# soham97/mellow

Measured on AMD Instinct MI355X. Metric: audio-pair responses/sec (v0 167M, 2x10s clips, max_len=64, greedy), higher is better.
Workload: dtype f32 (encoder/prefill GEMM operands split EXACTLY into 3 bf16 terms, 6 bf16 MFMA products per fp32 product, f32 accumulate: fp32-accurate, parity suite green; mel included, the STFT is an fp32 FFT; attentions and decode on exact fp32 MFMA / VALU)

## Files before the change

### mellow_amd/csrc/decode.hip

```cpp
#include "common.h"
#include "kernels.h"
#include <cstdio>
#include <mutex>
#include <set>
#include <type_traits>
#include <utility>

namespace mellow {

__device__ uint64_t* g_kdbg = nullptr;
#ifdef MELLOW_KDEBUG
__device__ __forceinline__ void kstamp(int slot, int idx, bool who) {
    if (g_kdbg && who) g_kdbg[slot * 8 + idx] = __builtin_readcyclecounter();
}
__device__ __forceinline__ void kspan(int seq, int end) {
    if (g_kdbg && seq >= 0 && seq < 480 && threadIdx.x == 0) {
        const unsigned long long t = wall_clock64();
        if (end) atomicMax(reinterpret_cast<unsigned long long*>(g_kdbg) + 64 + 2 * seq + 1, t);
        else atomicMin(reinterpret_cast<unsigned long long*>(g_kdbg) + 64 + 2 * seq, t);
    }
}
#else
#define kstamp(slot, idx, who) ((void)0)
#define kspan(seq, end) ((void)0)
// ... 209 lines not shown
        }
        if (nt == 0) {
            ssp = half_sum(ssp);
            if (lane < 32) ssq_s[wave * 32 + lane] = ssp;
        }
#pragma unroll
        for (int r = 0; r < 16; ++r) red[(wave * 16 + r) * 64 + lane] = acc[r];
    }
    __syncthreads();
    if (nt == 0 && tid < 32)
    {
        float ssum = ssq_s[tid & 31];
#pragma unroll
        for (int wv = 1; wv < QW; ++wv) ssum += ssq_s[wv * 32 + (tid & 31)];
        a.ssq1[((int64_t)rb * 32 + tid) * DEC_KC_QKV + kc] = ssum;
    }
    if (tid >= 256) return;
    const int mm = tid & 31, hh = (tid >> 5) & 1, gq = tid >> 6;
    float v[4];
#pragma unroll
    for (int j = 0; j < 4; ++j) {
        const int r = 4 * gq + j;
        float sacc = red[r * 64 + mm + 32 * hh];
#pragma unroll
        for (int wv = 1; wv < QW; ++wv) sacc += red[(wv * 16 + r) * 64 + mm + 32 * hh];
        v[j] = sacc;
    }
    const int n = nt * 32 + 8 * gq + 4 * hh;
    if (W8) {
#pragma unroll
        for (int j = 0; j < 4; ++j) v[j] *= wscale[n + j];
    }
    if (n < 960)
        *reinterpret_cast<float4*>(a.pq + ((int64_t)kc * a.rows + rb * 32 + mm) * 960 + n) = make_float4(v[0], v[1], v[2], v[3]);
    kspan(a.dbg_seq, 1);
}

#ifndef MELLOW_DA_ABL
#define MELLOW_DA_ABL 0
#endif
#ifndef MELLOW_DA_WAVES
#define MELLOW_DA_WAVES 8
#define MELLOW_DA_G 7
#endif
#ifndef MELLOW_DA_MINW
#define MELLOW_DA_MINW 4
#endif
constexpr int DA_MINW = MELLOW_DA_WAVES == 8 || MELLOW_DA_WAVES == 4 ? MELLOW_DA_MINW : 1;
constexpr int DA_WAVES = MELLOW_DA_WAVES;
constexpr int DA_G = MELLOW_DA_G;
#ifndef MELLOW_DA_G1
#define MELLOW_DA_G1 5
#endif
constexpr int DA_G1 = MELLOW_DA_G1 < DA_G ? MELLOW_DA_G1 : DA_G;
#ifndef MELLOW_DA16_MFMA
#define MELLOW_DA16_MFMA 1
#endif
constexpr int DA_GM = 8;
#ifndef MELLOW_DA16_KNT
#define MELLOW_DA16_KNT 0
#endif
#ifndef MELLOW_DA16_MINW
#define MELLOW_DA16_MINW MELLOW_DA_MINW
#endif
#ifndef MELLOW_DA16_NW
#define MELLOW_DA16_NW 8
#endif

template <bool KV16>
__device__ __forceinline__ float4 ld_kv(const float* page, int64_t elem) {
    if constexpr (KV16) {
        typedef unsigned u32x2 __attribute__((ext_vector_type(2)));
        const u32x2 r = __builtin_nontemporal_load(reinterpret_cast<const u32x2*>(reinterpret_cast<const uint16_t*>(page) + elem));
        return make_float4(__uint_as_float(r[0] << 16), __uint_as_float(r[0] & 0xffff0000u), __uint_as_float(r[1] << 16), __uint_as_float(r[1] & 0xffff0000u));
    } else {
        return ldg_nt(reinterpret_cast<const float4*>(page + elem));
    }
}
template <bool KV16>
__device__ __forceinline__ void st_kv(float* page, int64_t elem, float v) {
    if constexpr (KV16) reinterpret_cast<__bf16*>(page)[elem] = static_cast<__bf16>(v);
    else page[elem] = v;
}
template <bool BLK, bool FUSED, bool ONE, bool KV16, int NW, int TS>
__global__ __launch_bounds__(NW * 64, ONE ? 2 : (KV16 && MELLOW_DA16_MFMA && DA_MINW > 1 ? MELLOW_DA16_MINW : DA_MINW)) void dec_attn_kernel(float* __restrict__ k_cache, float* __restrict__ v_cache,
                                                                  const int32_t* __restrict__ d_pos_p, const float* __restrict__ pq_p,
                                                                  const float* __restrict__ xmidF_p, int Tmax_p, int gs_p, int rows_p,
                                                                  const DecArgs a) {
    kspan(a.dbg_seq, 0);
    __shared__ float ssq_part[3];
    __shared__ __attribute__((aligned(16))) float qs[3 * 64];
    __shared__ __attribute__((aligned(16))) float knew[64], vnew[64];
    __shared__ __attribute__((aligned(16))) float xs[320];
    __shared__ __attribute__((aligned(16))) float ored[DA_WAVES * 3 * 64];
    __shared__ float mred[DA_WAVES * 3], lred[DA_WAVES * 3];
    __shared__ float snew_s[3];
    constexpr bool MF = KV16 && MELLOW_DA16_MFMA != 0;
    __shared__ __attribute__((aligned(16))) float pl[MF ? DA_WAVES * 32 * 4 : 4];
    __shared__ __attribute__((aligned(16))) __bf16 qb[MF ? 10 * 64 : 8];
    constexpr int VPW = DA_WAVES / NW;
    static_assert(DA_WAVES % NW == 0 && (MF || NW == DA_WAVES), "the vector form runs one chunk stream per wave");
    auto mf_group = [&](int g0, int u) { return g0 + u * DA_WAVES; };

    static_assert(TS == DEC_TS || !(ONE || KV16), "one row block and the bf16 pages always run DEC_TS key splits (kernels.h dec_key_splits)");
    const int g = blockIdx.x, b = blockIdx.y, sp = blockIdx.z;
    int row = b;
    if (BLK) {
        const int live = a.blk_live[b >> 5];
        if (a.row_of_slot) row = a.row_of_slot[b];
        if (live == 0 || row < 0) return;
    }
    const int tid = threadIdx.x, lane = tid & 63, wave = tid >> 6;
    const int Tmax = Tmax_p;
    float* kpage = k_cache + (((int64_t)row * 3 + g) * Tmax * 64 >> (KV16 ? 1 : 0));
    float* vpage = v_cache + (((int64_t)row * 3 + g) * Tmax * 64 >> (KV16 ? 1 : 0));
    const int sub = lane >> 4, quad = lane & 15;

    const bool dbg = tid == 0 && g == 0 && b == 0 && sp == 0;
    kstamp(1, 0, dbg);
#ifdef MELLOW_POS_VECTOR_LOAD
    const int pos = __builtin_amdgcn_readfirstlane(*reinterpret_cast<const volatile int*>(d_pos_p));
#else
    const int pos = *d_pos_p;
#endif
    const int hsel = (tid >> 5) & 3, i = tid & 31;
    const int r = tid < 80 ? tid : 0;
    const int pcol = r < 48 ? (3 * g + (r >> 4)) * 64 + 4 * (r & 15) : r < 64 ? 576 + g * 64 + 4 * (r - 48) : 768 + g * 64 + 4 * (r - 64);
    const float* prow = pq_p + (int64_t)b * 960 + pcol;
    constexpr int NPQ = FUSED ? Q2_NPQ : DEC_KC_QKV;
    float4 sl4[NPQ], sq4[2];
    if (tid < 80) {
#pragma unroll
        for (int s = 0; s < NPQ; ++s)
            sl4[s] = (MELLOW_DA_ABL & 4) ? make_float4(0.1f * s, 0.2f, 0.3f, 0.4f) : *reinterpret_cast<const float4*>(prow + (int64_t)s * rows_p * 960);
        if (!FUSED) {
            sq4[0] = reinterpret_cast<const float4*>(a.ssq1 + (int64_t)b * DEC_KC_QKV)[0];
            sq4[1] = reinterpret_cast<const float4*>(a.ssq1 + (int64_t)b * DEC_KC_QKV)[1];
        }
    }
    float4 xr4 = make_float4(0.f, 0.f, 0.f, 0.f), xd4[FUSED ? Q2_HC : 1];
    if (FUSED && tid < 144) {
        const int64_t fi = ((int64_t)(b >> 5) * 72 + (tid >> 1)) * 64 + (b & 31) + 32 * (tid & 1);
        xr4 = reinterpret_cast<const float4*>(xmidF_p)[fi];
#pragma unroll
        for (int s = 0; s < Q2_HC; ++s) xd4[s] = reinterpret_cast<const float4*>(a.dslabF)[(int64_t)s * a.slabF_stride4 + fi];
    }
    const float c = a.rope_cur[i], sn = a.rope_cur[32 + i];
    const int gbeg = sp * gs_p;
    const int gend_fixed = sp == TS - 1 ? 0x3fffffff : gbeg + gs_p;
    typedef unsigned u32x2 __attribute__((ext_vector_type(2)));
    const int kk = lane & 31, hf = lane >> 5;
    i32x4 kq[4];
    u32x2 vq[DA_GM];
    auto load_ktile = [&](int g0) {
        const int gi = g0 + (kk >> 2) * DA_WAVES;
        const int tc = min(gi * 4 + (kk & 3), Tmax - 1);
        const i32x4* kp = reinterpret_cast<const i32x4*>(reinterpret_cast<const uint16_t*>(kpage) + (int64_t)tc * 64 + hf * 32);
#pragma unroll
        for (int st = 0; st < 4; ++st)
            kq[st] = (MELLOW_DA_ABL & 1) ? i32x4{tc, 0x3c003c00, st, 0x3c003c00} : (MELLOW_DA16_KNT ? __builtin_nontemporal_load(kp + st) : kp[st]);
    };
    auto load_vgroup = [&](int g0, int u) {
        const int gi = mf_group(g0, u);
        const int tc = min(gi * 4 + sub, Tmax - 1);
        vq[u] = (MELLOW_DA_ABL & 1) ? u32x2{0x3c003c00u, (unsigned)tc}
                                    : __builtin_nontemporal_load(reinterpret_cast<const u32x2*>(reinterpret_cast<const uint16_t*>(vpage) + (int64_t)tc * 64 + quad * 4));
    };
    float4 k4[MF ? 1 : DA_G], v4[MF ? 1 : DA_G];
    auto load_group = [&](int u) {
        const int gi = gbeg + wave + u * DA_WAVES;
        const int tc = min(gi * 4 + sub, Tmax - 1);
        if (MELLOW_DA_ABL & 1) {
            k4[u] = make_float4(0.01f * tc, 0.02f, 0.03f, 0.04f);
            v4[u] = make_float4(0.01f, 0.02f * tc, 0.03f, 0.04f);
        } else {
            k4[u] = ld_kv<KV16>(kpage, (int64_t)tc * 64 + quad * 4);
            v4[u] = ld_kv<KV16>(vpage, (int64_t)tc * 64 + quad * 4);
        }
    };
    const int g_first_mf = gbeg + wave;
    if constexpr (MF) {
        load_ktile(g_first_mf);
#pragma unroll
        for (int u = 0; u < DA_GM / 2; ++u) load_vgroup(g_first_mf, u);
    } else {
#pragma unroll
        for (int u = 0; u < DA_G1; ++u) load_group(u);
    }
    MELLOW_HOIST(a.attF16); MELLOW_HOIST(a.att_ml); MELLOW_HOIST(a.RB); MELLOW_HOIST(a.eps);
    if (FUSED) MELLOW_HOIST(a.xnewR);
    __builtin_amdgcn_sched_barrier(0);
    kstamp(1, 1, dbg);

    const int ngroups = (pos + 3) >> 2;
    const int gend = min(ngroups, gend_fixed);
    static_assert(DEC_KC_QKV == 8, "fixed summation order below");
    if (FUSED) {
        if (tid < 192) {
            float4 x = xr4;
#pragma unroll
            for (int s = 0; s < Q2_HC; ++s) x = f4add(x, xd4[s]);
            const float ss = wave_sum(tid < 144 ? f4ssq(x) : 0.f);
            if (lane == 0) ssq_part[wave] = ss;
            if (g == 0 && sp == 0 && tid < 144) reinterpret_cast<float4*>(a.xnewR + (int64_t)b * 576)[tid] = x;
        }
        if (tid < 80) {
            float4 x = sl4[0];
#pragma unroll
            for (int s = 1; s < NPQ; ++s) x = f4add(x, sl4[s]);
            *reinterpret_cast<float4*>(xs + 4 * tid) = x;
        }
    } else if (tid < 80) {
        float4 x = sl4[0];
#pragma unroll
        for (int s = 1; s < DEC_KC_QKV; ++s) x = f4add(x, sl4[s]);
        const float ssum = ((sq4[0].x + sq4[0].y) + (sq4[0].z + sq4[0].w)) + ((sq4[1].x + sq4[1].y) + (sq4[1].z + sq4[1].w));
        const float rscale = 1.0f / sqrtf(ssum / 576.0f + a.eps);
        *reinterpret_cast<float4*>(xs + 4 * tid) = make_float4(x.x * rscale, x.y * rscale, x.z * rscale, x.w * rscale);
    }
    __syncthreads();
    kstamp(1, 2, dbg);
    const float rs2 = FUSED ? 1.0f / sqrtf(((ssq_part[0] + ssq_part[1]) + ssq_part[2]) / 576.0f + a.eps) : 1.0f;
    if (tid < 128) {
        const int base = hsel < 3 ? hsel * 64 : 192;
        const float x1 = xs[base + i] * rs2, x2 = xs[base + i + 32] * rs2;
        const float o1 = __fadd_rn(__fmul_rn(x1, c), __fmul_rn(-x2, sn));
        const float o2 = __fadd_rn(__fmul_rn(x2, c), __fmul_rn(x1, sn));
        if (hsel < 3) {
            qs[hsel * 64 + i] = o1 * 0.125f;
            qs[hsel * 64 + i + 32] = o2 * 0.125f;
            if constexpr (MF) {
                __bf16 p0, p1, p2;
                split3(o1 * 0.125f, p0, p1, p2);
                qb[(0 * 3 + hsel) * 64 + i] = p0; qb[(1 * 3 + hsel) * 64 + i] = p1; qb[(2 * 3 + hsel) * 64 + i] = p2;
                split3(o2 * 0.125f, p0, p1, p2);
                qb[(0 * 3 + hsel) * 64 + i + 32] = p0; qb[(1 * 3 + hsel) * 64 + i + 32] = p1; qb[(2 * 3 + hsel) * 64 + i + 32] = p2;
            }
        } else {
            knew[i] = o1; knew[i + 32] = o2;
            if (sp == 0) { st_kv<KV16>(kpage, (int64_t)pos * 64 + i, o1); st_kv<KV16>(kpage, (int64_t)pos * 64 + i + 32, o2); }
        }
    } else if (tid < 192) {
        const float x1 = xs[256 + tid - 128] * rs2;
        vnew[tid - 128] = x1;
        if (sp == 0) st_kv<KV16>(vpage, (int64_t)pos * 64 + (tid - 128), x1);
    } else if (MF && tid < 256) {
        qb[9 * 64 + tid - 192] = static_cast<__bf16>(0.f);
    }
    __syncthreads();
    __builtin_amdgcn_sched_barrier(0);
    if constexpr (MF) {
#pragma unroll
        for (int u = DA_GM / 2; u < DA_GM; ++u) load_vgroup(g_first_mf, u);
    } else {
#pragma unroll
        for (int u = DA_G1; u < DA_G; ++u) load_group(u);
    }
    __builtin_amdgcn_sched_barrier(0);
    kstamp(1, 3, dbg);

    if (wave < 3) {
        const float sn_ = wave_sum(qs[wave * 64 + lane] * knew[lane]);
        if (lane == 0) snew_s[wave] = sn_;
    }
    float4 q4[3];
    const int aq_off = ((kk >> 2) < 3 && (kk & 3) < 3 ? (kk >> 2) * 3 + (kk & 3) : 9) * 64 + hf * 32;
    if constexpr (!MF) {
#pragma unroll
        for (int hh = 0; hh < 3; ++hh) q4[hh] = *reinterpret_cast<const float4*>(qs + hh * 64 + quad * 4);
    }
    float m_run[3] = {-INFINITY, -INFINITY, -INFINITY};
    float l_run[3] = {0.f, 0.f, 0.f};
    float4 acc[3];
#pragma unroll
    for (int hh = 0; hh < 3; ++hh) acc[hh] = make_float4(0.f, 0.f, 0.f, 0.f);

#define MELLOW_DA_CHUNK(g0)                                                                                              \
    {                                                                                                                    \
        float sc[DA_G][3];                                                                                               \
        float cmax[3] = {-INFINITY, -INFINITY, -INFINITY};                                                               \
_Pragma("unroll")                                                                                                        \
        for (int u = 0; u < DA_G; ++u) {                                                                                 \
            const int gi = g0 + u * DA_WAVES;                                                                            \
            const int t = gi * 4 + sub;                                                                                  \
            const bool ok = gi < gend && t < pos;                                                                        \
_Pragma("unroll")                                                                                                        \
            for (int hh = 0; hh < 3; ++hh) {                                                                             \
                float sv = q4[hh].x * k4[u].x + q4[hh].y * k4[u].y + q4[hh].z * k4[u].z + q4[hh].w * k4[u].w;            \
                sv = row16_sum(sv);                                                                                      \
                sv = ok ? sv : -INFINITY;                                                                                \
                sc[u][hh] = sv;                                                                                          \
                cmax[hh] = fmaxf(cmax[hh], sv);                                                                          \
            }                                                                                                            \
        }                                                                                                                \
_Pragma("unroll")                                                                                                        \
        for (int hh = 0; hh < 3; ++hh) {                                                                                 \
            float cm = cmax[hh];                                                                                         \
            cm = fmaxf(cm, swz_xor16(cm));                                                                               \
            cm = half_max(cm);                                                                                           \
            const float m_new = fmaxf(m_run[hh], cm);                                                                    \
            const float alpha = fast_exp(m_run[hh] - m_new);                                                             \
            m_run[hh] = m_new;                                                                                           \
// ... 369 lines not shown
#pragma unroll
    for (int r = 0; r < 16; ++r) acc[r] = 0.f;
    if constexpr (W8 == 2) {
        float am = 0.f, inv, sc;
#pragma unroll
        for (int i = 0; i < KPW; ++i) am = fmaxf(am, f4amax(x[i]));
        a8_scales(half_max(am), inv, sc);
        uint32_t xq[KPW];
#pragma unroll
        for (int i = 0; i < KPW; ++i) xq[i] = q4_e4m3(x[i], inv);
        acc = mfma8_32<KPW>(acc, w8, xq);
#pragma unroll
        for (int r = 0; r < 16; ++r) acc[r] *= sc;
    } else {
#pragma unroll
        for (int i = 0; i < KPW; ++i) acc = mfma4(acc, w[i], x[i]);
    }
    kstamp(dslot, 2, dbg && acc[0] == acc[0]);
#pragma unroll
    for (int r = 0; r < 16; ++r) red[(wave * 16 + r) * 64 + lane] = acc[r];
    __syncthreads();
    kstamp(dslot, 3, dbg);
    const bool epi = tid < 256;
    const int mm = tid & 31, hh = (tid >> 5) & 1, gq = (tid >> 6) & 3;
    float v[4];
#pragma unroll
    for (int j = 0; j < 4; ++j) {
        const int r = 4 * gq + j;
        float sacc = red[r * 64 + mm + 32 * hh];
#pragma unroll
        for (int wv = 1; wv < LM_WAVES; ++wv) sacc += red[(wv * 16 + r) * 64 + mm + 32 * hh];
        v[j] = sacc;
    }
    {
        const int n = nt * 32 + 8 * gq + 4 * hh;
        if (W8) {
#pragma unroll
            for (int j = 0; j < 4; ++j) v[j] *= wscale[n + j];
        }
        const int64_t row = (int64_t)rb * 32 + mm;
        if (epi && a.logits && n < N) *reinterpret_cast<float4*>(a.logits + row * N + n) = make_float4(v[0], v[1], v[2], v[3]);
        __syncthreads();
        float bv = v[0];
        int bi = n;
#pragma unroll
        for (int j = 1; j < 4; ++j)
            if (arg_better(v[j], n + j, bv, bi)) { bv = v[j]; bi = n + j; }
        if (epi) {
            red[tid] = bv;
            reinterpret_cast<int*>(red)[256 + tid] = bi;
        }
        __syncthreads();
        if (tid < 32) {
            float best = red[tid];
            int idx = reinterpret_cast<int*>(red)[256 + tid];
#pragma unroll
            for (int q = 1; q < 8; ++q) {
                const float ov = red[tid + 32 * q];
                const int oi = reinterpret_cast<int*>(red)[256 + tid + 32 * q];
                if (arg_better(ov, oi, best, idx)) { best = ov; idx = oi; }
            }
            const int64_t o = ((int64_t)rb * 32 + tid) * (N >> 5) + nt;
            a.cand_val[o] = best;
            a.cand_idx[o] = idx;
        }
    }
    kspan(a.dbg_seq, 1);
}


#ifndef MELLOW_H3_NW
#define MELLOW_H3_NW 8
#endif
#ifndef MELLOW_H3R_D1
#define MELLOW_H3R_D1 1
#endif
#ifndef MELLOW_H3R_D2
#define MELLOW_H3R_D2 1
#endif
#ifndef MELLOW_H3R_D4
#define MELLOW_H3R_D4 1
#endif
constexpr int H3_NW = MELLOW_H3_NW, H3_CP = 3, H3_NC = 36 / H3_CP;
template <int G, int D, bool BLK>
__global__ __launch_bounds__(H3_NW * 64) void dec_head3r_kernel(const float* __restrict__ Wp, const i32x4* __restrict__ X3, int K8p, int N,
                                                                int RB_p, const DecArgs a) {
    kspan(a.dbg_seq, 0);
    extern __shared__ __attribute__((aligned(16))) i32x4 xs[];
    constexpr int PPH = 36 / G, NCH = PPH / H3_CP;
    constexpr int STAGE = G * PPH * 3 * 64;
    static_assert(PPH * G == 36 && NCH * H3_CP == PPH && H3_NC % D == 0 && NCH % D == 0, "phases hold whole chunks");
    const int tid = threadIdx.x, lane = tid & 63, wave = tid >> 6;
    const int nt = blockIdx.x * H3_NW + wave;
    const float4* wbase = reinterpret_cast<const float4*>(Wp) + (int64_t)nt * K8p * 64 + lane;
    for (int rb0 = 0; rb0 < RB_p; rb0 += G) {
        const int gn = min(G, RB_p - rb0);
        f32x16 acc[G];
#pragma unroll
        for (int g = 0; g < G; ++g)
#pragma unroll
            for (int r = 0; r < 16; ++r) acc[g][r] = 0.f;
        float4 wn[D][2 * H3_CP];
#pragma unroll
        for (int d = 0; d < D; ++d)
#pragma unroll
            for (int i = 0; i < 2 * H3_CP; ++i) wn[d][i] = ldg_nt(wbase + (d * 2 * H3_CP + i) * 64);
        for (int ph = 0; ph < G; ++ph) {
            if (ph || rb0) __syncthreads();
            {
                constexpr int FILL = (STAGE + H3_NW * 64 - 1) / (H3_NW * 64);
                i32x4 t[FILL];
#pragma unroll
                for (int j = 0; j < FILL; ++j) {
                    const int i = tid + j * H3_NW * 64;
                    if (i < STAGE) {
                        const int g = i / (PPH * 3 * 64), rest = i % (PPH * 3 * 64);
                        t[j] = X3[(((int64_t)(rb0 + (g < gn ? g : 0)) * 36 + ph * PPH) * 3) * 64 + rest];
                    }
                }
#pragma unroll
                for (int j = 0; j < FILL; ++j) {
                    const int i = tid + j * H3_NW * 64;
                    if (i < STAGE) xs[i] = t[j];
                }
            }
            __syncthreads();
            for (int c0 = 0; c0 < NCH; c0 += D) {
#pragma unroll
                for (int d = 0; d < D; ++d) {
                    const int cc = c0 + d, c = ph * NCH + cc;
                    float4 w[2 * H3_CP];
#pragma unroll
                    for (int i = 0; i < 2 * H3_CP; ++i) w[i] = wn[d][i];
                    if (c + D < H3_NC) {
#pragma unroll
                        for (int i = 0; i < 2 * H3_CP; ++i) wn[d][i] = ldg_nt(wbase + ((c + D) * 2 * H3_CP + i) * 64);
                    }
                    __builtin_amdgcn_sched_barrier(0);
                    i32x4 wp[H3_CP][3];
#pragma unroll
                    for (int p = 0; p < H3_CP; ++p) {
                        pair_natural(w[2 * p], w[2 * p + 1]);
                        split_pair(w[2 * p], w[2 * p + 1], wp[p][0], wp[p][1], wp[p][2]);
                    }
                    const i32x4* st = xs + (cc * H3_CP) * 3 * 64 + lane;
#pragma unroll
                    for (int g = 0; g < G; ++g) {
                        if (g < gn) {
#pragma unroll
                            for (int p = 0; p < H3_CP; ++p) {
                                const i32x4 xq[3] = {st[((g * PPH + p) * 3 + 0) * 64], st[((g * PPH + p) * 3 + 1) * 64], st[((g * PPH + p) * 3 + 2) * 64]};
                                acc[g] = mma6(acc[g], wp[p], xq);
                            }
                        }
                    }
                    __builtin_amdgcn_sched_barrier(0);
                }
            }
        }
        const int m = lane & 31, h = lane >> 5;
#pragma unroll
        for (int g = 0; g < G; ++g) {
            if (g < gn && !(BLK && a.blk_live[rb0 + g] == 0)) {
                const int64_t row = (int64_t)(rb0 + g) * 32 + m;
                float bv = -INFINITY;
                int bi = 0x7fffffff;
#pragma unroll
                for (int q = 0; q < 4; ++q) {
                    const int n = nt * 32 + 8 * q + 4 * h;
                    if (a.logits) *reinterpret_cast<float4*>(a.logits + row * N + n) = make_float4(acc[g][4 * q], acc[g][4 * q + 1], acc[g][4 * q + 2], acc[g][4 * q + 3]);
#pragma unroll
                    for (int j = 0; j < 4; ++j)
                        if (arg_better(acc[g][4 * q + j], n + j, bv, bi)) { bv = acc[g][4 * q + j]; bi = n + j; }
                }
                auto rv = __builtin_amdgcn_permlane32_swap(__float_as_uint(bv), __float_as_uint(bv), false, false);
                auto ri = __builtin_amdgcn_permlane32_swap((unsigned)bi, (unsigned)bi, false, false);
                const float ov = __uint_as_float(h ? rv[0] : rv[1]);
                const int oi = (int)(h ? ri[0] : ri[1]);
                if (arg_better(ov, oi, bv, bi)) { bv = ov; bi = oi; }
                if (h == 0) {
                    const int64_t o = row * (N >> 5) + nt;
                    a.cand_val[o] = bv;
                    a.cand_idx[o] = bi;
                }
            }
        }
    }
    kspan(a.dbg_seq, 1);
}

#define MELLOW_BF16S(W, X, ACC) ACC = __builtin_amdgcn_mfma_f32_16x16x32_bf16(__builtin_bit_cast(bf16x8, W), __builtin_bit_cast(bf16x8, X), ACC, 0, 0, 0)
__device__ __forceinline__ f32x4 mma6s(f32x4 acc, const i32x4 (&w)[3], const i32x4 (&x)[3]) {
// ... 519 lines not shown
        } else {
#pragma unroll
            for (int i = 0; i < HT; ++i) acc = mfma4(acc, w[i], h4[i]);
        }
        kstamp(7, 2, dbg && acc[0] == acc[0]);
        if (side) nt -= 30;
    }
#pragma unroll
    for (int r = 0; r < 16; ++r) red[(wave * 16 + r) * 64 + lane] = acc[r];
    __syncthreads();
    kstamp(7, 3, dbg);
    if (tid < 256) {
        const int mm = tid & 31, hh = (tid >> 5) & 1, gq = tid >> 6;
        float v[4];
#pragma unroll
        for (int j = 0; j < 4; ++j) {
            const int q = 4 * gq + j;
            float sacc = red[q * 64 + mm + 32 * hh];
#pragma unroll
            for (int wv = 1; wv < Q2W; ++wv) sacc += red[(wv * 16 + q) * 64 + mm + 32 * hh];
            v[j] = sacc;
        }
        const int n = nt * 32 + 8 * gq + 4 * hh;
        if (W8) {
#pragma unroll
            for (int j = 0; j < 4; ++j) v[j] *= wsc[n + j];
        }
        const float4 o = make_float4(v[0], v[1], v[2], v[3]);
        if (side) st_out(reinterpret_cast<float4*>(a.dslabF) + (int64_t)slab * a.slabF_stride4 + f32_idx(rb, 72, mm, n), o);
        else st_out(reinterpret_cast<float4*>(a.pq + ((int64_t)slab * a.rows + rb * 32 + mm) * 960 + n), o);
    }
    kstamp(7, 4, dbg);
    kspan(a.dbg_seq, 1);
}

template <int KCD, bool BLK>
__global__ __launch_bounds__(192) void dec_final_norm_kernel(const float* __restrict__ norm_w, const float* __restrict__ xmidF_p,
                                                             const float* __restrict__ dslabF_p, int64_t stride4_p, const DecArgs a) {
    kspan(a.dbg_seq, 0);
    __shared__ float part[3];
    const int b = blockIdx.x, tid = threadIdx.x;
    if (BLK && b == 0 && tid < 32) a.blk_snap[tid] = a.blk_live[tid];
    MELLOW_BLK_EXIT(b >> 5)
    const int xi = tid < 144 ? tid : 0;
    const int64_t fi = f32_idx(b >> 5, 72, b & 31, xi * 4);
    float4 v = reinterpret_cast<const float4*>(xmidF_p)[fi];
    float4 xs[KCD > 0 ? KCD : 1];
#pragma unroll
    for (int s = 0; s < KCD; ++s) xs[s] = reinterpret_cast<const float4*>(dslabF_p)[(int64_t)s * stride4_p + fi];
    const float4 wv = reinterpret_cast<const float4*>(norm_w)[xi];
#pragma unroll
    for (int s = 0; s < KCD; ++s) v = f4add(v, xs[s]);
    float ss = tid < 144 ? f4ssq(v) : 0.f;
    ss = wave_sum(ss);
    if ((tid & 63) == 0) part[tid >> 6] = ss;
    __syncthreads();
    const float r = 1.0f / sqrtf((part[0] + part[1] + part[2]) / 576.0f + a.eps);
    if (tid < 144) {
        float4 y;
        y.x = __fmul_rn(wv.x, __fmul_rn(v.x, r)); y.y = __fmul_rn(wv.y, __fmul_rn(v.y, r));
        y.z = __fmul_rn(wv.z, __fmul_rn(v.z, r)); y.w = __fmul_rn(wv.w, __fmul_rn(v.w, r));
        if (!a.xn3) reinterpret_cast<float4*>(a.xnF)[fi] = y;
    }
    if (a.xn3) {
        float4 y = make_float4(0.f, 0.f, 0.f, 0.f);
        if (tid < 144) {
            y.x = __fmul_rn(wv.x, __fmul_rn(v.x, r)); y.y = __fmul_rn(wv.y, __fmul_rn(v.y, r));
            y.z = __fmul_rn(wv.z, __fmul_rn(v.z, r)); y.w = __fmul_rn(wv.w, __fmul_rn(v.w, r));
        }
        const F3Quad mine = f3_split4(y), other = f3_partner(mine);
        if (tid < 144 && !(tid & 1)) f3_store8(a.xn3, f3_32_slot(b >> 5, 36, b & 31, tid * 4), mine, other);
    }
    kspan(a.dbg_seq, 1);
}

__global__ __launch_bounds__(256) void dec_argmax_kernel(const float* __restrict__ cand_val_p, const int32_t* __restrict__ cand_idx_p, int n,
                                                         const DecArgs a, int32_t* __restrict__ tokens,
                                                         const float* __restrict__ embed, int write_x, const LoopArgs lp) {
    kspan(a.dbg_seq, 0);
    __shared__ float bv[4];
    __shared__ int bi[4];
    __shared__ int tok_s;
    const int b = blockIdx.x, tid = threadIdx.x;
    const int row = lp.row_of_slot ? lp.row_of_slot[b] : b;
    const bool dead = (lp.blk_snap && lp.blk_snap[b >> 5] == 0) || row < 0;
    float best = -INFINITY;
    int idx = 0x7fffffff;
    if (!dead) {
        for (int i = tid; i < n; i += 256) {
            const float v = cand_val_p[(int64_t)b * n + i];
            const int id = cand_idx_p[(int64_t)b * n + i];
            if (arg_better(v, id, best, idx)) { best = v; idx = id; }
        }
#pragma unroll
        for (int off = 32; off > 0; off >>= 1) {
            const float ov = __shfl_xor(best, off, 64);
            const int oi = __shfl_xor(idx, off, 64);
            if (arg_better(ov, oi, best, idx)) { best = ov; idx = oi; }
        }
        if ((tid & 63) == 0) { bv[tid >> 6] = best; bi[tid >> 6] = idx; }
    }
    __syncthreads();
    if (tid == 0) {
        if (!dead) {
            for (int w = 1; w < 4; ++w)
                if (arg_better(bv[w], bi[w], best, idx)) { best = bv[w]; idx = bi[w]; }
            idx = min(max(idx, 0), n * 32 - 1);
            tokens[b] = idx;
            tok_s = idx;
        }
        if (lp.out_tokens) {
            if (!dead) {
                const int max_len = lp.params[0], stop_id = lp.params[1];
                const int step = *a.d_pos - lp.T0 + 1;
                if (step >= 0 && step < max_len) lp.out_tokens[(int64_t)row * max_len + step] = idx;
                if (idx == stop_id && lp.seen_stop[row] == 0) {
                    lp.seen_stop[row] = 1;
                    atomicAdd(lp.n_seen, 1);
                    if (lp.blk_left && atomicSub(lp.blk_left + (b >> 5), 1) == 1) lp.blk_live[b >> 5] = 0;
                }
            }
            asm volatile("s_waitcnt vmcnt(0)" ::: "memory");
            if (atomicAdd(lp.arrive, 1) == (int)gridDim.x - 1) {
                *lp.arrive = 0;
                const int t = *lp.ticket + 1;
                *lp.ticket = t;
                const int ns = atomicAdd(lp.n_seen, 0);
                __hip_atomic_store(lp.host_progress, ((unsigned long long)(unsigned)t << 32) | (unsigned)ns, __ATOMIC_RELAXED,
                                   __HIP_MEMORY_SCOPE_SYSTEM);
            }
        }
    }
    if (dead) return;
    if (write_x) {
        __syncthreads();
        if (tid < 144) {
            const float4 e = reinterpret_cast<const float4*>(embed + (int64_t)tok_s * 576)[tid];
            reinterpret_cast<float4*>(a.xmidF)[f32_idx(b >> 5, 72, b & 31, tid * 4)] = e;
        }
    }
    kspan(a.dbg_seq, 1);
}

__global__ __launch_bounds__(1024) void dec_compact_kernel(const DecArgs a, int B, const LoopArgs lp) {
    __shared__ int src_of[1024];
    __shared__ int row_new[1024];
    __shared__ int wsum[16];
    __shared__ int n_act_s, n_live_s;
    const int tid = threadIdx.x, lane = tid & 63, wave = tid >> 6;
    const int nblk = (B + 31) >> 5;
    int row = -1, active = 0;
    if (tid < B) {
        row = lp.row_of_slot[tid];
        active = row >= 0 && lp.blk_live[tid >> 5] != 0 && lp.seen_stop[row] == 0;
    }
    const unsigned long long m = __ballot(active);
    const int before = __popcll(m & ((1ull << lane) - 1ull));
    if (lane == 0) wsum[wave] = __popcll(m);
    if (tid == 0) {
        int live = 0;
        for (int k = 0; k < nblk; ++k) live += lp.blk_live[k] != 0;
        n_live_s = live;
    }
    src_of[tid] = -1;
    row_new[tid] = -1;
    __syncthreads();
    int base = 0;
    for (int w = 0; w < wave; ++w) base += wsum[w];
    if (tid == 0) {
        int n = 0;
        for (int w = 0; w < 16; ++w) n += wsum[w];
        n_act_s = n;
    }
    __syncthreads();
    const int n_act = n_act_s;
    if ((n_act + 31) / 32 >= n_live_s) return;
    if (active) { src_of[base + before] = tid; row_new[base + before] = row; }
    __syncthreads();
    float4* x = reinterpret_cast<float4*>(a.xmidF);
    for (int d0 = 0; d0 < n_act; d0 += 7) {
        const int d = d0 + tid / 144, c = tid % 144;
        const bool mv = tid < 1008 && d < n_act && src_of[d] != d;
        float4 v = make_float4(0.f, 0.f, 0.f, 0.f);
        if (mv) v = x[f32_idx(src_of[d] >> 5, 72, src_of[d] & 31, c * 4)];
        __syncthreads();
        if (mv) x[f32_idx(d >> 5, 72, d & 31, c * 4)] = v;
        __syncthreads();
    }
    if (tid < B) lp.row_of_slot[tid] = row_new[tid];
    if (tid < 32) {
        const int left = tid < nblk ? min(max(n_act - 32 * tid, 0), 32) : 0;
        lp.blk_left[tid] = left;
        lp.blk_live[tid] = left > 0;
    }
    if (tid == 0) *lp.n_compactions += 1;
}
__global__ __launch_bounds__(256) void kv_to_bf16_kernel(const float4* __restrict__ src, uint4* __restrict__ dst, int64_t n8) {
    for (int64_t i = (int64_t)blockIdx.x * 256 + threadIdx.x; i < n8; i += (int64_t)gridDim.x * 256) {
        const float4 a = src[2 * i], b = src[2 * i + 1];
        typedef __bf16 bf16x8v __attribute__((ext_vector_type(8)));
        const bf16x8v o = {static_cast<__bf16>(a.x), static_cast<__bf16>(a.y), static_cast<__bf16>(a.z), static_cast<__bf16>(a.w),
                           static_cast<__bf16>(b.x), static_cast<__bf16>(b.y), static_cast<__bf16>(b.z), static_cast<__bf16>(b.w)};
        dst[i] = __builtin_bit_cast(uint4, o);
    }
}
void launch_kv_to_bf16(const float* src, void* dst, int64_t n, hipStream_t s) {
    const int64_t n8 = n >> 3;
    const int blocks = (int)((n8 + 255) / 256 < 8192 ? (n8 + 255) / 256 : 8192);
    hipLaunchKernelGGL(kv_to_bf16_kernel, dim3(blocks), dim3(256), 0, s, reinterpret_cast<const float4*>(src), reinterpret_cast<uint4*>(dst), n8);
}
void launch_dec_compact(const DecArgs& a, int B, const LoopArgs& loop, hipStream_t s) {
    hipLaunchKernelGGL(dec_compact_kernel, dim3(1), dim3(1024), 0, s, a, B, loop);
}

__global__ __launch_bounds__(192) void dec_load_rows_kernel(const DecArgs a, const float* __restrict__ in, int64_t ld,
                                                            const int32_t* __restrict__ row_ids, int T_last, int n_src) {
    const int b = blockIdx.x, tid = threadIdx.x;
    const int64_t src = row_ids ? (int64_t)min(max(row_ids[b], 0), n_src - 1) : (int64_t)b * T_last + (T_last - 1);
    if (tid < 144) {
        const float4 e = reinterpret_cast<const float4*>(in + src * ld)[tid];
        reinterpret_cast<float4*>(a.xmidF)[f32_idx(b >> 5, 72, b & 31, tid * 4)] = e;
    }
}

void set_max_dynamic_lds(const void* fn, size_t bytes) {
    if (bytes <= 64 * 1024) return;
    static std::mutex mu;
    static std::set<std::pair<const void*, int>> done;
    int dev = 0;
    (void)hipGetDevice(&dev);
    std::lock_guard<std::mutex> lk(mu);
    if (done.insert({fn, dev}).second) {
        const hipError_t e = hipFuncSetAttribute(fn, hipFuncAttributeMaxDynamicSharedMemorySize, (int)bytes);
        if (e != hipSuccess) fprintf(stderr, "mellow: hipFuncSetAttribute(max dynamic LDS %zu) failed: %s\n", bytes, hipGetErrorString(e));
    }
}
template <class F> static inline void with_bool(bool v, F&& f) {
    if (v) f(std::true_type{}); else f(std::false_type{});
}
template <int V0, int... Vs, class F> static inline void with_int(int v, F&& f) {
    if constexpr (sizeof...(Vs) == 0) f(std::integral_constant<int, V0>{});
    else if (v == V0) f(std::integral_constant<int, V0>{});
    else with_int<Vs...>(v, f);
}
static inline int w8_mode(const DecArgs& a, const float* wscale) { return wscale ? (a.a8 ? 2 : 1) : 0; }
template <class F> static inline void with_blk_w8(const DecArgs& a, const float* wscale, F&& f) {
    with_bool(a.blk_live != nullptr, [&](auto blk) { with_int<2, 1, 0>(w8_mode(a, wscale), [&](auto w8) { f(blk, w8); }); });
}
void launch_dec_qkv(const DecArgs& a, const float* Wp, int K8p, int kcd, hipStream_t s, const float* wscale) {
    const dim3 grid(30, DEC_KC_QKV, a.RB);
    with_int<0, DEC_KC_DOWN>(kcd, [&](auto kcd_c) { with_bool(a.first != 0, [&](auto first) { with_blk_w8(a, wscale, [&](auto blk, auto w8) {
        hipLaunchKernelGGL((dec_qkv_kernel<kcd_c.value, blk.value, first.value, w8.value>), grid, dim3(QKV_THREADS), 0, s, Wp, (const float*)a.xmidF,
                           (const float*)a.dslabF, K8p, a, wscale);
    }); }); });
}
void launch_dec_attn(const DecArgs& a, float* k_cache, float* v_cache, bool fused, hipStream_t s) {
    const dim3 grid(3, a.rows, a.ts);
    const bool one = a.RB == 1 && !a.blk_live;
    if (a.ts != DEC_TS && (one || a.kv16 || a.ts != DEC_TS_MULTI)) {
        fprintf(stderr, "mellow: decode attention launched with %d key splits at RB = %d\n", a.ts, a.RB);
        abort();
    }
    auto launch = [&](auto blk, auto one_c) { with_bool(fused, [&](auto fused_c) { with_bool(a.kv16 != 0, [&](auto kv16) {
        constexpr bool ONE = one_c.value, KV16 = kv16.value;
        constexpr int NW = !KV16 ? DA_WAVES : MELLOW_DA16_MFMA && DA_WAVES == 8 && !ONE ? MELLOW_DA16_NW : DA_WAVES;
        constexpr int TSM = ONE || KV16 ? DEC_TS : DEC_TS_MULTI;
        with_int<DEC_TS, TSM>(a.ts, [&](auto ts) {
            hipLaunchKernelGGL((dec_attn_kernel<blk.value, fused_c.value, ONE, KV16, NW, ts.value>), grid, dim3(NW * 64), 0, s, k_cache, v_cache,
                               (const int32_t*)a.d_pos, (const float*)a.pq, (const float*)a.xmidF, a.Tmax, a.gs, a.rows, a);
        });
    }); }); };
    if (one) launch(std::false_type{}, std::true_type{});
    else with_bool(a.blk_live != nullptr, [&](auto blk) { launch(blk, std::false_type{}); });
}
static void launch_dec_qkv2_any(const DecArgs& a, const float* Wx, int K8x, const float* Wh, int K8h, const float* Wd,
                                const float* sc_x, const float* sc_h, const float* sc_d, hipStream_t s) {
    const dim3 grid(Q2_BLOCKS, a.RB);
#ifdef MELLOW_Q2_WAVES_FORCED
    bool few = false;
#else
    bool few = a.RB == 1;
#endif
    if (w8_mode(a, sc_x) == 2) few = false;
    with_bool(few, [&](auto few_c) { with_blk_w8(a, sc_x, [&](auto blk, auto w8) {
        constexpr int WV = few_c.value ? 4 : Q2_WAVES;
        hipLaunchKernelGGL((dec_qkv2_kernel<blk.value, WV, w8.value>), grid, dim3(WV * 64), 0, s, Wx, Wh, Wd, (const float*)a.xmidF,
                           (const float*)a.guF, K8x, K8h, a, sc_x, sc_h, sc_d);
    }); });
}
constexpr size_t dec_qkv2x3_lds(int rbm) { return (size_t)Q3W * rbm * 16 * 64 * 4; }
constexpr size_t dec_gateup3_lds(int rbm) { return (size_t)GU3W * rbm * 8 * 64 * 4; }
constexpr size_t dec_head3r_lds() { return (size_t)36 * 3 * 64 * 16; }
template <class F> static inline void with_qkv2x3(int rb, bool blk, F&& f) {
    with_int<1, 2, 4>(rb, [&](auto rbm) { with_bool(blk, [&](auto b) { f(&dec_qkv2x3_kernel<b.value, rbm.value>, dec_qkv2x3_lds(rbm.value)); }); });
}
template <class F> static inline void with_gateup3(int rb, bool blk, F&& f) {
    with_int<1, 2, 4>(rb, [&](auto rbm) { with_bool(blk, [&](auto b) { f(&dec_gateup3_kernel<b.value, rbm.value>, dec_gateup3_lds(rbm.value)); }); });
}
template <class F> static inline void with_head3r(int rb, bool blk, F&& f) {
    with_int<1, 2, 4>(rb, [&](auto g) { with_bool(blk, [&](auto b) {
        constexpr int G = g.value, D = G == 1 ? MELLOW_H3R_D1 : G == 2 ? MELLOW_H3R_D2 : MELLOW_H3R_D4;
        f(&dec_head3r_kernel<G, D, b.value>, dec_head3r_lds());
    }); });
}
void launch_dec_qkv2x3(const DecArgs& a, const float* Wq2, const float* Wd, hipStream_t s) {
    const float* Wh = Wq2 + (size_t)72 * 64 * 4;
    const i32x4 *x3 = reinterpret_cast<const i32x4*>(a.xmid3_32), *h3 = reinterpret_cast<const i32x4*>(a.h3);
    with_qkv2x3(a.RB, a.blk_live != nullptr, [&](auto* kernel, size_t lds) {
        set_max_dynamic_lds(reinterpret_cast<const void*>(kernel), lds);
        hipLaunchKernelGGL(kernel, dim3(Q2_BLOCKS), dim3(Q3W * 64), lds, s, Wq2, Wh, Wd, x3, h3, Q2_K8, Q2_K8, a.RB, a);
    });
}
void launch_dec_gateup3(const DecArgs& a, const float* Wp16, hipStream_t s) {
    const i32x4* x3 = reinterpret_cast<const i32x4*>(a.xmid3_16);
    with_gateup3(a.RB, a.blk_live != nullptr, [&](auto* kernel, size_t lds) {
        set_max_dynamic_lds(reinterpret_cast<const void*>(kernel), lds);
        hipLaunchKernelGGL(kernel, dim3(192), dim3(GU3W * 64), lds, s, Wp16, x3, (const float*)a.ssq, a.RB, a);
    });
}
void launch_dec_qkv2(const DecArgs& a, const float* Wq2, const float* Wd, hipStream_t s) {
    launch_dec_qkv2_any(a, Wq2, Q2_K8, Wq2 + (size_t)72 * 64 * 4, Q2_K8, Wd, nullptr, nullptr, nullptr, s);
}
void launch_dec_qkv2_w8(const DecArgs& a, const float* Wx8, const float* sc_x, const float* Wh8, const float* sc_h,
                        const float* Wd8, const float* sc_d, hipStream_t s) {
    launch_dec_qkv2_any(a, Wx8, 72, Wh8, 192, Wd8, sc_x, sc_h, sc_d, s);
}
__global__ __launch_bounds__(256) void compose_f64_kernel(const float* __restrict__ A, const float* __restrict__ B, float* __restrict__ C,
                                                          int M, int N, int K) {
    __shared__ double as[16][17], bs[16][17];
    const int tx = threadIdx.x & 15, ty = threadIdx.x >> 4;
    const int m = blockIdx.y * 16 + ty, n = blockIdx.x * 16 + tx;
    double acc = 0.0;
    for (int k0 = 0; k0 < K; k0 += 16) {
        as[ty][tx] = (m < M && k0 + tx < K) ? (double)A[(int64_t)m * K + k0 + tx] : 0.0;
        bs[ty][tx] = (k0 + ty < K && n < N) ? (double)B[(int64_t)(k0 + ty) * N + n] : 0.0;
        __syncthreads();
#pragma unroll
        for (int kk = 0; kk < 16; ++kk) acc += as[ty][kk] * bs[kk][tx];
        __syncthreads();
    }
    if (m < M && n < N) C[(int64_t)m * N + n] = (float)acc;
}
void launch_compose_f64(const float* A, const float* B, float* C, int M, int N, int K, hipStream_t s) {
    hipLaunchKernelGGL(compose_f64_kernel, dim3((N + 15) / 16, (M + 15) / 16), dim3(256), 0, s, A, B, C, M, N, K);
}
int dec_attn_chunk_groups(bool kv16) { return DA_WAVES * (kv16 && MELLOW_DA16_MFMA ? DA_GM : DA_G); }
void launch_dec_oproj(const DecArgs& a, const float* Wp16, hipStream_t s, const float* wscale) {
#ifdef MELLOW_OPROJ_ROWS
    const int rows = MELLOW_OPROJ_ROWS;
#else
    const int rows = a.RB == 1 ? 8 : 16;
#endif
    with_int<8, 16>(rows, [&](auto rows_c) { with_int<1, DEC_TS>(a.ts, [&](auto ts) { with_blk_w8(a, wscale, [&](auto blk, auto w8) {
        constexpr int ROWS = rows_c.value, PARTS = ROWS == 8 ? 4 : 2;
        hipLaunchKernelGGL((dec_oproj_kernel<blk.value, w8.value, ROWS, ts.value>), dim3(36, PARTS * a.RB), dim3(OP_WAVES * 64), 0, s, Wp16,
                           (const float*)a.attF16, (const float*)a.att_ml, (const float*)a.xnewR, a.RB, a.rows, a, wscale);
    }); }); });
}
void launch_dec_gateup(const DecArgs& a, const float* Wp16, hipStream_t s, const float* wscale) {
    with_blk_w8(a, wscale, [&](auto blk, auto w8) {
        hipLaunchKernelGGL((dec_gateup16_kernel<blk.value, w8.value>), dim3(192, a.RB), dim3(GU_WAVES * 64), 0, s, Wp16, a.xmidF16, a.ssq, a, wscale);
    });
}
void launch_dec_down(const DecArgs& a, const float* Wp, int K8p, hipStream_t s, const float* wscale) {
    with_blk_w8(a, wscale, [&](auto blk, auto w8) {
        hipLaunchKernelGGL((dec_down_kernel<blk.value, w8.value>), dim3(18, DEC_KC_DOWN, a.RB), dim3(DN_WAVES * 64), 0, s, Wp, (const float*)a.guF,
                           K8p, a, wscale);
    });
}
void launch_dec_final_norm(const DecArgs& a, const float* norm_w, int kcd, hipStream_t s) {
    with_int<0, DEC_KC_DOWN>(kcd, [&](auto kcd_c) { with_bool(a.blk_live != nullptr, [&](auto blk) {
        hipLaunchKernelGGL((dec_final_norm_kernel<kcd_c.value, blk.value>), dim3(a.rows), dim3(192), 0, s, norm_w, (const float*)a.xmidF,
                           (const float*)a.dslabF, a.slabF_stride4, a);
    }); });
}
bool dec_head3r_fits(int vocab) { return vocab % 32 == 0 && (vocab / 32) % H3_NW == 0; }
void launch_dec_lm_head(const DecArgs& a, const float* Wp, int K8p, int vocab, hipStream_t s, const float* wscale) {
    if ((a.x3 & DEC_X3_HEAD) && !wscale && a.xn3 && (vocab / 32) % H3_NW == 0) {
        const i32x4* X3 = reinterpret_cast<const i32x4*>(a.xn3);
        with_head3r(a.RB, a.blk_live != nullptr, [&](auto* kernel, size_t lds) {
            set_max_dynamic_lds(reinterpret_cast<const void*>(kernel), lds);
            hipLaunchKernelGGL(kernel, dim3(vocab / 32 / H3_NW), dim3(H3_NW * 64), lds, s, Wp, X3, K8p, vocab, a.RB, a);
        });
        return;
    }
    with_blk_w8(a, wscale, [&](auto blk, auto w8) {
        hipLaunchKernelGGL((dec_fullk_kernel<OUT_LOGITS, blk.value, w8.value>), dim3(vocab / 32, 1, a.RB), dim3(LM_WAVES * 64), 0, s, Wp,
                           (const float*)a.xnF, K8p, vocab, a, wscale);
    });
}
void dec_prepare_lds_attributes() {
    const auto raise = [](auto* kernel, size_t lds) { set_max_dynamic_lds(reinterpret_cast<const void*>(kernel), lds); };
    for (const int rb : {1, 2, 4})
        for (const bool blk : {false, true}) {
            with_head3r(rb, blk, raise);
            with_qkv2x3(rb, blk, raise);
            with_gateup3(rb, blk, raise);
        }
}
__global__ __launch_bounds__(256) void pack_dec_fp8_kernel(const float4* __restrict__ Wp, int slots, int rows, uint32_t* __restrict__ out,
                                                           float* __restrict__ scale) {
    __shared__ unsigned amax_s[32];
    __shared__ float inv_s[32];
    const int tile = blockIdx.x, tid = threadIdx.x;
    if (tid < 32) amax_s[tid] = 0u;
    __syncthreads();
    const float4* src = Wp + (int64_t)tile * slots;
    for (int i = tid; i < slots; i += 256) {
        const float4 v = src[i];
        const float m = fmaxf(fmaxf(fabsf(v.x), fabsf(v.y)), fmaxf(fabsf(v.z), fabsf(v.w)));
        atomicMax(&amax_s[(i & 63) & (rows - 1)], __float_as_uint(m));
    }
    __syncthreads();
    if (tid < rows) {
        const float am = __uint_as_float(amax_s[tid]);
        const float sc = am > 0.f ? am / 448.0f : 1.0f;
        scale[(int64_t)tile * rows + tid] = sc;
        inv_s[tid] = 1.0f / sc;
    }
    __syncthreads();
    for (int i = tid; i < slots; i += 256) {
        const float4 v = src[i];
        const float inv = inv_s[(i & 63) & (rows - 1)];
        int w = 0;
        w = __builtin_amdgcn_cvt_pk_fp8_f32(v.x * inv, v.y * inv, w, false);
        w = __builtin_amdgcn_cvt_pk_fp8_f32(v.z * inv, v.w * inv, w, true);
        out[(int64_t)tile * slots + i] = (uint32_t)w;
    }
}
void launch_pack_dec_fp8(const float* Wp, int tiles, int slots_per_tile, int rows_per_tile, void* out, float* scale, hipStream_t s) {
    hipLaunchKernelGGL(pack_dec_fp8_kernel, dim3(tiles), dim3(256), 0, s, reinterpret_cast<const float4*>(Wp), slots_per_tile,
                       rows_per_tile, reinterpret_cast<uint32_t*>(out), scale);
}
void launch_dec_argmax(const DecArgs& a, int B, int n_tiles, int32_t* tokens, const float* embed, int write_x,
                       const LoopArgs& loop, hipStream_t s) {
    hipLaunchKernelGGL(dec_argmax_kernel, dim3(B), dim3(256), 0, s, (const float*)a.cand_val, (const int32_t*)a.cand_idx, n_tiles, a, tokens, embed,
                       write_x, loop);
}
void launch_dec_load_rows(const DecArgs& a, int B, const float* in, int64_t ld, const int32_t* row_ids, int T_last,
                          int n_src, hipStream_t s) {
    hipLaunchKernelGGL(dec_load_rows_kernel, dim3(B), dim3(192), 0, s, a, in, ld, row_ids, T_last, n_src);
}

__global__ __launch_bounds__(1024) void argmax_kernel(const float* __restrict__ logits, int V, int64_t ld,
                                                      int32_t* __restrict__ tokens) {
    __shared__ float bv[16];
    __shared__ int bi[16];
    const int b = blockIdx.x, tid = threadIdx.x;
    const float4* row = reinterpret_cast<const float4*>(logits + (int64_t)b * ld);
    float best = -INFINITY;
    int idx = 0x7fffffff;
    for (int i = tid; i < (V >> 2); i += 1024) {
        const float4 v = row[i];
        const float vv[4] = {v.x, v.y, v.z, v.w};
#pragma unroll
        for (int j = 0; j < 4; ++j)
            if (arg_better(vv[j], 4 * i + j, best, idx)) { best = vv[j]; idx = 4 * i + j; }
    }
#pragma unroll
    for (int off = 32; off > 0; off >>= 1) {
        const float ov = __shfl_xor(best, off, 64);
        const int oi = __shfl_xor(idx, off, 64);
        if (arg_better(ov, oi, best, idx)) { best = ov; idx = oi; }
    }
    if ((tid & 63) == 0) { bv[tid >> 6] = best; bi[tid >> 6] = idx; }
    __syncthreads();
    if (tid == 0) {
        for (int w = 1; w < 16; ++w)
            if (arg_better(bv[w], bi[w], best, idx)) { best = bv[w]; idx = bi[w]; }
        tokens[b] = min(max(idx, 0), V - 1);
    }
}
void launch_argmax(const float* logits, int B, int V, int64_t ld, int32_t* tokens, hipStream_t s) {
    hipLaunchKernelGGL(argmax_kernel, dim3(B), dim3(1024), 0, s, logits, V, ld, tokens);
}
// ... 34 lines not shown
```

### mellow_amd/csrc/engine.cpp

```cpp
#include "engine_internal.h"

static thread_local std::string g_err;
int fail(const char* fmt, ...) {
    char buf[1024];
    va_list ap;
    va_start(ap, fmt);
    vsnprintf(buf, sizeof(buf), fmt, ap);
    va_end(ap);
    g_err = buf;
    return 1;
}
int ensure(mellow_engine* e, mellow_engine::Buf& b, size_t floats) {
    if (b.cap >= floats) return 0;
    if (b.p) HIPCHK(hipFree(b.p));
    b.p = nullptr;
    b.cap = 0;
    HIPCHK(hipMalloc(&b.p, floats * sizeof(float)));
    b.cap = floats;
    return 0;
}
int dev_alloc(mellow_engine* e, float** out, size_t floats) {
    const size_t bytes = (floats * sizeof(float) + 4095) / 4096 * 4096;
    if (!e->arena) {
        const size_t want = (size_t)(e->opt.arena_mb < 0 ? 0 : e->opt.arena_mb) << 20;
// ... 183 lines not shown
    if (cfg->abi_version != MELLOW_ABI_VERSION) return fail("ABI version mismatch: caller %d, library %d", cfg->abi_version, MELLOW_ABI_VERSION);
    if (cfg->hidden_size != 576 || cfg->head_dim != 64 || cfg->num_heads != 9 || cfg->num_kv_heads != 3 ||
        cfg->intermediate_size != 1536)
        return fail("unsupported decoder geometry (engine is built for SmolLM2-135M: hidden 576, 9q/3kv heads x 64, inter 1536)");
    if (cfg->prefix_len != 2 * 129 + 2 + cfg->text_len) return fail("prefix_len must be 2*129+2+text_len");
    if (cfg->vocab_size % 128) return fail("vocab_size must be a multiple of 128");
    int n = 0;
    if (hipGetDeviceCount(&n) != hipSuccess || n <= 0) return fail("no HIP device available: the Mellow engine has no CPU fallback");
    if (device < 0 || device >= n) return fail("device %d out of range (%d devices)", device, n);
    HIPCHK(hipSetDevice(device));
    mellow_engine* e = new mellow_engine();
    e->cfg = *cfg;
    e->device = device;
    HIPCHK(hipStreamCreateWithFlags(&e->stream, hipStreamNonBlocking));
    HIPCHK(hipEventCreateWithFlags(&e->ev_fork, hipEventDisableTiming));
    for (int i = 0; i < 3; ++i) HIPCHK(hipEventCreateWithFlags(&e->ev_join[i], hipEventDisableTiming));
    for (int i = 0; i < 4; ++i) HIPCHK(hipEventCreate(&e->ev_phase[i]));
    *out = e;
    return mellow_engine_set_precision(e, MELLOW_PRECISION_F32X3);
}

void mellow_engine_destroy(mellow_engine_t* e) {
    if (!e) return;
    hipSetDevice(e->device);
    if (e->stream) hipStreamSynchronize(e->stream);
    if (e->parent && --e->parent->n_forks == 0) e->parent->prefill_parts = e->parent->prefill_parts_saved;
    e->graphs.reset();
    for (void* p : e->allocs) hipFree(p);
    for (auto ev : e->ev_pool) hipEventDestroy(ev);
    for (int i = 0; i < 4; ++i)
        if (e->ev_phase[i]) hipEventDestroy(e->ev_phase[i]);
    if (e->d_tokens) hipFree(e->d_tokens);
    if (e->h_progress) hipHostFree(e->h_progress);
    if (e->ev_fork) hipEventDestroy(e->ev_fork);
    for (int i = 0; i < 3; ++i) {
        if (e->ev_join[i]) hipEventDestroy(e->ev_join[i]);
        if (e->stream2[i]) hipStreamDestroy(e->stream2[i]);
    }
    if (e->stream) hipStreamDestroy(e->stream);
    delete e;
}

int mellow_engine_load_tensor(mellow_engine_t* e, const char* key, const void* data, const int64_t* shape, int ndim,
                              int dtype) {
    if (!e || !key || !data) return fail("null argument");
    if (e->finalized) return fail("engine already finalized");
    std::string k = key;
    if (k.rfind("module.", 0) == 0) k = k.substr(7);
    if (is_ignored_key(k)) return 0;
    bool known = (k == "mellow.rope_cos" || k == "mellow.rope_sin");
    if (!known) {
        for (const auto& r : build_required(&e->cfg))
            if (r == k) { known = true; break; }
    }
    if (!known) return fail("unexpected key in state_dict: %s", key);
    HostTensor t;
    t.dtype = dtype;
    for (int i = 0; i < ndim; ++i) t.shape.push_back(shape[i]);
    const size_t esz = dtype == MELLOW_I64 ? 8 : 4;
    t.data.resize((size_t)t.numel() * esz);
    HIPCHK(hipSetDevice(e->device));
    HIPCHK(hipMemcpy(t.data.data(), data, t.data.size(), hipMemcpyDefault));
    e->host[k] = std::move(t);
    return 0;
}

}

int alloc_state_words(mellow_engine* e) {
    HIPCHK(hipMalloc(&e->d_tokens, 4096 * sizeof(int32_t)));
    HIPCHK(hipMemset(e->d_tokens, 0, 4096 * sizeof(int32_t)));
    e->d_step = e->d_tokens + 1024;
    e->d_pos = e->d_tokens + 1025;
    e->d_nseen = e->d_tokens + 1026;
    e->d_arrive = e->d_tokens + 1027;
    e->d_ticket = e->d_tokens + 1028;
    e->d_params = e->d_tokens + 1032;
    e->d_sparams = reinterpret_cast<uint32_t*>(e->d_tokens + 1536);
    e->d_blk_left = e->d_tokens + 1040;
    e->d_blk_live = e->d_tokens + 1072;
    e->d_seen = e->d_tokens + 2048;
    e->d_row_of_slot = e->d_tokens + 3072;
    e->d_ncompact = e->d_tokens + 1029;
    HIPCHK(hipHostMalloc(reinterpret_cast<void**>(&e->h_progress), 64, hipHostMallocMapped | hipHostMallocCoherent));
    *e->h_progress = 0;
    HIPCHK(hipHostGetDevicePointer(reinterpret_cast<void**>(&e->d_progress), e->h_progress, 0));
    return 0;
}

__global__ void stream_probe_kernel(unsigned long long* out, unsigned long long ticks) {
    const unsigned long long t0 = wall_clock64();
    out[0] = t0;
    while (wall_clock64() - t0 < ticks) __builtin_amdgcn_s_sleep(8);
    out[1] = wall_clock64();
}
static int streams_overlap(mellow_engine* e, hipStream_t a, hipStream_t b, bool* yes) {
    unsigned long long* d = nullptr;
    HIPCHK(hipMalloc(&d, 4 * sizeof(unsigned long long)));
    HIPCHK(hipMemsetAsync(d, 0, 4 * sizeof(unsigned long long), a));
    HIPCHK(hipStreamSynchronize(a));
    HIPCHK(hipStreamSynchronize(b));
    hipLaunchKernelGGL(stream_probe_kernel, dim3(1), dim3(1), 0, a, d, 20000ull);
    hipLaunchKernelGGL(stream_probe_kernel, dim3(1), dim3(1), 0, b, d + 2, 2000ull);
    HIPCHK(hipStreamSynchronize(a));
    HIPCHK(hipStreamSynchronize(b));
    unsigned long long h[4];
    HIPCHK(hipMemcpy(h, d, sizeof(h), hipMemcpyDeviceToHost));
    HIPCHK(hipFree(d));
    *yes = h[2] < h[1];
    return 0;
}
int ensure_prefill_streams(mellow_engine* e) {
    if (e->n_forks > 0 || e->parent) return 0;
    if (e->streams_probed) {
        if (++e->probe_backoff < 16) { e->prefill_parts = e->prefill_parts_ok; return 0; }
        e->streams_probed = false;
        e->probe_backoff = 0;
        e->prefill_parts = e->prefill_parts_want;
    }
    int nh = e->prefill_parts < 1 ? 1 : (e->prefill_parts > 4 ? 4 : e->prefill_parts);
    for (int h = 1; h < nh; ++h) {
        if (e->stream2[h - 1]) continue;
        bool ok = false;
        for (int attempt = 0; attempt < 8 && !ok; ++attempt) {
            hipStream_t st = nullptr;
            HIPCHK(hipStreamCreateWithFlags(&st, hipStreamNonBlocking));
            int rc = streams_overlap(e, e->stream, st, &ok);
            for (int k = 1; k < h && ok && !rc; ++k) rc = streams_overlap(e, e->stream2[k - 1], st, &ok);
            if (rc) { hipStreamDestroy(st); return rc; }
            if (ok) e->stream2[h - 1] = st; else hipStreamDestroy(st);
        }
        if (!ok) {
            e->prefill_parts_want = e->prefill_parts;
            e->prefill_parts = e->prefill_parts_ok = h;
            e->streams_probed = true;
            break;
        }
    }
    return 0;
}
struct OptDesc { const char* key; const char* dflt; bool answers; const char* what; };
static const OptDesc kOptions[] = {
    {"prefill_split", "2", false, "f32x3: parts of the split LM prefill (1..4); bit-identical for every value"},
    {"prefill_fuse_norm", "1", true, "f32x3: norm-free LM prefill (GEMM epilogues emit split output + RMS partials); 0 = a normalisation launch per GEMM input"},
    {"decode_fuse", "1", true, "down projection of layer l fused with q/k/v of layer l + 1 through the load-time product W'Wd; 0 = five launches per layer"},
    {"decode_fuse_max_rb", "1", true, "largest number of 32-row blocks that runs the fused down + q/k/v launch on fp32 weights"},
    {"splitk", "8", true, "f32x3 encoder: largest split count of the split-K launches (0 = never split; a summation order)"},
    {"enc_apb", "0x1CC", false, "f32x3 encoder: Swin stages whose producers hand over pre-split (bit st, 4 + st, 8 + st); bit-identical"},
    {"graph", "1", false, "decode steps as hipGraph replays (0 = eager launches)"},
    {"fp8_decode", "1", true, "fp8 mode: e4m3 weights in the decode kernels"},
    {"fp8_prefill", "1", true, "fp8 mode: e4m3 GEMMs in encoder + LM prefill"},
    {"fp8_decode_act", "1", true, "fp8 mode: e4m3 activations in the decode GEMM kernels (fp8 matrix pipe)"},
    {"fp8_kv16", "1", true, "fp8 mode: bf16 shadow of the K/V pages for the decode step"},
    {"fp8_attn_bf16", "1", true, "fp8 mode: q / k / v stored once as bf16 (LM: bf16 K/V pages + bf16-once prefill attention; Swin: bf16 q/k/v rows into the exact window attention); 0 = fp32 q/k/v, the 3-way split attention"},
    {"decode_x3", "7", true, "f32x3: mask of decode GEMM launches on the bf16 pipe (1 lm_head, 2 gate/up, 4 fused down + q/k/v)"},
    {"decode_x3_min_rb", "2", true, "f32x3: fewest 32-row blocks at which the layer launches take their f32x3 forms"},
    {"x3_stft", "1", true, "f32x3: STFT / mel GEMMs on the split kernel (0 = exact fp32 kernel)"},
    {"stft_fft", "1", true, "f32x3: STFT as a 1024-point FFT when the checkpoint's conv weights are the windowed DFT basis"},
    {"x3_apb", "1", true, "f32x3 LM prefill: producers hand over pre-split, GEMMs staged by LDS-DMA (0 = register-staged kernel on fp32 activations)"},
    {"x3_attn", "1", true, "f32x3: prefill attention on exact bf16 splits (0 = exact fp32 MFMA kernel)"},
    {"x3w", "1", false, "f32x3: K = 96 GEMMs on the weight-stationary persistent kernel; bit-identical"},
    {"row_migration", "1", false, "reference-semantics loop, B > 32: rows still running are packed into the lowest 32-row blocks; tokens unchanged"},
    {"arena_mb", "3400", false, "size of the weight arena in MiB (before the first tensor is loaded)"},
};
static const OptDesc* find_opt(const char* key) {
    for (const auto& o : kOptions)
        if (!strcmp(o.key, key)) return &o;
    return nullptr;
}
static long opt_val(const mellow_engine* e, const char* key) {
    auto it = e->opt.given.find(key);
    return strtol(it != e->opt.given.end() ? it->second.c_str() : find_opt(key)->dflt, nullptr, 0);
}
int apply_options(mellow_engine* e) {
    const int mode = e->opt.mode;
    e->prefill_parts = (int)opt_val(e, "prefill_split");
    e->opt.prefill_fuse_norm = opt_val(e, "prefill_fuse_norm") != 0;
    e->opt.decode_fuse = opt_val(e, "decode_fuse") != 0;
    e->opt.dec_fuse_max_rb = (int)opt_val(e, "decode_fuse_max_rb");
    e->opt.sk_max = (int)opt_val(e, "splitk");
    e->opt.enc_apb_stages = (int)opt_val(e, "enc_apb");
    e->use_graph = opt_val(e, "graph") != 0;
    e->opt.x3_stft = opt_val(e, "x3_stft") != 0;
    e->opt.stft_fft = opt_val(e, "stft_fft") != 0 && e->opt.x3_stft;
    e->opt.x3_apb = opt_val(e, "x3_apb") != 0;
    e->opt.x3_attn = opt_val(e, "x3_attn") != 0;
    e->opt.x3w = opt_val(e, "x3w") != 0;
    e->opt.row_migration = opt_val(e, "row_migration") != 0;
    e->opt.arena_mb = (int)opt_val(e, "arena_mb");
    e->opt.fp8 = mode == MELLOW_PRECISION_FP8;
    e->opt.fp8_decode = e->opt.fp8 && opt_val(e, "fp8_decode") != 0;
    e->opt.fp8_decode_act = e->opt.fp8_decode && opt_val(e, "fp8_decode_act") != 0;
    e->opt.fp8_prefill = opt_val(e, "fp8_prefill") != 0;
    e->opt.fp8_attn_bf16 = opt_val(e, "fp8_attn_bf16") != 0;
    e->opt.kv16 = e->opt.fp8_decode && opt_val(e, "fp8_kv16") != 0;
    e->opt.f32x3_terms = mode == MELLOW_PRECISION_F32X3 ? 6 : 0;
    e->opt.dec_x3 = mode == MELLOW_PRECISION_F32X3 ? ((int)opt_val(e, "decode_x3") & DEC_X3_ALL) : 0;
    e->opt.dec_x3_min_rb = (int)opt_val(e, "decode_x3_min_rb") < 1 ? 1 : (int)opt_val(e, "decode_x3_min_rb");
    return 0;
}

extern "C" {

int mellow_engine_set_option(mellow_engine_t* e, const char* key, const char* value) {
    if (!e || !key || !value) return fail("null argument");
    if (e->finalized) return fail("options must be set before mellow_engine_finalize");
    const OptDesc* o = find_opt(key);
    if (!o) return fail("unknown option \"%s\" (mellow_engine_describe lists them)", key);
    char* end = nullptr;
    const long v = strtol(value, &end, 0);
    if (end == value || *end) return fail("option \"%s\": \"%s\" is not an integer", key, value);
    if (!strcmp(key, "prefill_split") && (v < 1 || v > 4)) return fail("option prefill_split must be 1..4");
    if (!strcmp(key, "arena_mb") && e->arena) return fail("option arena_mb must be set before the first tensor is loaded");
    e->opt.given[key] = value;
    return apply_options(e);
}

int64_t mellow_engine_describe(mellow_engine_t* e, char* buf, int64_t capacity) {
    if (!e) return -1;
    std::string s = "{\"abi\": [" + std::to_string(MELLOW_ABI_VERSION) + ", " + std::to_string(MELLOW_ABI_MINOR) + "], \"precision\": \"";
    s += e->opt.mode == MELLOW_PRECISION_F32 ? "f32" : e->opt.mode == MELLOW_PRECISION_FP8 ? "fp8" : "f32x3";
    s += "\", \"reads_environment\": false, \"finalized\": ";
    s += e->finalized ? "true" : "false";
    s += ", \"stft_is_fft\": ";
    s += e->w.fft_win ? "true" : "false";
    s += ", \"non_default\": [";
    bool first = true;
    for (const auto& o : kOptions)
        if (opt_val(e, o.key) != strtol(o.dflt, nullptr, 0)) { s += std::string(first ? "" : ", ") + "\"" + o.key + "\""; first = false; }
    s += "], \"options\": {";
    first = true;
    for (const auto& o : kOptions) {
        s += std::string(first ? "" : ", ") + "\"" + o.key + "\": {\"value\": " + std::to_string(opt_val(e, o.key)) + ", \"default\": " +
             std::to_string(strtol(o.dflt, nullptr, 0)) + ", \"changes_answers\": " + (o.answers ? "true" : "false") + "}";
        first = false;
    }
    s += "}}";
    if (buf && capacity > (int64_t)s.size()) memcpy(buf, s.c_str(), s.size() + 1);
    return (int64_t)s.size() + 1;
}

int mellow_last_steps_enqueued(mellow_engine_t* e) { return e ? e->last_steps_enqueued : -1; }

int mellow_last_row_repacks(mellow_engine_t* e) { return e ? e->last_compactions : -1; }

int mellow_stft_is_fft(mellow_engine_t* e) { return e && e->w.fft_win ? 1 : 0; }

int mellow_abi_minor(void) { return MELLOW_ABI_MINOR; }
int mellow_prefill_parts(mellow_engine_t* e) {
    if (!e) return -1;
    if (!e->opt.f32x3_terms && !(e->opt.fp8 && e->opt.fp8_prefill)) return 1;
    if (hipSetDevice(e->device) != hipSuccess) return -1;
    if (ensure_prefill_streams(e) != 0) return -1;
    return e->prefill_parts < 1 ? 1 : (e->prefill_parts > 4 ? 4 : e->prefill_parts);
}

int mellow_prof_enable(mellow_engine_t* e, int on) {
    if (!e) return fail("null engine");
    e->prof_on = on != 0;
    return 0;
}

int mellow_prof_reset(mellow_engine_t* e) {
    if (!e) return fail("null engine");
    hipStreamSynchronize(e->stream);
    e->prof.clear();
    e->ev_used = 0;
    return 0;
}

int mellow_prof_get(mellow_engine_t* e, int i, int64_t* launches, double* ms, double* flops, double* bytes) {
// ... 68 lines not shown
```

### mellow_amd/csrc/engine_dev.cpp

```cpp
#include "engine_internal.h"

extern "C" {

__attribute__((visibility("default"))) int mellow_dev_gemm_time(mellow_engine_t* e, int M, int N, int K, int iters, float* ms_out) {
    if (!e || M <= 0 || N <= 0 || K <= 0 || K % 32 || N % 4 || iters <= 0 || !ms_out) return fail("bad argument");
    HIPCHK(hipSetDevice(e->device));
    mellow_engine::Buf A, W, Cc;
    const size_t NP = (size_t)rup(N, 128);
    CHK(ensure(e, A, (size_t)M * K));
    CHK(ensure(e, W, NP * K));
    CHK(ensure(e, Cc, (size_t)M * N));
    HIPCHK(hipMemsetAsync(A.p, 0x3c, (size_t)M * K * 4, e->stream));
    HIPCHK(hipMemsetAsync(W.p, 0x3c, NP * K * 4, e->stream));
    GemmArgs g;
    g.A = A.p; g.lda = K; g.M = M; g.K = K; g.Wp = W.p; g.Nw = N; g.N = N; g.C = Cc.p; g.ldc = N;
    launch_gemm(g, e->stream);
    hipEvent_t a, b;
    HIPCHK(hipEventCreate(&a));
    HIPCHK(hipEventCreate(&b));
    HIPCHK(hipEventRecord(a, e->stream));
    for (int i = 0; i < iters; ++i) launch_gemm(g, e->stream);
    HIPCHK(hipEventRecord(b, e->stream));
    HIPCHK(hipEventSynchronize(b));
    float ms = 0.f;
    HIPCHK(hipEventElapsedTime(&ms, a, b));
    *ms_out = ms / iters;
    hipEventDestroy(a); hipEventDestroy(b);
    return 0;
}

int mellow_debug_gemm_f32(mellow_engine_t* e, int mode, const float* A, int M, int K, const float* W, int N, float* C_out,
                          int iters, float* ms2) {
    if (!e || !A || !W || M <= 0 || N <= 0 || K <= 0 || K % 32 || N % 4) return fail("bad argument");
    if (mode != 0 && mode != 16 && mode != 17) return fail("mode must be 0 (fp32 MFMA), 16 (f32x3, A split in registers) or 17 (f32x3, pre-split A, LDS-DMA)");
    HIPCHK(hipSetDevice(e->device));
    hipStream_t s = e->stream;
    const int NP = rup(N, 128);
    mellow_engine::Buf bA, bW, bWp, bC, bA3, bPB;
    CHK(ensure(e, bA, (size_t)M * K));
    CHK(ensure(e, bW, (size_t)N * K));
    CHK(ensure(e, bWp, (size_t)NP * K));
    CHK(ensure(e, bC, (size_t)M * N));
    CHK(ensure(e, bA3, (size_t)rup(M, 128) * K * 6 / 4));
    CHK(ensure(e, bPB, (size_t)NP * K * 6 / 4));
    float *dA = bA.p, *dW = bW.p, *dWp = bWp.p, *dC = bC.p;
    void *dA3 = bA3.p, *dPB = bPB.p;
    HIPCHK(hipMemcpy(dA, A, (size_t)M * K * 4, hipMemcpyHostToDevice));
    HIPCHK(hipMemcpy(dW, W, (size_t)N * K * 4, hipMemcpyHostToDevice));
    launch_pack_weight(dW, N, K, K, dWp, NP, K, s);
    launch_pack_bf16x3(dWp, NP, K, dPB, s);
    GemmArgs g;
    g.A = dA; g.lda = K; g.M = M; g.K = K; g.Wp = dWp; g.Nw = N; g.N = N; g.C = dC; g.ldc = N;
    g.A8 = reinterpret_cast<const uint8_t*>(dA3); g.lda8 = (int64_t)3 * (K >> 3); g.W8 = reinterpret_cast<const uint8_t*>(dPB);
    auto run = [&](bool pre, bool main) {
        if (mode == 0) { if (main) launch_gemm(g, s); }
        else if (mode == 16) { if (main) launch_gemm_bf16x3_fused(g, s); }
        else { if (pre) launch_split_rows_apb(dA, K, M, K, dA3, s); if (main) launch_gemm_bf16x3_apb(g, s); }
    };
    run(true, true);
    HIPCHK(hipGetLastError());
    HIPCHK(hipStreamSynchronize(s));
    if (C_out) HIPCHK(hipMemcpy(C_out, dC, (size_t)M * N * 4, hipMemcpyDeviceToHost));
    if (ms2 && iters > 0) {
        hipEvent_t a, b;
        HIPCHK(hipEventCreate(&a));
        HIPCHK(hipEventCreate(&b));
        float m0 = 0.f, m1 = 0.f;
        HIPCHK(hipEventRecord(a, s));
        for (int i = 0; i < iters; ++i) run(true, false);
        HIPCHK(hipEventRecord(b, s));
        HIPCHK(hipEventSynchronize(b));
        HIPCHK(hipEventElapsedTime(&m0, a, b));
        HIPCHK(hipEventRecord(a, s));
        for (int i = 0; i < iters; ++i) run(false, true);
        HIPCHK(hipEventRecord(b, s));
        HIPCHK(hipEventSynchronize(b));
        HIPCHK(hipEventElapsedTime(&m1, a, b));
        ms2[0] = m0 / iters;
        ms2[1] = m1 / iters;
        hipEventDestroy(a); hipEventDestroy(b);
    }
    return 0;
}

int mellow_debug_gemm_fp8(mellow_engine_t* e, const float* A, int M, int K, const float* W, int N, float* C_out, int iters,
                        float* ms_out) {
    if (!e || !A || !W || M <= 0 || N <= 0 || K <= 0 || K % 32 || N % 4) return fail("bad argument");
    HIPCHK(hipSetDevice(e->device));
    hipStream_t s = e->stream;
    const int NP = rup(N, 128), K64 = rup(K, 64), Mp = rup(M, 128);
    mellow_engine::Buf bA, bW, bWp, bC, bsa, bsw, bA8, bW8;
    CHK(ensure(e, bA, (size_t)M * K));
    CHK(ensure(e, bW, (size_t)N * K));
    CHK(ensure(e, bWp, (size_t)NP * K));
    CHK(ensure(e, bC, (size_t)M * N));
    CHK(ensure(e, bsa, (size_t)Mp * ((K64 / 64 + 3) / 4) * 2));
    CHK(ensure(e, bsw, (size_t)NP));
    CHK(ensure(e, bA8, (size_t)Mp * K64 / 4));
    CHK(ensure(e, bW8, (size_t)NP * K64 / 4));
    float *dA = bA.p, *dW = bW.p, *dWp = bWp.p, *dC = bC.p, *dsa = bsa.p, *dsw = bsw.p;
    uint8_t *dA8 = reinterpret_cast<uint8_t*>(bA8.p), *dW8 = reinterpret_cast<uint8_t*>(bW8.p);
    HIPCHK(hipMemcpy(dA, A, (size_t)M * K * 4, hipMemcpyHostToDevice));
    HIPCHK(hipMemcpy(dW, W, (size_t)N * K * 4, hipMemcpyHostToDevice));
    launch_pack_weight(dW, N, K, K, dWp, NP, K, s);
    launch_pack_fp8(dWp, NP, K, dW8, dsw, s);
    GemmArgs g;
    g.A = dA; g.lda = K; g.M = M; g.K = K; g.Wp = dWp; g.Nw = N; g.N = N; g.C = dC; g.ldc = N;
    g.A8 = dA8; g.lda8 = K64; g.a_sc = reinterpret_cast<const uint32_t*>(dsa); g.W8 = dW8; g.w_scale = dsw;
    launch_quant_mx8(dA, K, M, K, dA8, dsa, s);
    launch_gemm_fp8(g, s);
    HIPCHK(hipGetLastError());
// ... 71 lines not shown
```

### mellow_amd/csrc/engine_internal.h

```cpp
#pragma once
#include <hip/hip_runtime.h>

#include <chrono>
#include <cmath>
#include <cstdarg>
#include <cstdio>
#include <cstdlib>
#include <cstring>
#include <map>
#include <unordered_map>
#include <string>
#include <thread>
#include <type_traits>
#include <utility>
#include <vector>

#include "../../include/mellow_hip.h"
#include "kernels.h"

using namespace mellow;

int fail(const char* fmt, ...);
struct mellow_engine;
int apply_options(mellow_engine* e);
// ... 29 lines not shown
    std::vector<char> data;
    std::vector<int64_t> shape;
    int dtype = 0;
    int64_t numel() const {
        int64_t n = 1;
        for (auto d : shape) n *= d;
        return n;
    }
    const float* f() const { return reinterpret_cast<const float*>(data.data()); }
};

struct Packed {
    float* p = nullptr;
    int N = 0, K = 0, NP = 0, KP = 0;
    int Nw = 0;
};

struct SwinBlockW {
    float *n1w, *n1b, *n2w, *n2b;
    Packed qkv, proj, fc1, fc2;
    float *qkv_b, *proj_b, *fc1_b, *fc2_b;
    float* bias_exp;
    float* mask;
};
struct MergeW {
    float *nw, *nb;
    Packed red;
};
struct DecW {
    const float *p, *scale;
};
struct LMLayerW {
    Packed qkv, o, gateup, down;
    Packed qkv_f, gateup_f;
    float* o16 = nullptr;
    float* gu16n = nullptr;
    float* gu16 = nullptr;
    float* qkv2 = nullptr;
    float *q2h8 = nullptr, *q2h_sc = nullptr;
    float *qkv8 = nullptr, *qkv_sc = nullptr, *o8 = nullptr, *o_sc = nullptr, *gu8 = nullptr, *gu_sc = nullptr, *dn8 = nullptr,
          *dn_sc = nullptr;
    float *in_ln, *post_ln;
    DecW qkv_w() const { return qkv8 ? DecW{qkv8, qkv_sc} : DecW{qkv_f.p, nullptr}; }
    DecW o_w() const { return o8 ? DecW{o8, o_sc} : DecW{o16, nullptr}; }
    DecW gateup_w() const { return gu8 ? DecW{gu8, gu_sc} : DecW{gu16, nullptr}; }
    DecW down_w() const { return dn8 ? DecW{dn8, dn_sc} : DecW{down.p, nullptr}; }
};

struct ProfRec {
    int fam;
    hipEvent_t a, b;
    double flops, bytes;
    int M = 0, N = 0, K = 0, epi = 0;
};

#define LOCAL __attribute__((visibility("hidden")))
struct mellow_engine {
    struct Buf {
        float* p = nullptr;
        size_t cap = 0;
        Buf() = default; Buf(const Buf&) = delete; Buf& operator=(const Buf&) = delete;
        Buf(Buf&& o) noexcept : p(o.p), cap(o.cap) { o.p = nullptr; o.cap = 0; }
        Buf& operator=(Buf&& o) noexcept { std::swap(p, o.p); std::swap(cap, o.cap); return *this; }
        LOCAL ~Buf() { if (p) (void)hipFree(p); }
    };
    struct LOCAL Options {
        std::map<std::string, std::string> given;
        int mode = MELLOW_PRECISION_F32X3;
        bool x3_stft = true, stft_fft = true, x3_apb = true, x3_attn = true, x3w = true, row_migration = true, decode_fuse = true;
        int arena_mb = 3400;
        bool kv16 = false;
        bool fp8 = false;
        bool fp8_decode = false;
        bool fp8_decode_act = false;
        bool fp8_attn_bf16 = true;
        bool fp8_prefill = true;
        int dec_x3_min_rb = 2;
        int dec_x3 = 0;
        int f32x3_terms = 0;
        bool prefill_fuse_norm = true;
        int enc_apb_stages = 0x1CC;
        int sk_max = 8;
        int dec_fuse_max_rb = 1;
    };
    struct Fp8W { uint8_t* w8; float* scale; };
    struct LOCAL Weights {
        Packed dft, mel;
        float *fft_win = nullptr, *fft_tw1 = nullptr, *fft_tw2 = nullptr;
        float *bn_alpha = nullptr, *bn_beta = nullptr;
        float *pe_w = nullptr, *pe_b = nullptr, *pe_nw = nullptr, *pe_nb = nullptr;
        std::vector<SwinBlockW> blocks[4];
        MergeW merge[3];
        int32_t* win_map[4][2] = {{nullptr}};
        float *fn_w = nullptr, *fn_b = nullptr;
        Packed tscam, c2l, lin1, lin2;
        float *tscam_b = nullptr, *c2l_b = nullptr, *pln_w = nullptr, *pln_b = nullptr;
        int32_t* emb_row_map = nullptr;
        float* embed = nullptr;
        Packed lm_head;
        std::vector<LMLayerW> layers;
        float* final_norm = nullptr;
        float *rope_cos = nullptr, *rope_sin = nullptr;
        float *head8 = nullptr, *head_sc = nullptr;
        DecW head_w() const { return head8 ? DecW{head8, head_sc} : DecW{lm_head.p, nullptr}; }
        std::unordered_map<const float*, void*> bf_w;
        std::unordered_map<const float*, Fp8W> fp8_w;
    };
    struct LOCAL StepGraphs {
        struct Key {
            int B = -1, Tmax = -1, sample = -1;
            const void *out_tok = nullptr, *blk_live = nullptr, *row_of_slot = nullptr;
            bool operator==(const Key& k) const { return B == k.B && Tmax == k.Tmax && out_tok == k.out_tok && blk_live == k.blk_live && row_of_slot == k.row_of_slot && sample == k.sample; }
        };
        hipGraphExec_t one = nullptr, eight = nullptr;
        Key key;
        StepGraphs() = default; StepGraphs(const StepGraphs&) = delete; StepGraphs& operator=(const StepGraphs&) = delete;
        void reset() {
            for (hipGraphExec_t* x : {&one, &eight}) if (*x) { (void)hipGraphExecDestroy(*x); *x = nullptr; }
        }
        ~StepGraphs() { reset(); }
    };

    mellow_config_t cfg;
    int device = 0;
    hipStream_t stream = nullptr;
    Options opt;
    Weights w;
    bool use_graph = true;
    int prefill_parts = 2;
    bool streams_probed = false;
    int probe_backoff = 0, prefill_parts_ok = 1, prefill_parts_want = 2;
    hipStream_t stream2[3] = {nullptr, nullptr, nullptr};
    hipEvent_t ev_fork = nullptr, ev_join[3] = {nullptr, nullptr, nullptr};
    bool finalized = false;
    bool owns_weights = true;
    std::map<std::string, HostTensor> host;
    std::vector<void*> allocs;
    char* arena = nullptr;
    size_t arena_size = 0, arena_used = 0;
    bool decode_only_weight = false;

    Buf wavcat, wpad, power, logmel, X0, X1, T, QKV, H, ats, fpx, fpxavg, latv, emb33, e1, gbuf, sbuf, proj33;
    Buf lm_x, lm_xn, lm_q, lm_o, lm_h, kcache, vcache;
    Buf kcache16, vcache16;
    bool kv16_direct = false;
    Buf lm_xn3, lm_o3, lm_h3;
    Buf lm_ssq;
    Buf dec;
    Buf dlogits, cand;
    Buf sc_prefix, sc_part, sc_ws;
    Buf sk_ws;
    bool sk_enable = false;
    Buf enc_a3, enc_h3;
    Buf a8, a8_scale;
    DecArgs da;
    int32_t *d_tokens = nullptr, *d_step = nullptr, *d_pos = nullptr, *d_seen = nullptr, *d_nseen = nullptr;
    int32_t *d_arrive = nullptr, *d_ticket = nullptr, *d_params = nullptr;
    int32_t *d_blk_left = nullptr, *d_blk_live = nullptr;
    int32_t *d_row_of_slot = nullptr, *d_ncompact = nullptr;
    int last_compactions = 0;
    unsigned long long* h_progress = nullptr;
    unsigned long long* d_progress = nullptr;
    std::map<std::pair<int, int>, float*> resample_banks;
    int32_t h_params[2] = {0, 0};
    uint32_t* d_sparams = nullptr;
    uint32_t h_sparams[SMP_WORDS] = {0};
    bool sample_on = false;
    int32_t h_blk[64] = {0};
    std::vector<int32_t> h_ident;
    int last_steps_enqueued = 0;
    Buf out_tok;
    int kv_B = 0, kv_Tmax = 0;
    int cur_B = 0, cur_pos = 0;
    int32_t h_pos_word = 0;
    StepGraphs graphs;

    bool taps_on = false;
    std::map<std::string, Buf> taps;
    std::map<std::string, int64_t> tap_numel;

    uint64_t dbg_spans[960] = {};
    int dbg_seq0 = -1;
    mellow_engine* parent = nullptr;
    int n_forks = 0, prefill_parts_saved = 2;

    bool prof_on = false;
    std::vector<ProfRec> prof;
    std::vector<hipEvent_t> ev_pool;
    size_t ev_used = 0;
    hipEvent_t ev_phase[4] = {nullptr, nullptr, nullptr, nullptr};
    float phase_ms[3] = {0, 0, 0};
};

#undef LOCAL
static_assert(!std::is_copy_constructible<mellow_engine::Buf>::value, "a Buf owns its device memory: it moves, it is never copied");
static_assert(std::is_copy_assignable<mellow_engine::Weights>::value && std::is_copy_assignable<mellow_engine::Options>::value, "a fork copies these by assignment: no owning member (Buf, StepGraphs) belongs in them");

int ensure(mellow_engine* e, mellow_engine::Buf& b, size_t floats);
int dev_alloc(mellow_engine* e, float** out, size_t floats);
int upload(mellow_engine* e, float** out, const float* src, size_t floats, size_t alloc_floats = 0);
hipEvent_t next_event(mellow_engine* e);
int tap(mellow_engine* e, const char* name, const float* src, int64_t n);
std::vector<std::string> build_required(const mellow_config_t* cfg);
const std::vector<std::string>& default_required();
bool is_ignored_key(const std::string& k);
void window_map_host(int R, int shift, int32_t* out);
void pack_weight_host(const float* w, int N, int K, int NP, int KP, float* out);
void rope_tables_host(float theta, int head_dim, int P, float* c, float* s);
int alloc_state_words(mellow_engine* e);
struct ProfScope {
    mellow_engine* e;
    ProfRec r;
    bool on;
    ProfScope(mellow_engine* e_, int fam, double flops, double bytes) : e(e_), on(e_->prof_on) {
        if (on) {
            r.fam = fam;
            r.flops = flops;
            r.bytes = bytes;
            r.a = next_event(e);
            r.b = next_event(e);
            hipEventRecord(r.a, e->stream);
        }
    }
    ~ProfScope() {
        if (on) {
            hipEventRecord(r.b, e->stream);
            e->prof.push_back(r);
        }
    }
};
int run_gemm(mellow_engine* e, const GemmArgs& a);
int run_gemm_apb(mellow_engine* e, const GemmArgs& a, const void* a3, hipStream_t st = nullptr, const void* a3_scales = nullptr);
GemmArgs lin(const float* A, int64_t lda, int M, const Packed& w, float* C, int64_t ldc, const float* bias);
int run_encoder(mellow_engine* e, const float* wav, int n, int64_t n_samples, int want_logmel_only, int apply_bn, float* logmel_out);
static inline int rb_of(int B) { return (B + 31) / 32; }
static inline size_t kv_layer_floats(const mellow_engine* e) { return (size_t)e->kv_B * 3 * e->kv_Tmax * 64; }
struct RecordArgs {
    bool embed_next = false;
};
int ensure_lm(mellow_engine* e, int B, int T, int Tmax, int ctx_end = 0);
int clear_page_tails(mellow_engine* e, int T, int t_end);
LoopArgs loop_args(mellow_engine* e);
int run_lm_head(mellow_engine* e, int B, int pending_kcd, const RecordArgs* rec);
int run_prefill(mellow_engine* e, int B, int T, const RecordArgs* rec, bool all_positions = false);
int enqueue_decode_layer_range(mellow_engine* e, int B, int l_begin, int l_end, bool inc_pos);
int enqueue_decode_layers(mellow_engine* e, int B, const RecordArgs* rec);
int ensure_prefill_streams(mellow_engine* e);
int encode_pair_to_prefix(mellow_engine* e, const float* a1, const float* a2, int64_t n_samples, const int32_t* ids, int B, float* prefix_out);
int run_score_head(mellow_engine* e, int B, int T, int from_pos, int n, const int32_t* targets, float* out_logprob,
                   int32_t* out_argmax, float* out_lse, float* out_max);
void clear_bad_id(mellow_engine* e);
int check_bad_id(mellow_engine* e);
```

### mellow_amd/csrc/engine_lm.cpp

```cpp
#include "engine_internal.h"

int ensure_lm(mellow_engine* e, int B, int T, int Tmax, int ctx_end) {
    if (B > 1024) return fail("batch of %d exceeds the 1024 rows one pass takes (mellow_generate chunks larger batches itself; the decode state block is sized for 32 row blocks)", B);
    if (ctx_end <= 0 || ctx_end > Tmax) ctx_end = Tmax;
    if (Tmax > e->cfg.max_positions) return fail("prefix + max_len = %d exceeds max_positions %d", Tmax, e->cfg.max_positions);
    const size_t Mp = (size_t)B * T;
    CHK(ensure(e, e->lm_x, Mp * 576));
    CHK(ensure(e, e->lm_xn, Mp * 576));
    CHK(ensure(e, e->lm_q, Mp * 576));
    CHK(ensure(e, e->lm_o, Mp * 576));
    CHK(ensure(e, e->lm_h, Mp * 1536));
    if (e->opt.f32x3_terms || (e->opt.fp8 && e->opt.fp8_prefill)) {
        const size_t Mq = (size_t)rup((int)Mp, 128) + 3 * 128;
        CHK(ensure(e, e->lm_xn3, Mq * 576 * 6 / 4));
        CHK(ensure(e, e->lm_o3, Mq * 576 * 6 / 4));
        CHK(ensure(e, e->lm_h3, Mq * 1536 * 6 / 4));
        CHK(ensure(e, e->lm_ssq, Mq * 2 * 16));
    }
    e->kv16_direct = e->opt.kv16 && e->opt.fp8 && e->opt.fp8_prefill && e->opt.fp8_attn_bf16 && e->opt.x3_apb && e->opt.x3_attn && !e->w.layers.empty() &&
                     e->w.fp8_w.count(e->w.layers[0].qkv.p) != 0;
    dec_prepare_lds_attributes();
    const int Bp = rb_of(B) * 32;
    if (e->kv_B != Bp || e->kv_Tmax != Tmax) {
        e->kv_B = Bp;
        e->kv_Tmax = Tmax;
        CHK(ensure(e, e->kcache, kv_layer_floats(e) * e->cfg.num_layers));
        CHK(ensure(e, e->vcache, kv_layer_floats(e) * e->cfg.num_layers));
        if (e->opt.kv16) {
            CHK(ensure(e, e->kcache16, kv_layer_floats(e) * e->cfg.num_layers / 2));
            CHK(ensure(e, e->vcache16, kv_layer_floats(e) * e->cfg.num_layers / 2));
        }
        HIPCHK(hipMemsetAsync(e->kcache.p, 0, kv_layer_floats(e) * e->cfg.num_layers * sizeof(float), e->stream));
        HIPCHK(hipMemsetAsync(e->vcache.p, 0, kv_layer_floats(e) * e->cfg.num_layers * sizeof(float), e->stream));
        if (e->opt.kv16) {
            HIPCHK(hipMemsetAsync(e->kcache16.p, 0, kv_layer_floats(e) * e->cfg.num_layers * sizeof(float) / 2, e->stream));
            HIPCHK(hipMemsetAsync(e->vcache16.p, 0, kv_layer_floats(e) * e->cfg.num_layers * sizeof(float) / 2, e->stream));
        }
        e->graphs.reset();
    }
    {
        const size_t RB = (size_t)Bp / 32, V = (size_t)e->cfg.vocab_size;
        const size_t n_x = (size_t)Bp * 576;
        size_t off = 0;
        auto take = [&](size_t n) { size_t o = off; off += (n + 63) / 64 * 64; return o; };
        const size_t o_xmidF = take(n_x), o_xnewR = take(n_x), o_xnF = take(n_x * 3 / 2);
        const size_t o_dslabF = take(DEC_KC_DOWN * n_x), o_ssq1 = take((size_t)Bp * DEC_KC_QKV), o_rope = take(64);
        const size_t o_pq = take((size_t)DEC_KC_QKV * Bp * 960);
        const size_t o_att = take((size_t)DEC_TS * n_x), o_aml = take((size_t)DEC_TS * 9 * Bp * 2);
        const size_t o_ssq = take((size_t)Bp * 40), o_gu = take(RB * 192 * 256), o_xmidF16 = take(n_x);
        const bool x3l = (e->opt.dec_x3 & DEC_X3_GATEUP) && (e->opt.dec_x3 & DEC_X3_QKV) && (int)RB >= e->opt.dec_x3_min_rb && !e->opt.fp8_decode &&
                         e->w.layers.size() > 1 && e->w.layers[1].qkv2 != nullptr && e->w.layers[1].gu16n != nullptr;
        const size_t o_x3a = take(x3l ? n_x * 3 / 2 : 0), o_x3b = take(x3l ? n_x * 3 / 2 : 0), o_h3 = take(x3l ? RB * 192 * 256 * 3 / 2 : 0);
        const bool fresh = e->dec.cap < off;
        CHK(ensure(e, e->dec, off));
        CHK(ensure(e, e->dlogits, (size_t)Bp * V));
        CHK(ensure(e, e->cand, (size_t)2 * Bp * (V / 32)));
        if (fresh) {
            HIPCHK(hipMemsetAsync(e->dec.p, 0, off * sizeof(float), e->stream));
            e->graphs.reset();
        }
        float* p = e->dec.p;
        DecArgs& a = e->da;
        a.rows = Bp; a.RB = (int)RB; a.Tmax = Tmax; a.eps = e->cfg.rms_norm_eps; a.d_pos = e->d_pos; a.inc_pos = 0; a.first = 0;
        a.a8 = e->opt.fp8_decode_act ? 1 : 0;
        a.kv16 = e->opt.kv16 ? 1 : 0;
        a.x3 = e->opt.dec_x3;
        a.blk_live = nullptr;
        a.row_of_slot = nullptr;
        a.rope_cos = e->w.rope_cos; a.rope_sin = e->w.rope_sin;
        a.xmidF = p + o_xmidF; a.xnewR = p + o_xnewR; a.xnF = p + o_xnF;
        a.xn3 = (a.x3 & DEC_X3_HEAD) && !e->w.head8 && dec_head3r_fits(e->cfg.vocab_size) ? (void*)(p + o_xnF) : nullptr;
        a.xmid3_32 = x3l ? (void*)(p + o_x3a) : nullptr; a.xmid3_16 = x3l ? (void*)(p + o_x3b) : nullptr; a.h3 = x3l ? (void*)(p + o_h3) : nullptr;
        a.dslabF = p + o_dslabF; a.slabF_stride4 = (int64_t)(n_x / 4); a.ssq1 = p + o_ssq1; a.rope_cur = p + o_rope;
        {
            const int ng_end = (ctx_end - 1 + 3) / 4, chunk = dec_attn_chunk_groups(e->opt.kv16);
            a.ts = dec_key_splits((int)RB, e->opt.kv16 || e->opt.mode != MELLOW_PRECISION_F32X3);
            int gs = (ng_end + a.ts - 1) / a.ts;
            if (gs > chunk && gs % chunk <= 4) gs -= gs % chunk;
            gs = gs < 1 ? 1 : gs;
            if (gs != a.gs) e->graphs.reset();
            a.gs = gs;
        }
        a.pq = p + o_pq; a.attF16 = p + o_att; a.att_ml = p + o_aml; a.ssq = p + o_ssq; a.guF = p + o_gu; a.xmidF16 = p + o_xmidF16;
        a.logits = e->dlogits.p; a.cand_val = e->cand.p; a.cand_idx = reinterpret_cast<int32_t*>(e->cand.p + (size_t)Bp * (V / 32));
    }
    if (Bp > 1024) return fail("batch too large for the decode state block");
    return 0;
}

int clear_page_tails(mellow_engine* e, int T, int t_end) {
    const int Tmax = e->kv_Tmax;
    if (t_end > Tmax) t_end = Tmax;
    if (T >= t_end) return 0;
    if (e->kv16_direct) launch_clear_page_slots(e->vcache16.p, (int64_t)e->cfg.num_layers * e->kv_B * 3, Tmax, T, t_end, e->stream, true);
    else launch_clear_page_slots(e->vcache.p, (int64_t)e->cfg.num_layers * e->kv_B * 3, Tmax, T, t_end, e->stream);
    HIPCHK(hipGetLastError());
    return 0;
}

LoopArgs loop_args(mellow_engine* e) {
    LoopArgs lp;
    lp.out_tokens = reinterpret_cast<int32_t*>(e->out_tok.p);
    lp.params = e->d_params; lp.seen_stop = e->d_seen; lp.n_seen = e->d_nseen; lp.arrive = e->d_arrive; lp.ticket = e->d_ticket;
    lp.host_progress = e->d_progress; lp.T0 = e->cfg.prefix_len;
    if (e->da.blk_live) { lp.blk_left = e->d_blk_left; lp.blk_live = e->d_blk_live; lp.blk_snap = e->d_blk_live + 32; }
    if (e->da.row_of_slot) { lp.row_of_slot = e->d_row_of_slot; lp.n_compactions = e->d_ncompact; }
    return lp;
}

int run_lm_head(mellow_engine* e, int B, int pending_kcd, const RecordArgs* rec) {
    const int NT = e->cfg.vocab_size / 32, Bp = e->da.rows;
    auto dh = [&](int k) { DecArgs x = e->da; x.dbg_seq = e->dbg_seq0 >= 0 ? e->dbg_seq0 + 5 * e->cfg.num_layers + k : -1000; return x; };
    { ProfScope ps(e, PF_NORM, 0, (double)(pending_kcd + 2) * Bp * 576 * 4);
      launch_dec_final_norm(dh(0), e->w.final_norm, pending_kcd, e->stream); }
    { ProfScope ps(e, PF_SKINNY, 2.0 * Bp * 576.0 * e->cfg.vocab_size, 576.0 * e->cfg.vocab_size * 4);
      const DecW h = e->w.head_w();
      launch_dec_lm_head(dh(1), h.p, e->w.lm_head.KP / 8, e->cfg.vocab_size, e->stream, h.scale); }
    { ProfScope ps(e, PF_MISC, 0, 0);
      if (e->sample_on) {
          SampleArgs sa;
          sa.logits = e->da.logits; sa.ld = e->cfg.vocab_size; sa.prm = e->d_sparams;
          launch_dec_sample(sa, dh(2), B, e->d_tokens, e->w.embed, (rec && rec->embed_next) ? 1 : 0, rec ? loop_args(e) : LoopArgs(),
                            e->stream);
      } else {
          launch_dec_argmax(dh(2), B, NT, e->d_tokens, e->w.embed, (rec && rec->embed_next) ? 1 : 0, rec ? loop_args(e) : LoopArgs(),
                            e->stream);
      }
      if (rec && e->da.row_of_slot) launch_dec_compact(e->da, B, loop_args(e), e->stream); }
    return 0;
}

int run_prefill(mellow_engine* e, int B, int T, const RecordArgs* rec, bool all_positions) {
    hipStream_t s = e->stream;
    const int M = B * T, Tmax = e->kv_Tmax;
    const int NL = e->cfg.num_layers;
    float *x = e->lm_x.p, *xn = e->lm_xn.p;
    const bool amx = e->opt.fp8 && e->opt.fp8_prefill && e->opt.x3_apb && e->w.fp8_w.count(e->w.layers[0].qkv.p) != 0;
    const bool apb = (e->opt.f32x3_terms && e->opt.x3_apb) || amx;
    if (apb && !e->prof_on && (e->prefill_parts > 1 || e->streams_probed)) CHK(ensure_prefill_streams(e));
    int nh = (apb && !e->prof_on) ? e->prefill_parts : 1;
    nh = nh < 1 ? 1 : (nh > 4 ? 4 : nh);
    if (nh > B) nh = B;
    int hb0[4], hB[4];
    size_t prow[4];
    hipStream_t hs[4] = {s, e->stream2[0], e->stream2[1], e->stream2[2]};
    for (int h = 0, b0 = 0, r = 0; h < nh; ++h) {
        hb0[h] = b0; hB[h] = B / nh + (h < B % nh ? 1 : 0); prow[h] = (size_t)r;
        b0 += hB[h]; r += rup(hB[h] * T, 128);
    }
    const bool split = nh > 1;
    struct Join {
        mellow_engine* e; hipStream_t* hs; int nh; bool done;
        int run() {
            if (done) return 0;
            done = true;
            for (int h = 1; h < nh; ++h) {
                HIPCHK(hipEventRecord(e->ev_join[h - 1], hs[h]));
                HIPCHK(hipStreamWaitEvent(hs[0], e->ev_join[h - 1], 0));
            }
            return 0;
        }
        ~Join() { (void)run(); }
    } join{e, hs, nh, !split};
    if (split) {
        HIPCHK(hipEventRecord(e->ev_fork, s));
        for (int h = 1; h < nh; ++h) HIPCHK(hipStreamWaitEvent(hs[h], e->ev_fork, 0));
    }
    for (int l = 0; l < NL; ++l) {
        const LMLayerW& w = e->w.layers[l];
        bool last = false;
        for (int h = 0; h < nh; ++h) {
            hipStream_t st = hs[h];
            const int64_t r0 = (int64_t)hb0[h] * T;
            const int Mh = hB[h] * T, Bh = hB[h];
            float* xh = x + r0 * 576;
            float* xnh = xn + r0 * 576;
            float* qh = e->lm_q.p + r0 * 576;
            float* oh = e->lm_o.p + r0 * 576;
            float* hh = e->lm_h.p + r0 * 1536;
            const bool p16 = amx && e->kv16_direct;
            float* kc = p16 ? e->kcache16.p + (kv_layer_floats(e) * l + (size_t)hb0[h] * 3 * Tmax * 64) / 2
                            : e->kcache.p + kv_layer_floats(e) * l + (size_t)hb0[h] * 3 * Tmax * 64;
            float* vc = p16 ? e->vcache16.p + (kv_layer_floats(e) * l + (size_t)hb0[h] * 3 * Tmax * 64) / 2
                            : e->vcache.p + kv_layer_floats(e) * l + (size_t)hb0[h] * 3 * Tmax * 64;
            char* xn3 = apb ? reinterpret_cast<char*>(e->lm_xn3.p) + prow[h] * 576 * 6 : nullptr;
            char* o3 = apb ? reinterpret_cast<char*>(e->lm_o3.p) + prow[h] * 576 * 6 : nullptr;
            char* h3 = apb ? reinterpret_cast<char*>(e->lm_h3.p) + prow[h] * 1536 * 6 : nullptr;
            char *xn3s = nullptr, *o3s = nullptr, *h3s = nullptr;
            if (amx) {
                xn3s = xn3 + (size_t)rup(Mh, 128) * 576; o3s = o3 + (size_t)rup(Mh, 128) * 576; h3s = h3 + (size_t)rup(Mh, 128) * 1536;
            }
            auto c3_amx = [&](GemmArgs& g, char* scales, int kt64) { if (amx) { g.c3_fmt = 1; g.C3s = reinterpret_cast<uint8_t*>(scales); g.c3_kt64 = kt64; } };
            const bool fz = apb && e->opt.prefill_fuse_norm && w.gateup_f.p != nullptr;
            float* ssq_in = fz ? e->lm_ssq.p + prow[h] * 9 : nullptr;
            float* ssq_mid = fz ? e->lm_ssq.p + e->lm_ssq.cap / 2 + prow[h] * 9 : nullptr;
            auto with_rs = [&](GemmArgs& g, const float* ssq) { g.rs_ssq = ssq; g.rs_parts = 9; g.rs_dim = 576.f; g.rs_eps = e->cfg.rms_norm_eps; };
            (void)ssq_mid;
            const bool fz_in = fz && l > 0;
            if (fz_in) {}
            else if (apb) { ProfScope ps(e, PF_NORM, 0, 2.5 * Mh * 576 * 4); launch_rmsnorm_apb(xh, xn3, Mh, 576, w.in_ln, e->cfg.rms_norm_eps, st, xn3s); }
            else { ProfScope ps(e, PF_NORM, 0, 2.0 * Mh * 576 * 4); launch_rmsnorm(xh, xnh, Mh, 576, w.in_ln, e->cfg.rms_norm_eps, st); }
            {
                GemmArgs g;
                g.A = xnh; g.lda = 576; g.M = Mh; g.K = 576; g.Wp = fz_in ? w.qkv_f.p : w.qkv.p; g.Nw = 960; g.N = 960; g.epi = EPI_QKV_ROPE;
                if (fz_in) with_rs(g, ssq_in);
                g.q_out = qh; g.k_cache = kc; g.v_cache = vc; g.rope_cos = e->w.rope_cos; g.rope_sin = e->w.rope_sin;
                g.T = T; g.Tmax = Tmax; g.q_heads = 9; g.kv_heads = 3; g.kv16 = p16 ? 1 : 0;
                if (apb) CHK(run_gemm_apb(e, g, xn3, st, xn3s)); else CHK(run_gemm(e, g));
            }
            if (l == NL - 1 && !all_positions) { last = true; continue; }
            {
                ProfScope ps(e, PF_PREFILL_ATTN, 4.0 * 64 * 9 * (double)Bh * ((double)T * (T + 1) / 2), 0);
                const bool attn_f32 = !e->opt.x3_attn;
                launch_prefill_attention(qh, kc, vc, oh, apb ? o3 : nullptr, Bh, T, Tmax, (e->opt.f32x3_terms != 0 || amx) && !attn_f32, st, o3s, amx && e->opt.fp8_attn_bf16, p16);
            }
            {
                GemmArgs g = lin(oh, 576, Mh, w.o, xh, 576, nullptr);
                g.resid = xh; g.ldr = 576;
                if (fz) { g.C3 = xn3; g.ssq_out = ssq_mid; g.ssq_parts = 9; c3_amx(g, xn3s, 9); }
                if (apb) CHK(run_gemm_apb(e, g, o3, st, o3s)); else CHK(run_gemm(e, g));
            }
            if (fz) {}
            else if (apb) { ProfScope ps(e, PF_NORM, 0, 2.5 * Mh * 576 * 4); launch_rmsnorm_apb(xh, xn3, Mh, 576, w.post_ln, e->cfg.rms_norm_eps, st, xn3s); }
            else { ProfScope ps(e, PF_NORM, 0, 2.0 * Mh * 576 * 4); launch_rmsnorm(xh, xnh, Mh, 576, w.post_ln, e->cfg.rms_norm_eps, st); }
            {
                GemmArgs g;
                g.A = xnh; g.lda = 576; g.M = Mh; g.K = 576; g.Wp = fz ? w.gateup_f.p : w.gateup.p; g.Nw = 3072; g.N = 1536; g.C = hh; g.ldc = 1536;
                g.epi = EPI_SWIGLU;
                if (fz) with_rs(g, ssq_mid);
                if (apb) { g.C3 = h3; c3_amx(g, h3s, 24); CHK(run_gemm_apb(e, g, xn3, st, xn3s)); } else CHK(run_gemm(e, g));
            }
            {
                GemmArgs g = lin(hh, 1536, Mh, w.down, xh, 576, nullptr);
                g.resid = xh; g.ldr = 576;
                if (fz) { g.C3 = xn3; g.ssq_out = ssq_in; g.ssq_parts = 9; c3_amx(g, xn3s, 9); }
                if (apb) CHK(run_gemm_apb(e, g, h3, st, h3s)); else CHK(run_gemm(e, g));
            }
        }
        if (last) break;
    }
    CHK(join.run());
    if (e->opt.kv16 && !e->kv16_direct && !all_positions) {
        ProfScope ps(e, PF_MISC, 0, 3.0 * kv_layer_floats(e) * NL * 4);
        launch_kv_to_bf16(e->kcache.p, e->kcache16.p, (int64_t)(kv_layer_floats(e) * NL), s);
        launch_kv_to_bf16(e->vcache.p, e->vcache16.p, (int64_t)(kv_layer_floats(e) * NL), s);
    }
    if (all_positions) {
        HIPCHK(hipGetLastError());
        return 0;
    }
    { ProfScope ps(e, PF_MISC, 0, 0); launch_dec_load_rows(e->da, B, x, 576, nullptr, T, 0, s); }
    e->cur_B = B;
    e->cur_pos = T;
    e->h_pos_word = T - 1;
    HIPCHK(hipMemcpyAsync(e->d_pos, &e->h_pos_word, sizeof(int32_t), hipMemcpyHostToDevice, s));
    CHK(enqueue_decode_layer_range(e, B, NL - 1, NL, false));
    CHK(run_lm_head(e, B, DEC_KC_DOWN, rec));
    HIPCHK(hipGetLastError());
    return 0;
}

int enqueue_decode_layer_range(mellow_engine* e, int B, int l_begin, int l_end, bool inc_pos) {
    hipStream_t s = e->stream;
    const int Bp = e->da.rows;
#ifdef MELLOW_DEVPROBE
    static const bool same_w = getenv("MELLOW_DEV_SAME_WEIGHTS") != nullptr, same_kv = getenv("MELLOW_DEV_SAME_KV") != nullptr;
    static const int skip = getenv("MELLOW_DEV_SKIP") ? atoi(getenv("MELLOW_DEV_SKIP")) : 0;
#else
    constexpr bool same_w = false, same_kv = false;
    constexpr int skip = 0;
#endif
    for (int l = l_begin; l < l_end; ++l) {
        const LMLayerW& w = e->w.layers[same_w ? 0 : l];
        const DecW qkv = w.qkv_w(), o = w.o_w(), gu = w.gateup_w(), dn = w.down_w();
        float* kc = e->opt.kv16 ? e->kcache16.p + kv_layer_floats(e) / 2 * (same_kv ? 0 : l) : e->kcache.p + kv_layer_floats(e) * (same_kv ? 0 : l);
        float* vc = e->opt.kv16 ? e->vcache16.p + kv_layer_floats(e) / 2 * (same_kv ? 0 : l) : e->vcache.p + kv_layer_floats(e) * (same_kv ? 0 : l);
        const int kcd = l == l_begin ? 0 : DEC_KC_DOWN;
        const bool x3l = e->da.xmid3_32 != nullptr;
        const bool fuse_rb = x3l || e->da.RB <= e->opt.dec_fuse_max_rb;
        const bool fused_in = l > l_begin && ((w.qkv2 != nullptr && fuse_rb) || w.q2h8 != nullptr) && !same_w;
        DecArgs a = e->da;
        const int sq = e->dbg_seq0 >= 0 ? e->dbg_seq0 + 5 * (l - l_begin) : -1000;
        auto da = [&](int k) { DecArgs x = e->da; x.dbg_seq = sq + k; return x; };
        a.dbg_seq = sq;
        a.first = l == l_begin ? 1 : 0;
        a.inc_pos = (inc_pos && l == l_begin) ? 1 : 0;
        if (!(skip & 1) && !fused_in)
        { ProfScope ps(e, PF_SKINNY, 2.0 * Bp * 576.0 * 960.0, 576.0 * 960.0 * 4);
          launch_dec_qkv(a, qkv.p, w.qkv_f.KP / 8, kcd, s, qkv.scale); }
        if (!(skip & 2))
        { ProfScope ps(e, PF_DECODE_ATTN, 4.0 * 64 * 9 * (double)B * (e->cur_pos + 1), 2.0 * (double)B * 3 * 64 * 4 * (e->cur_pos + 1));
          launch_dec_attn(da(1), kc, vc, fused_in, s); }
        if (!(skip & 4))
        { ProfScope ps(e, PF_SKINNY, 2.0 * Bp * 576.0 * 576.0, 576.0 * 576.0 * 4);
          launch_dec_oproj(da(2), o.p, s, o.scale); }
        if (!(skip & 8))
        { ProfScope ps(e, PF_SKINNY, 2.0 * Bp * 576.0 * 3072.0, 576.0 * 3072.0 * 4);
          if (x3l && !w.gu8) launch_dec_gateup3(da(3), w.gu16n, s);
          else launch_dec_gateup(da(3), gu.p, s, gu.scale); }
        const LMLayerW* nx = (l + 1 < l_end && !same_w) ? &e->w.layers[l + 1] : nullptr;
        if (nx && ((nx->qkv2 && fuse_rb) || nx->q2h8)) {
            if (!(skip & 16))
            { ProfScope ps(e, PF_SKINNY, 2.0 * Bp * (2112.0 * 960.0 + 1536.0 * 576.0), (2112.0 * 960.0 + 1536.0 * 576.0) * (nx->q2h8 ? 1 : 4));
              if (nx->q2h8) launch_dec_qkv2_w8(da(4), nx->qkv8, nx->qkv_sc, nx->q2h8, nx->q2h_sc, w.dn8, w.dn_sc, s);
              else if (x3l) launch_dec_qkv2x3(da(4), nx->qkv2, w.down.p, s);
              else launch_dec_qkv2(da(4), nx->qkv2, w.down.p, s); }
        } else if (!(skip & 16))
        { ProfScope ps(e, PF_SKINNY, 2.0 * Bp * 576.0 * 1536.0, 576.0 * 1536.0 * 4);
          launch_dec_down(da(4), dn.p, w.down.KP / 8, s, dn.scale); }
    }
    return 0;
}
int enqueue_decode_layers(mellow_engine* e, int B, const RecordArgs* rec) {
    CHK(enqueue_decode_layer_range(e, B, 0, e->cfg.num_layers, true));
    CHK(run_lm_head(e, B, DEC_KC_DOWN, rec));
    return 0;
}

static int capture_steps(mellow_engine* e, int B, const RecordArgs* rec, int n, hipGraphExec_t* exec) {
    hipGraph_t gr = nullptr;
    HIPCHK(hipStreamBeginCapture(e->stream, hipStreamCaptureModeThreadLocal));
    int rc = 0;
    for (int k = 0; k < n && !rc; ++k) rc = enqueue_decode_layers(e, B, rec);
    hipError_t err = hipStreamEndCapture(e->stream, &gr);
    if (!rc && err != hipSuccess) rc = fail("hipStreamEndCapture failed: %s", hipGetErrorString(err));
    if (!rc && (err = hipGraphInstantiate(exec, gr, nullptr, nullptr, 0)) != hipSuccess) { *exec = nullptr; rc = fail("instantiating the captured decode step failed: %s", hipGetErrorString(err)); }
    if (gr) (void)hipGraphDestroy(gr);
    return rc;
}

int encode_pair_to_prefix(mellow_engine* e, const float* a1, const float* a2, int64_t n_samples, const int32_t* ids,
                                 int B, float* prefix_out) {
    mellow_engine::Buf& cat = e->wavcat;
    CHK(ensure(e, cat, (size_t)2 * B * n_samples));
    HIPCHK(hipMemcpyAsync(cat.p, a1, (size_t)B * n_samples * 4, hipMemcpyDeviceToDevice, e->stream));
    HIPCHK(hipMemcpyAsync(cat.p + (size_t)B * n_samples, a2, (size_t)B * n_samples * 4, hipMemcpyDeviceToDevice, e->stream));
    CHK(run_encoder(e, cat.p, 2 * B, n_samples, 0, 1, nullptr));
    { ProfScope ps(e, PF_MISC, 0, 0);
      launch_prefix_assemble(e->proj33.p, e->w.embed, ids, B, e->cfg.text_len, e->cfg.sep_token_id, e->cfg.vocab_size, prefix_out,
                             e->d_progress + 1, e->stream); }
    HIPCHK(hipGetLastError());
    return 0;
}

void clear_bad_id(mellow_engine* e) { __atomic_store_n(e->h_progress + 1, 0ull, __ATOMIC_RELEASE); }

int check_bad_id(mellow_engine* e) {
    const unsigned long long w = __atomic_load_n(e->h_progress + 1, __ATOMIC_ACQUIRE);
    if (!w) return 0;
    return fail("index out of range in self: prompt id %d of example %u is outside the vocabulary [0, %d)", (int)(unsigned)(w & 0xffffffffu),
                (unsigned)((w >> 32) & 0x7fffffffu), e->cfg.vocab_size);
}

static int wait_ticket(mellow_engine* e, unsigned want, unsigned* nseen) {
    const auto t0 = std::chrono::steady_clock::now();
    for (unsigned spins = 1;; ++spins) {
        const unsigned long long v = __atomic_load_n(e->h_progress, __ATOMIC_ACQUIRE);
        if ((unsigned)(v >> 32) >= want) {
            if (nseen) *nseen = (unsigned)(v & 0xffffffffu);
            return 0;
        }
        if ((spins & 0x3ff) == 0) {
            const hipError_t q = hipStreamQuery(e->stream);
            if (q == hipSuccess) {
                const unsigned long long v2 = __atomic_load_n(e->h_progress, __ATOMIC_ACQUIRE);
                if ((unsigned)(v2 >> 32) >= want) continue;
                return fail("decode progress word stalled at ticket %u (wanted %u) with an idle stream", (unsigned)(v2 >> 32), want);
            }
            if (q != hipErrorNotReady) return fail("stream error while waiting for a decode step: %s", hipGetErrorString(q));
            if (std::chrono::steady_clock::now() - t0 > std::chrono::seconds(60))
                return fail("timed out waiting for decode ticket %u", want);
        }
#if defined(__x86_64__) || defined(__i386__)
        __builtin_ia32_pause();
#elif defined(__aarch64__)
        __asm__ __volatile__("yield");
#endif
        if (spins > 4096) std::this_thread::yield();
    }
}

static void clear_bad_target(mellow_engine* e) { __atomic_store_n(e->h_progress + 2, 0ull, __ATOMIC_RELEASE); }
static int check_bad_target(mellow_engine* e, const char* what, int lo) {
    const unsigned long long w = __atomic_load_n(e->h_progress + 2, __ATOMIC_ACQUIRE);
    if (!w) return 0;
    return fail("index out of range in self: %s id %d of row %u is outside [%d, %d)", what, (int)(unsigned)(w & 0xffffffffu),
                (unsigned)((w >> 32) & 0x7fffffffu), lo, e->cfg.vocab_size);
}

int run_score_head(mellow_engine* e, int B, int T, int from_pos, int n, const int32_t* targets, float* out_logprob,
                   int32_t* out_argmax, float* out_lse, float* out_max) {
    hipStream_t s = e->stream;
    const int V = e->cfg.vocab_size, rows = B * n, groups = V / 64;
    if (V % 64 != 0 || e->w.lm_head.Nw != V) return fail("the scoring head tiles the vocabulary in groups of 64 columns (vocab %d)", V);
    const size_t ld = (size_t)rup(rows, 64);
    CHK(ensure(e, e->sc_part, (size_t)groups * ld * 3));
    float2* part_ms = reinterpret_cast<float2*>(e->sc_part.p);
    int32_t* part_arg = reinterpret_cast<int32_t*>(e->sc_part.p + (size_t)groups * ld * 2);
    float* tgt_logit = e->sc_ws.p;
    GemmArgs g = lin(e->lm_xn.p, 576, rows, e->w.lm_head, nullptr, 0, nullptr);
    g.epi = EPI_LSE;
    g.lse_target = targets; g.lse_ms = part_ms; g.lse_arg = part_arg; g.lse_tgt = tgt_logit; g.lse_ld = (int64_t)ld;
    ProfScope ps(e, PF_LM_HEAD, gemm_flops(g), 576.0 * V * 4 + (double)rows * 576 * 4 + 3.0 * rows * groups * 12);
    launch_gather_span(e->lm_x.p, B, T, from_pos, n, e->lm_o.p, s);
    launch_rmsnorm(e->lm_o.p, e->lm_xn.p, rows, 576, e->w.final_norm, e->cfg.rms_norm_eps, s);
    launch_gemm(g, s);
    launch_lse_merge(part_ms, part_arg, (int64_t)ld, groups, rows, targets, tgt_logit, V, out_logprob, out_argmax, out_lse, out_max,
                     e->d_progress + 2, s);
    HIPCHK(hipGetLastError());
    return 0;
}

extern "C" {

int mellow_prefix(mellow_engine_t* e, const float* audio1, const float* audio2, int64_t n_samples, const int32_t* input_ids,
                  int B, float* out) {
    if (!e || !e->finalized) return fail("engine not finalized");
    if (!audio1 || !audio2 || !input_ids || !out) return fail("null argument");
    if (B <= 0) return fail("B must be positive");
    HIPCHK(hipSetDevice(e->device));
    clear_bad_id(e);
    CHK(encode_pair_to_prefix(e, audio1, audio2, n_samples, input_ids, B, out));
    HIPCHK(hipStreamSynchronize(e->stream));
    return check_bad_id(e);
}

int mellow_lm_prefill(mellow_engine_t* e, const float* prefix, int B, int T, int reserve, float* logits) {
    if (!e || !e->finalized) return fail("engine not finalized");
    if (!prefix || B <= 0 || T <= 0 || reserve < 0) return fail("bad argument");
    HIPCHK(hipSetDevice(e->device));
    CHK(ensure_lm(e, B, T, T + reserve + 1));
    HIPCHK(hipMemcpyAsync(e->lm_x.p, prefix, (size_t)B * T * 576 * 4, hipMemcpyDeviceToDevice, e->stream));
    CHK(clear_page_tails(e, T, e->kv_Tmax));
    CHK(run_prefill(e, B, T, nullptr));
    if (logits)
        HIPCHK(hipMemcpyAsync(logits, e->dlogits.p, (size_t)B * e->cfg.vocab_size * 4, hipMemcpyDeviceToDevice, e->stream));
    HIPCHK(hipStreamSynchronize(e->stream));
    return 0;
}

int mellow_lm_decode_step(mellow_engine_t* e, const int32_t* token_ids, float* logits) {
    if (!e || !e->finalized) return fail("engine not finalized");
    if (!token_ids) return fail("null argument");
    if (e->cur_B <= 0) return fail("decode step without a prefill");
    if (e->cur_pos + 1 > e->kv_Tmax) return fail("KV pages exhausted (reserve too small)");
    HIPCHK(hipSetDevice(e->device));
    const int B = e->cur_B;
    launch_dec_load_rows(e->da, B, e->w.embed, 576, token_ids, 0, e->cfg.vocab_size, e->stream);
    CHK(enqueue_decode_layers(e, B, nullptr));
    e->cur_pos += 1;
    if (logits)
        HIPCHK(hipMemcpyAsync(logits, e->dlogits.p, (size_t)B * e->cfg.vocab_size * 4, hipMemcpyDeviceToDevice, e->stream));
    HIPCHK(hipGetLastError());
    HIPCHK(hipStreamSynchronize(e->stream));
    return 0;
}

int mellow_debug_dec_head(mellow_engine_t* e, const float* x, int B, int act_fp8, float* logits) {
    if (!e || !e->finalized) return fail("engine not finalized");
    if (!x || !logits || B <= 0 || B > 1024) return fail("bad argument");
    if (e->cfg.hidden_size != 576) return fail("the decode kernels are built for hidden size 576");
    HIPCHK(hipSetDevice(e->device));
    CHK(ensure_lm(e, B, 1, 2));
    DecArgs a = e->da;
    a.blk_live = nullptr; a.row_of_slot = nullptr;
    a.a8 = (act_fp8 && e->w.head8) ? 1 : 0;
    a.xnF = a.xmidF;
    a.xn3 = nullptr;
    launch_dec_load_rows(a, B, x, 576, nullptr, 1, 0, e->stream);
    const DecW h = e->w.head_w();
    launch_dec_lm_head(a, h.p, e->w.lm_head.KP / 8, e->cfg.vocab_size, e->stream, h.scale);
    HIPCHK(hipMemcpyAsync(logits, e->dlogits.p, (size_t)B * e->cfg.vocab_size * 4, hipMemcpyDeviceToDevice, e->stream));
    HIPCHK(hipGetLastError());
    HIPCHK(hipStreamSynchronize(e->stream));
    e->cur_B = 0;
    return 0;
}

int mellow_embed_tokens(mellow_engine_t* e, const int32_t* token_ids, int n, float* out) {
    if (!e || !e->finalized) return fail("engine not finalized");
    if (!token_ids || !out || n <= 0) return fail("bad argument");
    HIPCHK(hipSetDevice(e->device));
    launch_gather_rows(e->w.embed, 576, token_ids, n, e->cfg.vocab_size, out, e->stream);
    HIPCHK(hipGetLastError());
    HIPCHK(hipStreamSynchronize(e->stream));
    return 0;
}

int mellow_lm_forward_logits(mellow_engine_t* e, const float* embeds, int B, int T, int from_pos, float* logits) {
    if (!e || !e->finalized) return fail("engine not finalized");
    if (!embeds || !logits || B <= 0 || T <= 0 || from_pos < 0 || from_pos >= T) return fail("bad argument");
    HIPCHK(hipSetDevice(e->device));
    hipStream_t s = e->stream;
    CHK(ensure_lm(e, B, T, T + 1));
    HIPCHK(hipMemcpyAsync(e->lm_x.p, embeds, (size_t)B * T * 576 * 4, hipMemcpyDeviceToDevice, s));
    CHK(run_prefill(e, B, T, nullptr, true));
    e->cur_B = 0;
    const int n = T - from_pos;
    GemmArgs g = lin(e->lm_xn.p, 576, B * n, e->w.lm_head, logits, e->cfg.vocab_size, nullptr);
    { ProfScope ps(e, PF_LM_HEAD, gemm_flops(g), (576.0 + (double)B * n) * e->cfg.vocab_size * 4 + (double)B * n * 576 * 4);
      launch_gather_span(e->lm_x.p, B, T, from_pos, n, e->lm_o.p, s);
      launch_rmsnorm(e->lm_o.p, e->lm_xn.p, B * n, 576, e->w.final_norm, e->cfg.rms_norm_eps, s);
      launch_gemm(g, s); }
    HIPCHK(hipGetLastError());
    HIPCHK(hipStreamSynchronize(s));
    return 0;
}

int mellow_lm_score(mellow_engine_t* e, const float* embeds, int B, int T, int from_pos, const int32_t* targets,
                    float* out_logprob, int32_t* out_argmax, float* out_lse, float* out_max) {
    if (!e || !e->finalized) return fail("engine not finalized");
    if (!embeds || !targets || !out_logprob || B <= 0 || T <= 0 || from_pos < 0 || from_pos >= T) return fail("bad argument");
    HIPCHK(hipSetDevice(e->device));
    hipStream_t s = e->stream;
    CHK(ensure_lm(e, B, T, T + 1));
    CHK(ensure(e, e->sc_ws, (size_t)B * (T - from_pos)));
    clear_bad_target(e);
    HIPCHK(hipMemcpyAsync(e->lm_x.p, embeds, (size_t)B * T * 576 * 4, hipMemcpyDeviceToDevice, s));
    CHK(run_prefill(e, B, T, nullptr, true));
    e->cur_B = 0;
    CHK(run_score_head(e, B, T, from_pos, T - from_pos, targets, out_logprob, out_argmax, out_lse, out_max));
    HIPCHK(hipStreamSynchronize(s));
    return check_bad_target(e, "target", -1);
}

int mellow_score(mellow_engine_t* e, const float* audio1, const float* audio2, int64_t n_samples, const int32_t* input_ids, int B,
                 const int32_t* cand_ids, const int32_t* cand_len, int K, int L, float* out_logprob, float* out_sum,
                 int32_t* out_argmax) {
    if (!e || !e->finalized) return fail("engine not finalized");
    if (!audio1 || !audio2 || !input_ids || !cand_ids || !cand_len || !out_logprob || !out_sum) return fail("null argument");
    if (B <= 0 || K <= 0 || L <= 0) return fail("B, K and L must be positive");
    if (B > 1024) return fail("mellow_score takes at most 1024 examples per call (got %d)", B);
// ... 151 lines not shown
                         int ignore_stop, int32_t* out_tokens, int32_t* out_len, int32_t* out_steps, float* first_token_ms,
                         const SampleCall& sc) {
    const auto t_entry = std::chrono::steady_clock::now();
    HIPCHK(hipSetDevice(e->device));
    hipStream_t s = e->stream;
    const int T = e->cfg.prefix_len;
    int Tmax = rup(T + max_len, 64);
    if (Tmax > e->cfg.max_positions) Tmax = T + max_len;
    CHK(ensure_lm(e, B, T, Tmax, T + max_len));
    const int Bp = e->da.rows;
    CHK(ensure(e, e->out_tok, (size_t)Bp * max_len));
    HIPCHK(hipEventRecord(e->ev_phase[0], s));
    __atomic_store_n(e->h_progress, 0ull, __ATOMIC_RELEASE);
    clear_bad_id(e);
    HIPCHK(hipMemsetAsync(e->d_nseen, 0, 3 * sizeof(int32_t), s));
    HIPCHK(hipMemsetAsync(e->d_seen, 0, 1024 * sizeof(int32_t), s));
    e->h_params[0] = max_len;
    e->h_params[1] = stop_id;
    HIPCHK(hipMemcpyAsync(e->d_params, e->h_params, 2 * sizeof(int32_t), hipMemcpyHostToDevice, s));
    e->da.logits = nullptr;
    e->sample_on = sc.on;
    struct SampleOff { mellow_engine* e; ~SampleOff() { e->sample_on = false; } } sample_off{e};
    if (sc.on) {
        e->da.logits = e->dlogits.p;
        stage_sampling(e, sc.top_p, sc.temperature, sc.seed, sc.row_offset, 0);
        HIPCHK(hipMemcpyAsync(e->d_sparams, e->h_sparams, sizeof(e->h_sparams), hipMemcpyHostToDevice, s));
    }
    e->da.blk_live = (!ignore_stop && e->da.RB > 1) ? e->d_blk_live : nullptr;
    e->da.blk_snap = e->d_blk_live + 32;
#ifdef MELLOW_DEVPROBE
    static const bool dev_dead = getenv("MELLOW_DEV_DEAD_BLOCKS") != nullptr;
#else
    constexpr bool dev_dead = false;
#endif
    const bool no_migrate = !e->opt.row_migration;
    e->da.row_of_slot = nullptr;
    if (dev_dead) {
        e->da.blk_live = e->d_blk_live;
        HIPCHK(hipMemsetAsync(e->d_blk_left, 0, 96 * sizeof(int32_t), s));
    } else if (e->da.blk_live) {
        if (!no_migrate && B <= 1024) {
            std::vector<int32_t> ident(1024);
            for (int i = 0; i < 1024; ++i) ident[i] = i < B ? i : -1;
            e->h_ident = ident;
            HIPCHK(hipMemcpyAsync(e->d_row_of_slot, e->h_ident.data(), 1024 * sizeof(int32_t), hipMemcpyHostToDevice, s));
            HIPCHK(hipMemsetAsync(e->d_ncompact, 0, sizeof(int32_t), s));
            e->da.row_of_slot = e->d_row_of_slot;
        }
        for (int rb = 0; rb < 32; ++rb) {
            const int left = B - 32 * rb;
            e->h_blk[rb] = left <= 0 ? 0 : (left > 32 ? 32 : left);
            e->h_blk[32 + rb] = left > 0 ? 1 : 0;
        }
        HIPCHK(hipMemcpyAsync(e->d_blk_left, e->h_blk, 64 * sizeof(int32_t), hipMemcpyHostToDevice, s));
        HIPCHK(hipMemsetAsync(e->out_tok.p, 0xff, (size_t)Bp * max_len * sizeof(int32_t), s));
    }
    CHK(clear_page_tails(e, T, e->kv_Tmax));
    CHK(encode_pair_to_prefix(e, audio1, audio2, n_samples, input_ids, B, e->lm_x.p));
    HIPCHK(hipEventRecord(e->ev_phase[1], s));
    RecordArgs rec;
    rec.embed_next = true;
    CHK(run_prefill(e, B, T, &rec));
    HIPCHK(hipEventRecord(e->ev_phase[2], s));

    const bool graph = e->use_graph && !e->prof_on && max_len > 1;
    const mellow_engine::StepGraphs::Key want{B, e->kv_Tmax, (int)sc.on, e->out_tok.p, e->da.blk_live, e->da.row_of_slot};
    if (graph && (!e->graphs.one || !(e->graphs.key == want))) {
        e->graphs.reset();
        int rc = capture_steps(e, B, &rec, 1, &e->graphs.one);
        if (!rc) rc = capture_steps(e, B, &rec, 8, &e->graphs.eight);
        if (rc) { e->graphs.reset(); return rc; }
        e->graphs.key = want;
    }
    int steps_done = 1;
    double first_ms = -1.0;
    auto note_first = [&]() {
        if (first_ms < 0) first_ms = std::chrono::duration<double, std::milli>(std::chrono::steady_clock::now() - t_entry).count();
    };
    if (ignore_stop) {
        for (int i = 1; i < max_len;) {
            const bool eight = graph && i + 8 <= max_len;
            if (eight) HIPCHK(hipGraphLaunch(e->graphs.eight, s));
            else if (graph) HIPCHK(hipGraphLaunch(e->graphs.one, s));
            else CHK(enqueue_decode_layers(e, B, &rec));
            i += eight ? 8 : 1;
            e->cur_pos += eight ? 8 : 1;
            steps_done = i;
        }
        CHK(wait_ticket(e, 1, nullptr));
        note_first();
    } else {
        for (int i = 1; i < max_len; ++i) {
            if (graph) HIPCHK(hipGraphLaunch(e->graphs.one, s));
            else CHK(enqueue_decode_layers(e, B, &rec));
            e->cur_pos += 1;
            steps_done = i + 1;
            unsigned nseen = 0;
            CHK(wait_ticket(e, (unsigned)i, &nseen));
            note_first();
            if ((int)nseen >= B) break;
        }
        if (first_ms < 0) { CHK(wait_ticket(e, 1, nullptr)); note_first(); }
    }
    HIPCHK(hipEventRecord(e->ev_phase[3], s));
    HIPCHK(hipGetLastError());
    std::vector<int32_t> toks((size_t)B * max_len);
    HIPCHK(hipMemcpyAsync(out_tokens, e->out_tok.p, toks.size() * sizeof(int32_t), hipMemcpyDefault, s));
    HIPCHK(hipMemcpyAsync(toks.data(), e->out_tok.p, toks.size() * sizeof(int32_t), hipMemcpyDeviceToHost, s));
    HIPCHK(hipStreamSynchronize(s));
    CHK(check_bad_id(e));
    for (int i = 0; i < 3; ++i) HIPCHK(hipEventElapsedTime(&e->phase_ms[i], e->ev_phase[i], e->ev_phase[i + 1]));
    if (first_token_ms) *first_token_ms = (float)first_ms;
    int ref_steps = steps_done;
    if (!ignore_stop) {
        std::vector<char> seen(B, 0);
        int nseen = 0;
        for (int st = 0; st < steps_done; ++st) {
            for (int b = 0; b < B; ++b)
                if (!seen[b] && toks[(size_t)b * max_len + st] == stop_id) { seen[b] = 1; ++nseen; }
            if (nseen == B) { ref_steps = st + 1; break; }
        }
    }
    e->last_steps_enqueued = steps_done;
    e->cur_B = 0;
    e->last_compactions = 0;
    if (e->da.row_of_slot) HIPCHK(hipMemcpy(&e->last_compactions, e->d_ncompact, sizeof(int32_t), hipMemcpyDeviceToHost));
    if (out_steps) *out_steps = ref_steps;
    if (out_len)
        for (int b = 0; b < B; ++b) {
            int n = ref_steps;
            for (int st = 0; st < ref_steps; ++st)
                if (toks[(size_t)b * max_len + st] == stop_id) { n = st; break; }
            out_len[b] = n;
        }
    return 0;
}

}
```

### mellow_amd/csrc/engine_weights.cpp

```cpp
#include "engine_internal.h"

static const HostTensor* get(mellow_engine* e, const std::string& k) {
    auto it = e->host.find(k);
    return it == e->host.end() ? nullptr : &it->second;
}
static int expect_shape(const HostTensor* t, const std::string& k, std::initializer_list<int64_t> shp) {
    if (!t) return fail("missing key in state_dict: %s", k.c_str());
    if (t->dtype != MELLOW_F32) return fail("%s: expected float32", k.c_str());
    if (t->shape.size() != shp.size())
        return fail("size mismatch for %s: rank %d in the checkpoint, %d expected", k.c_str(), (int)t->shape.size(), (int)shp.size());
    size_t i = 0;
    for (auto d : shp) {
        if (t->shape[i] != d)
            return fail("size mismatch for %s: dimension %d is %lld in the checkpoint, %lld expected", k.c_str(), (int)i,
                        (long long)t->shape[i], (long long)d);
        ++i;
    }
    return 0;
}
static int up_vec(mellow_engine* e, const std::string& k, int64_t n, float** out, int64_t pad_to = 0) {
    const HostTensor* t = get(e, k);
    CHK(expect_shape(t, k, {n}));
    return upload(e, out, t->f(), (size_t)n, (size_t)pad_to);
}
// ... 269 lines not shown
        CHK(pack_key(e, p + "self_attn.o_proj.weight", H, 576, &w.o));
        const HostTensor *g = get(e, p + "mlp.gate_proj.weight"), *u = get(e, p + "mlp.up_proj.weight");
        CHK(expect_shape(g, p + "mlp.gate_proj.weight", {I, H}));
        CHK(expect_shape(u, p + "mlp.up_proj.weight", {I, H}));
        CHK(make_packed(e, g->f(), u->f(), I, H, &w.gateup));
        CHK(pack_key(e, p + "mlp.down_proj.weight", H, I, &w.down));
        CHK(up_vec(e, p + "input_layernorm.weight", H, &w.in_ln));
        CHK(up_vec(e, p + "post_attention_layernorm.weight", H, &w.post_ln));
        {
            const HostTensor *l1 = get(e, p + "input_layernorm.weight"), *l2 = get(e, p + "post_attention_layernorm.weight");
            std::vector<float> f(qkv);
            for (int n = 0; n < 960; ++n)
                for (int kk = 0; kk < H; ++kk) f[(size_t)n * H + kk] = qkv[(size_t)n * H + kk] * l1->f()[kk];
            e->decode_only_weight = true;
            CHK(make_packed(e, f.data(), nullptr, 960, H, &w.qkv_f));
            e->decode_only_weight = false;
            if (e->opt.prefill_fuse_norm) { CHK(make_pb(e, w.qkv_f)); CHK(make_w8(e, w.qkv_f)); }
            if (fuse && l > 0) {
                const std::string kd = L + "model.layers." + std::to_string(l - 1) + ".mlp.down_proj.weight";
                CHK(expect_shape(get(e, kd), kd, {H, I}));
                HIPCHK(hipMemcpyAsync(cmpF.p, f.data(), (size_t)960 * 576 * 4, hipMemcpyHostToDevice, e->stream));
                HIPCHK(hipMemcpyAsync(cmpD.p, get(e, kd)->f(), (size_t)576 * 1536 * 4, hipMemcpyHostToDevice, e->stream));
                launch_compose_f64(cmpF.p, cmpD.p, cmpQ.p, 960, 1536, 576, e->stream);
                if (e->opt.fp8_decode) {
                    launch_pack_weight(cmpQ.p, 960, 1536, 1536, cmpCat.p, 1024, 1536, e->stream);
                    HIPCHK(hipGetLastError());
                    CHK(make_dec_fp8(e, cmpCat.p, 32, (1536 / 8) * 64, 32, &w.q2h8, &w.q2h_sc));
                } else {
                    HIPCHK(hipMemcpy2DAsync(cmpCat.p, (size_t)2112 * 4, cmpF.p, (size_t)576 * 4, (size_t)576 * 4, 960, hipMemcpyDeviceToDevice, e->stream));
                    HIPCHK(hipMemcpy2DAsync(cmpCat.p + 576, (size_t)2112 * 4, cmpQ.p, (size_t)1536 * 4, (size_t)1536 * 4, 960, hipMemcpyDeviceToDevice, e->stream));
                    CHK(dev_alloc(e, &w.qkv2, (size_t)1024 * 2112));
                    launch_pack_weight(cmpCat.p, 960, 2112, 2112, w.qkv2, 1024, 2112, e->stream);
                    HIPCHK(hipGetLastError());
                    HIPCHK(hipStreamSynchronize(e->stream));
                }
            }
            std::vector<float> gf((size_t)I * H), uf((size_t)I * H);
            for (int n = 0; n < I; ++n)
                for (int kk = 0; kk < H; ++kk) {
                    gf[(size_t)n * H + kk] = g->f()[(size_t)n * H + kk] * l2->f()[kk];
                    uf[(size_t)n * H + kk] = u->f()[(size_t)n * H + kk] * l2->f()[kk];
                }
            if (e->opt.prefill_fuse_norm && (e->opt.f32x3_terms || (e->opt.fp8 && e->opt.fp8_prefill))) {
                e->decode_only_weight = true;
                CHK(make_packed(e, gf.data(), uf.data(), I, H, &w.gateup_f));
                e->decode_only_weight = false;
                CHK(make_pb(e, w.gateup_f));
                CHK(make_w8(e, w.gateup_f));
            }
            {
                std::vector<float> il((size_t)2 * I * H);
                for (int t = 0; t < I / 8; ++t) {
                    memcpy(il.data() + (size_t)(2 * t) * 8 * H, gf.data() + (size_t)t * 8 * H, (size_t)8 * H * 4);
                    memcpy(il.data() + (size_t)(2 * t + 1) * 8 * H, uf.data() + (size_t)t * 8 * H, (size_t)8 * H * 4);
                }
                CHK(make_packed16(e, il.data(), 2 * I, H, &w.gu16));
                if (e->opt.f32x3_terms && fuse && !e->opt.fp8_decode) CHK(make_packed16(e, il.data(), 2 * I, H, &w.gu16n, true));
            }
            CHK(make_packed16(e, get(e, p + "self_attn.o_proj.weight")->f(), H, 576, &w.o16));
        }
        if (e->opt.fp8_decode) {
            CHK(make_dec_fp8(e, w.qkv_f.p, w.qkv_f.NP / 32, (w.qkv_f.KP / 8) * 64, 32, &w.qkv8, &w.qkv_sc));
            CHK(make_dec_fp8(e, w.o16, H / 16, (576 / 16) * 64, 16, &w.o8, &w.o_sc));
            CHK(make_dec_fp8(e, w.gu16, 2 * I / 16, (H / 16) * 64, 16, &w.gu8, &w.gu_sc));
            CHK(make_dec_fp8(e, w.down.p, w.down.NP / 32, (w.down.KP / 8) * 64, 32, &w.dn8, &w.dn_sc));
        }
        e->w.layers.push_back(w);
    }
    CHK(up_vec(e, L + "model.norm.weight", H, &e->w.final_norm));
    {
        const int P = e->cfg.max_positions;
        const HostTensor *tc = get(e, "mellow.rope_cos"), *ts = get(e, "mellow.rope_sin");
        std::vector<float> c((size_t)P * 32), s((size_t)P * 32);
        if (tc && ts && tc->numel() == (int64_t)P * 32 && ts->numel() == (int64_t)P * 32) {
            memcpy(c.data(), tc->f(), c.size() * 4);
            memcpy(s.data(), ts->f(), s.size() * 4);
        } else {
            rope_tables_host(e->cfg.rope_theta, 64, P, c.data(), s.data());
        }
        CHK(upload(e, &e->w.rope_cos, c.data(), c.size()));
        CHK(upload(e, &e->w.rope_sin, s.data(), s.size()));
    }
    CHK(alloc_state_words(e));
    e->host.clear();
    e->finalized = true;
    return 0;
}
```

### mellow_amd/csrc/kernels.h

```cpp
#pragma once
#include <hip/hip_runtime.h>
#include <stdint.h>

namespace mellow {

void launch_pack_weight(const float* w, int N, int K, int64_t ldw, float* out, int NP, int KP, hipStream_t s);
void launch_pack_weight_pairs(const float* w0, const float* w1, int N, int K, int64_t ldw, float* out, int NP,
                              int KP, hipStream_t s);

enum { ACT_NONE = 0, ACT_GELU = 1, ACT_SIGMOID = 2 };
enum { EPI_LINEAR = 0, EPI_POWER = 1, EPI_LOGMEL = 2, EPI_SWIGLU = 3, EPI_QKV_ROPE = 4, EPI_LSE = 5 };
enum { A_PLAIN = 0, A_FRAMES = 1 };

struct GemmArgs {
    const float* A = nullptr;
    int64_t lda = 0;
    int M = 0;
    int K = 0;
    int a_mode = A_PLAIN;
    int fpc = 1;
    int64_t clip_stride = 0;
    int hop = 0;
    const float* Wp = nullptr;
    int Nw = 0;
// ... 36 lines not shown
    uint8_t* C3s = nullptr;
    int c3_kt64 = 0;
    const int32_t* lse_target = nullptr;
    float2* lse_ms = nullptr;
    int32_t* lse_arg = nullptr;
    float* lse_tgt = nullptr;
    int64_t lse_ld = 0;
};
void launch_gemm(const GemmArgs& a, hipStream_t s);
void launch_quant_mx8(const float* A, int64_t lda, int M, int K, void* img, void* sc, hipStream_t s);
void launch_pack_fp8(const float* Wp, int NP, int KP, uint8_t* W8, float* w_scale, hipStream_t s);
void launch_gemm_fp8(const GemmArgs& a, hipStream_t s);
void launch_pack_bf16x3(const float* Wp, int NP, int KP, void* PB, hipStream_t s);
void launch_gemm_bf16x3_fused(const GemmArgs& a, hipStream_t s);
void launch_split_rows_apb(const float* A, int64_t lda, int M, int K, void* out, hipStream_t s);
void launch_gemm_bf16x3_apb(const GemmArgs& a, hipStream_t s);
double gemm_flops(const GemmArgs& a);

void set_max_dynamic_lds(const void* fn, size_t bytes);

constexpr int DEC_KC_QKV = 8;
#ifndef MELLOW_DEC_KC_DOWN
#define MELLOW_DEC_KC_DOWN 8
#endif
constexpr int DEC_KC_DOWN = MELLOW_DEC_KC_DOWN;
#ifndef MELLOW_DEC_TS
#define MELLOW_DEC_TS 2
#endif
constexpr int DEC_TS = MELLOW_DEC_TS;
#ifndef MELLOW_DEC_TS_MULTI
#define MELLOW_DEC_TS_MULTI 1
#endif
constexpr int DEC_TS_MULTI = MELLOW_DEC_TS_MULTI;
inline int dec_key_splits(int RB, bool fixed) { return RB <= 1 || fixed ? DEC_TS : DEC_TS_MULTI; }
#ifndef MELLOW_Q2_HC
#define MELLOW_Q2_HC 4
#endif
#ifndef MELLOW_Q2_WAVES
#define MELLOW_Q2_WAVES 12
#else
#define MELLOW_Q2_WAVES_FORCED 1
#endif
constexpr int Q2_HC = MELLOW_Q2_HC, Q2_WAVES = MELLOW_Q2_WAVES;
constexpr int Q2_NPQ = 2 + Q2_HC;
constexpr int Q2_K8 = 72 + 192;
constexpr int Q2_BLOCKS = 60 + 48 * Q2_HC;
static_assert(Q2_NPQ <= DEC_KC_QKV && Q2_HC <= DEC_KC_DOWN, "the fused kernel reuses the slab buffers of the split-K kernels");
enum { DEC_X3_HEAD = 1, DEC_X3_GATEUP = 2, DEC_X3_QKV = 4, DEC_X3_ALL = 7 };
struct DecArgs {
    int rows = 0, RB = 0;
    int Tmax = 0;
    float eps = 1e-5f;
    int32_t* d_pos = nullptr;
    int first = 0;
    int inc_pos = 0;
    int gs = 1;
    int ts = DEC_TS;
    float* rope_cur = nullptr;
    float* ssq1 = nullptr;
    const float* rope_cos = nullptr;
    const float* rope_sin = nullptr;
    float* xmidF = nullptr;
    float* xnewR = nullptr;
    float* dslabF = nullptr;
    int64_t slabF_stride4 = 0;
    float* pq = nullptr;
    float* attF16 = nullptr;
    float* att_ml = nullptr;
    float* ssq = nullptr;
    float* xmidF16 = nullptr;
    float* guF = nullptr;
    float* xnF = nullptr;
    void *xmid3_32 = nullptr, *xmid3_16 = nullptr, *h3 = nullptr;
    void* xn3 = nullptr;
    const int32_t* blk_live = nullptr;
    int32_t* blk_snap = nullptr;
    const int32_t* row_of_slot = nullptr;
    int kv16 = 0;
    int a8 = 0;
    int x3 = 0;
    int dbg_seq = -1;
    float* logits = nullptr;
    float* cand_val = nullptr; int32_t* cand_idx = nullptr;
};
void launch_dec_qkv(const DecArgs& a, const float* Wp_folded, int K8p, int kcd, hipStream_t s, const float* wscale = nullptr);
void launch_pack_dec_fp8(const float* Wp, int tiles, int slots_per_tile, int rows_per_tile, void* out, float* scale, hipStream_t s);
void launch_dec_attn(const DecArgs& a, float* k_cache, float* v_cache, bool fused, hipStream_t s);
void launch_kv_to_bf16(const float* src, void* dst, int64_t n, hipStream_t s);
void launch_dec_qkv2(const DecArgs& a, const float* Wq2, const float* Wd, hipStream_t s);
void launch_dec_qkv2x3(const DecArgs& a, const float* Wq2, const float* Wd, hipStream_t s);
void dec_prepare_lds_attributes();
void launch_dec_gateup3(const DecArgs& a, const float* Wp16n_folded_pairs, hipStream_t s);
void launch_dec_qkv2_w8(const DecArgs& a, const float* Wx8, const float* sc_x, const float* Wh8, const float* sc_h,
                        const float* Wd8, const float* sc_d, hipStream_t s);
void launch_compose_f64(const float* A, const float* B, float* C, int M, int N, int K, hipStream_t s);
int dec_attn_chunk_groups(bool kv16);
void launch_dec_oproj(const DecArgs& a, const float* Wp16, hipStream_t s, const float* wscale = nullptr);
void launch_dec_gateup(const DecArgs& a, const float* Wp16_folded_pairs, hipStream_t s, const float* wscale = nullptr);
void launch_dec_down(const DecArgs& a, const float* Wp, int K8p, hipStream_t s, const float* wscale = nullptr);
void launch_dec_final_norm(const DecArgs& a, const float* norm_w, int kcd, hipStream_t s);
bool dec_head3r_fits(int vocab);
void launch_dec_lm_head(const DecArgs& a, const float* Wp, int K8p, int vocab, hipStream_t s, const float* wscale = nullptr);
struct LoopArgs {
    int32_t* out_tokens = nullptr;
    const int32_t* params = nullptr;
    int32_t* seen_stop = nullptr;
    int32_t* n_seen = nullptr;
    int32_t* arrive = nullptr;
    int32_t* ticket = nullptr;
    int32_t* blk_left = nullptr;
    int32_t* blk_live = nullptr;
    const int32_t* blk_snap = nullptr;
    int32_t* row_of_slot = nullptr;
    int32_t* n_compactions = nullptr;
    unsigned long long* host_progress = nullptr;
    int T0 = 0;
};
void launch_dec_argmax(const DecArgs& a, int B, int n_tiles, int32_t* tokens, const float* embed, int write_x,
                       const LoopArgs& loop, hipStream_t s);
enum { SMP_SEED_LO = 0, SMP_SEED_HI, SMP_ROW_OFF, SMP_TOP_P, SMP_TEMP, SMP_STEP, SMP_WORDS = 8 };
struct SampleArgs {
    const float* logits = nullptr;
    int64_t ld = 0;
    const uint32_t* prm = nullptr;
    const int32_t* row_ids = nullptr;
};
constexpr int SAMPLE_MAX_V = 49152;
void launch_dec_sample(const SampleArgs& sa, const DecArgs& a, int B, int32_t* tokens, const float* embed, int write_x,
                       const LoopArgs& loop, hipStream_t s);
void launch_sample_logits(const SampleArgs& sa, int B, int32_t* tokens, hipStream_t s);
void launch_dec_compact(const DecArgs& a, int B, const LoopArgs& loop, hipStream_t s);
void launch_dec_load_rows(const DecArgs& a, int B, const float* in, int64_t ld, const int32_t* row_ids, int T_last,
                          int n_src , hipStream_t s);
void launch_pack_weight16(const float* w, int N, int K, float* out, hipStream_t s);
void launch_pack_weight16n(const float* w, int N, int K, float* out, hipStream_t s);
void set_kernel_debug_buffer(uint64_t* p);
void set_gemm_debug_buffer(uint64_t* p);

void launch_resample(const float* x, int n_clips, int64_t n_in, const float* wT, int orig, int nw, int klen, int width,
                     float* out, int64_t n_out, hipStream_t s);
void launch_reflect_pad(const float* wav, int n_clips, int64_t n_samples, float* out, int64_t padded_len, int pad,
                        hipStream_t s);
void launch_fold_patch_embed(const float* logmel_bn, int n_src, int src_frames, int n_crops, int crop_hop,
                             int crop_len, const float* conv_w, const float* conv_b, const float* ln_w,
                             const float* ln_b, float* x0, hipStream_t s);

void launch_layernorm(const float* in, float* out, int M, int C, const float* w, const float* b,
                      const int32_t* row_map, int ntok, hipStream_t s);
void launch_merge_layernorm(const float* in, float* out, int n, int R, int C, const float* w, const float* b,
                            hipStream_t s);
void launch_stft_fft_power(const float* wpad, int fpc, int64_t clip_stride, int hop, int M, const float* win, const float* tw1,
                           const float* tw2, float* power, hipStream_t s);
void launch_rmsnorm(const float* in, float* out, int M, int C, const float* w, float eps, hipStream_t s);
void launch_layernorm_apb(const float* in, void* out_apb, int M, int C, const float* w, const float* b, const int32_t* row_map,
                          int ntok, hipStream_t s, void* out_scales = nullptr);
void launch_rmsnorm_apb(const float* in, void* out_apb, int M, int C, const float* w, float eps, hipStream_t s, void* out_scales = nullptr);

void launch_window_attention(const float* qkv, float* out, int M, int C, int nH, const float* bias_exp,
                             const float* mask, int nW, hipStream_t s, void* out_apb = nullptr, bool qkv16 = false);

void launch_tail_latent_im2col(const float* y, int n, float* latent, int64_t latent_stride, float* a_ts,
                               hipStream_t s);
void launch_crop_average(const float* in, int n, int n_crops, int64_t len, int64_t in_stride, float* out,
                         int64_t out_stride, hipStream_t s);
void launch_gelu(const float* in, float* out, int64_t n, hipStream_t s);
void launch_prefix_assemble(const float* proj33, const float* embed, const int32_t* ids, int B, int text_len,
                            int sep_id, int vocab, float* prefix, unsigned long long* bad_id_word, hipStream_t s);
void launch_gather_rows(const float* table, int width, const int32_t* ids, int n, int n_rows, float* out, hipStream_t s);
void launch_gather_span(const float* in, int B, int T, int from_pos, int n, float* out, hipStream_t s);
void launch_clear_page_slots(float* cache, int64_t pages, int Tmax, int t0, int t1, hipStream_t s, bool pages16 = false);
void launch_downsample33(const float* proj33, int n, float* out, hipStream_t s);

void launch_prefill_attention(const float* q, const float* k_cache, const float* v_cache, float* o, void* o_apb, int B, int T,
                              int Tmax, bool x3, hipStream_t s, void* o_scales = nullptr, bool bf16_once = false, bool pages16 = false);
void launch_lse_merge(const float2* part_ms, const int32_t* part_arg, int64_t ld, int groups, int rows, const int32_t* targets,
                      const float* tgt_logit, int vocab, float* out_logprob, int32_t* out_argmax, float* out_lse, float* out_max,
                      unsigned long long* bad_word, hipStream_t s);
void launch_score_build_input(const float* prefix, const float* embed, const int32_t* cand_ids, const int32_t* cand_len, int K,
                              int L, int P, int vocab, int row0, int nr, float* x, int32_t* targets, unsigned long long* bad_word,
                              hipStream_t s);
void launch_score_sum(const float* logprob, const int32_t* cand_len, int rows, int L, float* out_sum, hipStream_t s);
void launch_argmax(const float* logits, int B, int V, int64_t ld, int32_t* tokens, hipStream_t s);

}
```

### mellow_amd/csrc/sample.hip

```cpp
#include "common.h"
#include "kernels.h"

namespace mellow {

namespace {

constexpr int SMP_THREADS = 1024, SMP_WAVES = SMP_THREADS / 64;
constexpr int SMP_NV4 = SAMPLE_MAX_V / 4 / SMP_THREADS;
static_assert(SMP_NV4 * 4 * SMP_THREADS == SAMPLE_MAX_V, "row tiling");

__device__ __forceinline__ int64_t f32_idx(int rb, int K8, int m, int k) {
    return ((int64_t)rb * K8 + (k >> 3)) * 64 + m + 32 * ((k >> 2) & 1);
}

__device__ __forceinline__ uint32_t okey(float z) {
    const uint32_t u = __float_as_uint(z);
    return (u & 0x80000000u) ? ~u : (u | 0x80000000u);
}

__device__ __forceinline__ float opaque(float x) {
    asm volatile("" : "+v"(x));
    return x;
}

// ... 120 lines not shown
    if (nan_idx != 0x7fffffff) return nan_idx;
    m = block_reduce(m, [](float a, float b) { return fmaxf(a, b); }, red_f);

    auto q_of = [&](int k, int j) -> unsigned long long {
        const float zz = opaque(z[k][j]);
        const float e = zz == m ? 1.0f : expf(zz - m);
        return __float2uint_rn(e * 2147483648.0f);
    };
    bool keep_all = !(top_p < 1.0f);
    uint32_t kstar = 0;
    int idx_cut = 0x7fffffff;
    if (!keep_all) {
        unsigned long long above, mass, thr;
        keep_all = !radix_select([&](int k, int j, uint32_t& key) { key = okey(opaque(z[k][j])); return true; }, q_of,
                                 [&](unsigned long long S) { return top_p > 0.0f ? (unsigned long long)((double)top_p * (double)S) : 0ull; },
                                 24, sh, kstar, above, mass, thr);
        if (!keep_all) {
#pragma unroll
            for (int k = 0; k < SMP_NV4; ++k)
#pragma unroll
                for (int j = 0; j < 4; ++j)
                    if (okey(opaque(z[k][j])) == kstar) qtie_s = (uint32_t)q_of(k, j);
            __syncthreads();
            const unsigned long long qt = qtie_s;
            const unsigned long long n_tie = mass / qt, c = (thr - above) / qt + 1;
            if (c < n_tie) {
                uint32_t kidx;
                unsigned long long a2, m2, t2;
                radix_select([&](int k, int j, uint32_t& key) {
                                 key = 0xFFFFu - (uint32_t)(4 * (k * SMP_THREADS + tid) + j);
                                 return okey(opaque(z[k][j])) == kstar; },
                             [](int, int) { return 1ull; }, [c](unsigned long long) { return c - 1; }, 8, sh, kidx, a2, m2, t2);
                idx_cut = (int)(0xFFFFu - kidx);
            }
        }
    }

    float best = -INFINITY;
    int bidx = 0x7fffffff;
#pragma unroll
    for (int k = 0; k < SMP_NV4; ++k) {
        const int i4 = k * SMP_THREADS + tid;
        bool kept[4], any = false;
#pragma unroll
        for (int j = 0; j < 4; ++j) {
            const uint32_t key = okey(opaque(z[k][j]));
            kept[j] = (keep_all || key > kstar || (key == kstar && 4 * i4 + j <= idx_cut));
            any |= kept[j];
        }
        if (any) {
            uint32_t x[4];
            philox4x32_10((uint32_t)i4, step, grow, 0u, seed_lo, seed_hi, x);
#pragma unroll
            for (int j = 0; j < 4; ++j)
                if (kept[j]) {
                    const float u = (float)(2u * (x[j] >> 9) + 1u) * 0x1p-24f;
                    const float s = z[k][j] - logf(-logf(u));
                    const int id = 4 * i4 + j;
                    if (s > best || (s == best && id < bidx)) { best = s; bidx = id; }
                }
        }
    }
#pragma unroll
    for (int off = 32; off > 0; off >>= 1) {
        const float ob = __shfl_xor(best, off, 64);
        const int oi = __shfl_xor(bidx, off, 64);
        if (ob > best || (ob == best && oi < bidx)) { best = ob; bidx = oi; }
    }
    if ((tid & 63) == 0) { red_f[tid >> 6] = best; red_i[tid >> 6] = bidx; }
    __syncthreads();
    best = red_f[0]; bidx = red_i[0];
    for (int w = 1; w < SMP_WAVES; ++w)
        if (red_f[w] > best || (red_f[w] == best && red_i[w] < bidx)) { best = red_f[w]; bidx = red_i[w]; }
    __syncthreads();
    return min(max(bidx, 0), SAMPLE_MAX_V - 1);
}

}

__global__ __launch_bounds__(SMP_THREADS) void dec_sample_kernel(const SampleArgs sa, const DecArgs a, int32_t* __restrict__ tokens,
                                                                 const float* __restrict__ embed, int write_x, const LoopArgs lp) {
    __shared__ int tok_s;
    const int b = blockIdx.x, tid = threadIdx.x;
    const int row = lp.row_of_slot ? lp.row_of_slot[b] : b;
    const bool dead = (lp.blk_snap && lp.blk_snap[b >> 5] == 0) || row < 0;
    int idx = 0;
    if (!dead) {
        const int step = lp.out_tokens ? *a.d_pos - lp.T0 + 1 : (int)sa.prm[SMP_STEP];
        idx = sample_row(sa.logits + (int64_t)b * sa.ld, sa.prm, sa.prm[SMP_ROW_OFF] + (uint32_t)row, (uint32_t)step);
    }
    if (tid == 0) {
        if (!dead) {
            tokens[b] = idx;
            tok_s = idx;
        }
        if (lp.out_tokens) {
            if (!dead) {
                const int max_len = lp.params[0], stop_id = lp.params[1];
                const int step = *a.d_pos - lp.T0 + 1;
                if (step >= 0 && step < max_len) lp.out_tokens[(int64_t)row * max_len + step] = idx;
                if (idx == stop_id && lp.seen_stop[row] == 0) {
                    lp.seen_stop[row] = 1;
                    atomicAdd(lp.n_seen, 1);
                    if (lp.blk_left && atomicSub(lp.blk_left + (b >> 5), 1) == 1) lp.blk_live[b >> 5] = 0;
                }
            }
            asm volatile("s_waitcnt vmcnt(0)" ::: "memory");
            if (atomicAdd(lp.arrive, 1) == (int)gridDim.x - 1) {
                *lp.arrive = 0;
                const int t = *lp.ticket + 1;
                *lp.ticket = t;
                const int ns = atomicAdd(lp.n_seen, 0);
                __hip_atomic_store(lp.host_progress, ((unsigned long long)(unsigned)t << 32) | (unsigned)ns, __ATOMIC_RELAXED,
                                   __HIP_MEMORY_SCOPE_SYSTEM);
            }
        }
    }
    if (dead) return;
    if (write_x) {
        __syncthreads();
        if (tid < 144) {
            const float4 e = reinterpret_cast<const float4*>(embed + (int64_t)tok_s * 576)[tid];
            reinterpret_cast<float4*>(a.xmidF)[f32_idx(b >> 5, 72, b & 31, tid * 4)] = e;
        }
    }
}

__global__ __launch_bounds__(SMP_THREADS) void sample_logits_kernel(const SampleArgs sa, int32_t* __restrict__ tokens) {
    const int b = blockIdx.x;
    const uint32_t grow = sa.prm[SMP_ROW_OFF] + (uint32_t)(sa.row_ids ? sa.row_ids[b] : b);
    const int idx = sample_row(sa.logits + (int64_t)b * sa.ld, sa.prm, grow, sa.prm[SMP_STEP]);
    if (threadIdx.x == 0) tokens[b] = idx;
}

void launch_dec_sample(const SampleArgs& sa, const DecArgs& a, int B, int32_t* tokens, const float* embed, int write_x,
                       const LoopArgs& loop, hipStream_t s) {
    hipLaunchKernelGGL(dec_sample_kernel, dim3(B), dim3(SMP_THREADS), 0, s, sa, a, tokens, embed, write_x, loop);
}

void launch_sample_logits(const SampleArgs& sa, int B, int32_t* tokens, hipStream_t s) {
    hipLaunchKernelGGL(sample_logits_kernel, dim3(B), dim3(SMP_THREADS), 0, s, sa, tokens);
}

}
```

Baseline: 462.5.

## Precompute layer-0 QKV per vocab token and fold final norm into lm_head

At finalize time the engine builds a table holding the layer-0 QKV projection (and its sum of squares) for every vocabulary token's embedding. During decode, the first layer's attention kernel looks up the current token's row instead of running the layer-0 QKV GEMM. That kernel also takes over the position increment and the rope update. A second path, used when a head_norm flag is set, fuses the final RMSNorm into the lm_head kernel. The cost is vocab×960 floats of extra memory, an extra position-tracking word, and token bookkeeping in the compact kernel.

```diff
diff --git a/mellow_amd/csrc/decode.hip b/mellow_amd/csrc/decode.hip
--- a/mellow_amd/csrc/decode.hip
+++ b/mellow_amd/csrc/decode.hip
@@ -315,7 +315,7 @@
     if constexpr (KV16) reinterpret_cast<__bf16*>(page)[elem] = static_cast<__bf16>(v);
     else page[elem] = v;
 }
-template <bool BLK, bool FUSED, bool ONE, bool KV16, int NW, int TS>
+template <bool BLK, bool FUSED, bool ONE, bool KV16, int NW, int TS, bool TAB = false>
 __global__ __launch_bounds__(NW * 64, ONE ? 2 : (KV16 && MELLOW_DA16_MFMA && DA_MINW > 1 ? MELLOW_DA16_MINW : DA_MINW)) void dec_attn_kernel(float* __restrict__ k_cache, float* __restrict__ v_cache,
                                                                   const int32_t* __restrict__ d_pos_p, const float* __restrict__ pq_p,
                                                                   const float* __restrict__ xmidF_p, int Tmax_p, int gs_p, int rows_p,
@@ -336,7 +336,15 @@
     auto mf_group = [&](int g0, int u) { return g0 + u * DA_WAVES; };
 
     static_assert(TS == DEC_TS || !(ONE || KV16), "one row block and the bf16 pages always run DEC_TS key splits (kernels.h dec_key_splits)");
+    static_assert(!TAB || (!FUSED && !KV16), "the table serves the first layer of a step on fp32 pages");
     const int g = blockIdx.x, b = blockIdx.y, sp = blockIdx.z;
+    if (TAB && g == 0 && b == 0 && sp == 0 && threadIdx.x < 32) {
+        const int p = *d_pos_p + a.inc_pos;
+        const float c0 = a.rope_cos[(int64_t)p * 32 + threadIdx.x], s0 = a.rope_sin[(int64_t)p * 32 + threadIdx.x];
+        a.rope_cur[threadIdx.x] = c0;
+        a.rope_cur[32 + threadIdx.x] = s0;
+        if (threadIdx.x == 0) *a.d_pos = p;
+    }
     int row = b;
     if (BLK) {
         const int live = a.blk_live[b >> 5];
@@ -354,21 +362,23 @@
 #ifdef MELLOW_POS_VECTOR_LOAD
     const int pos = __builtin_amdgcn_readfirstlane(*reinterpret_cast<const volatile int*>(d_pos_p));
 #else
-    const int pos = *d_pos_p;
+    const int pos = TAB ? *d_pos_p + a.inc_pos : *d_pos_p;
 #endif
     const int hsel = (tid >> 5) & 3, i = tid & 31;
     const int r = tid < 80 ? tid : 0;
     const int pcol = r < 48 ? (3 * g + (r >> 4)) * 64 + 4 * (r & 15) : r < 64 ? 576 + g * 64 + 4 * (r - 48) : 768 + g * 64 + 4 * (r - 64);
-    const float* prow = pq_p + (int64_t)b * 960 + pcol;
-    constexpr int NPQ = FUSED ? Q2_NPQ : DEC_KC_QKV;
+    const int tok = TAB ? min(max(a.tok0[b], 0), a.q0_vocab - 1) : 0;
+    const float* prow = TAB ? a.q0 + (int64_t)tok * 960 + pcol : pq_p + (int64_t)b * 960 + pcol;
+    const float* sqrow = TAB ? a.q0ssq + (int64_t)tok * DEC_KC_QKV : a.ssq1 + (int64_t)b * DEC_KC_QKV;
+    constexpr int NPQ = TAB ? 1 : FUSED ? Q2_NPQ : DEC_KC_QKV;
     float4 sl4[NPQ], sq4[2];
     if (tid < 80) {
 #pragma unroll
         for (int s = 0; s < NPQ; ++s)
             sl4[s] = (MELLOW_DA_ABL & 4) ? make_float4(0.1f * s, 0.2f, 0.3f, 0.4f) : *reinterpret_cast<const float4*>(prow + (int64_t)s * rows_p * 960);
         if (!FUSED) {
-            sq4[0] = reinterpret_cast<const float4*>(a.ssq1 + (int64_t)b * DEC_KC_QKV)[0];
-            sq4[1] = reinterpret_cast<const float4*>(a.ssq1 + (int64_t)b * DEC_KC_QKV)[1];
+            sq4[0] = reinterpret_cast<const float4*>(sqrow)[0];
+            sq4[1] = reinterpret_cast<const float4*>(sqrow)[1];
         }
     }
     float4 xr4 = make_float4(0.f, 0.f, 0.f, 0.f), xd4[FUSED ? Q2_HC : 1];
@@ -378,7 +388,9 @@
 #pragma unroll
         for (int s = 0; s < Q2_HC; ++s) xd4[s] = reinterpret_cast<const float4*>(a.dslabF)[(int64_t)s * a.slabF_stride4 + fi];
     }
-    const float c = a.rope_cur[i], sn = a.rope_cur[32 + i];
+    if (TAB && g == 0 && sp == 0 && tid < 144)
+        xr4 = reinterpret_cast<const float4*>(xmidF_p)[((int64_t)(b >> 5) * 72 + (tid >> 1)) * 64 + (b & 31) + 32 * (tid & 1)];
+    const float c = TAB ? a.rope_cos[(int64_t)pos * 32 + i] : a.rope_cur[i], sn = TAB ? a.rope_sin[(int64_t)pos * 32 + i] : a.rope_cur[32 + i];
     const int gbeg = sp * gs_p;
     const int gend_fixed = sp == TS - 1 ? 0x3fffffff : gbeg + gs_p;
     typedef unsigned u32x2 __attribute__((ext_vector_type(2)));
@@ -446,11 +458,12 @@
     } else if (tid < 80) {
         float4 x = sl4[0];
 #pragma unroll
-        for (int s = 1; s < DEC_KC_QKV; ++s) x = f4add(x, sl4[s]);
+        for (int s = 1; s < NPQ; ++s) x = f4add(x, sl4[s]);
         const float ssum = ((sq4[0].x + sq4[0].y) + (sq4[0].z + sq4[0].w)) + ((sq4[1].x + sq4[1].y) + (sq4[1].z + sq4[1].w));
         const float rscale = 1.0f / sqrtf(ssum / 576.0f + a.eps);
         *reinterpret_cast<float4*>(xs + 4 * tid) = make_float4(x.x * rscale, x.y * rscale, x.z * rscale, x.w * rscale);
     }
+    if (TAB && g == 0 && sp == 0 && tid < 144) reinterpret_cast<float4*>(a.xnewR + (int64_t)b * 576)[tid] = xr4;
     __syncthreads();
     kstamp(1, 2, dbg);
     const float rs2 = FUSED ? 1.0f / sqrtf(((ssq_part[0] + ssq_part[1]) + ssq_part[2]) / 576.0f + a.eps) : 1.0f;
@@ -986,10 +999,12 @@
 #define MELLOW_H3R_D4 1
 #endif
 constexpr int H3_NW = MELLOW_H3_NW, H3_CP = 3, H3_NC = 36 / H3_CP;
-template <int G, int D, bool BLK>
+template <int G, int D, bool BLK, bool NORM = false>
 __global__ __launch_bounds__(H3_NW * 64) void dec_head3r_kernel(const float* __restrict__ Wp, const i32x4* __restrict__ X3, int K8p, int N,
-                                                                int RB_p, const DecArgs a) {
+                                                                int RB_p, const DecArgs a, const float* __restrict__ norm_w) {
     kspan(a.dbg_seq, 0);
+    static_assert(!NORM || (G == 1 && !BLK && H3_NW == 8 && DEC_KC_DOWN >= 1), "the in-head norm is written for one row block and 512 threads");
+    __shared__ float rinv_s[NORM ? 32 : 1];
     extern __shared__ __attribute__((aligned(16))) i32x4 xs[];
     constexpr int PPH = 36 / G, NCH = PPH / H3_CP;
     constexpr int STAGE = G * PPH * 3 * 64;
@@ -1011,7 +1026,49 @@
             for (int i = 0; i < 2 * H3_CP; ++i) wn[d][i] = ldg_nt(wbase + (d * 2 * H3_CP + i) * 64);
         for (int ph = 0; ph < G; ++ph) {
             if (ph || rb0) __syncthreads();
-            {
+            if constexpr (NORM) {
+                const int m = lane & 31, hq = lane >> 5;
+                float4 x[9], nw[9];
+#pragma unroll
+                for (int j = 0; j < 9; ++j) nw[j] = reinterpret_cast<const float4*>(norm_w)[2 * (wave + 8 * j) + hq];
+#pragma unroll
+                for (int j0 = 0; j0 < 9; j0 += 3) {
+                    float4 sl[3][DEC_KC_DOWN];
+#pragma unroll
+                    for (int jj = 0; jj < 3; ++jj) {
+                        x[j0 + jj] = reinterpret_cast<const float4*>(a.xmidF)[tid + (j0 + jj) * 512];
+#pragma unroll
+                        for (int sk = 0; sk < DEC_KC_DOWN; ++sk)
+                            sl[jj][sk] = reinterpret_cast<const float4*>(a.dslabF)[(int64_t)sk * a.slabF_stride4 + tid + (j0 + jj) * 512];
+                    }
+#pragma unroll
+                    for (int jj = 0; jj < 3; ++jj)
+#pragma unroll
+                        for (int sk = 0; sk < DEC_KC_DOWN; ++sk) x[j0 + jj] = f4add(x[j0 + jj], sl[jj][sk]);
+                }
+                float* ssl = reinterpret_cast<float*>(xs);
+#pragma unroll
+                for (int j = 0; j < 9; ++j) ssl[m * 192 + 2 * (wave + 8 * j) + hq] = f4ssq(x[j]);
+                __syncthreads();
+                for (int row = wave; row < 32; row += 8) {
+                    const float p0 = wave_sum(ssl[row * 192 + lane]), p1 = wave_sum(ssl[row * 192 + 64 + lane]);
+                    const float p2 = wave_sum(lane < 16 ? ssl[row * 192 + 128 + lane] : 0.f);
+                    if (lane == 0) rinv_s[row] = 1.0f / sqrtf((p0 + p1 + p2) / 576.0f + a.eps);
+                }
+                __syncthreads();
+                const float r = rinv_s[m];
+#pragma unroll
+                for (int j = 0; j < 9; ++j) {
+                    const int k8 = wave + 8 * j;
+                    float4 y;
+                    y.x = __fmul_rn(nw[j].x, __fmul_rn(x[j].x, r)); y.y = __fmul_rn(nw[j].y, __fmul_rn(x[j].y, r));
+                    y.z = __fmul_rn(nw[j].z, __fmul_rn(x[j].z, r)); y.w = __fmul_rn(nw[j].w, __fmul_rn(x[j].w, r));
+                    asm volatile("" : "+v"(y.x), "+v"(y.y), "+v"(y.z), "+v"(y.w));
+                    const F3Quad q = f3_split4(y);
+                    uint2* half = reinterpret_cast<uint2*>(xs) + ((int64_t)((k8 >> 1) * 3) * 64 + m + 32 * (k8 & 1)) * 2 + hq;
+                    half[0] = q.p[0]; half[128] = q.p[1]; half[256] = q.p[2];
+                }
+            } else {
                 constexpr int FILL = (STAGE + H3_NW * 64 - 1) / (H3_NW * 64);
                 i32x4 t[FILL];
 #pragma unroll
@@ -1697,6 +1754,7 @@
     __shared__ int bi[4];
     __shared__ int tok_s;
     const int b = blockIdx.x, tid = threadIdx.x;
+    if (b == 0 && tid == 0 && a.d_pos_done) *a.d_pos_done = *a.d_pos;
     const int row = lp.row_of_slot ? lp.row_of_slot[b] : b;
     const bool dead = (lp.blk_snap && lp.blk_snap[b >> 5] == 0) || row < 0;
     float best = -INFINITY;
@@ -1757,7 +1815,7 @@
     kspan(a.dbg_seq, 1);
 }
 
-__global__ __launch_bounds__(1024) void dec_compact_kernel(const DecArgs a, int B, const LoopArgs lp) {
+__global__ __launch_bounds__(1024) void dec_compact_kernel(const DecArgs a, int B, const LoopArgs lp, int32_t* __restrict__ tokens) {
     __shared__ int src_of[1024];
     __shared__ int row_new[1024];
     __shared__ int wsum[16];
@@ -1792,6 +1850,9 @@
     if ((n_act + 31) / 32 >= n_live_s) return;
     if (active) { src_of[base + before] = tid; row_new[base + before] = row; }
     __syncthreads();
+    const int tok_mv = tokens && tid < n_act ? tokens[src_of[tid]] : 0;
+    __syncthreads();
+    if (tokens && tid < n_act) tokens[tid] = tok_mv;
     float4* x = reinterpret_cast<float4*>(a.xmidF);
     for (int d0 = 0; d0 < n_act; d0 += 7) {
         const int d = d0 + tid / 144, c = tid % 144;
@@ -1824,8 +1885,8 @@
     const int blocks = (int)((n8 + 255) / 256 < 8192 ? (n8 + 255) / 256 : 8192);
     hipLaunchKernelGGL(kv_to_bf16_kernel, dim3(blocks), dim3(256), 0, s, reinterpret_cast<const float4*>(src), reinterpret_cast<uint4*>(dst), n8);
 }
-void launch_dec_compact(const DecArgs& a, int B, const LoopArgs& loop, hipStream_t s) {
-    hipLaunchKernelGGL(dec_compact_kernel, dim3(1), dim3(1024), 0, s, a, B, loop);
+void launch_dec_compact(const DecArgs& a, int B, const LoopArgs& loop, hipStream_t s, int32_t* tokens) {
+    hipLaunchKernelGGL(dec_compact_kernel, dim3(1), dim3(1024), 0, s, a, B, loop, tokens);
 }
 
 __global__ __launch_bounds__(192) void dec_load_rows_kernel(const DecArgs a, const float* __restrict__ in, int64_t ld,
@@ -1869,21 +1930,48 @@
                            (const float*)a.dslabF, K8p, a, wscale);
     }); }); });
 }
-void launch_dec_attn(const DecArgs& a, float* k_cache, float* v_cache, bool fused, hipStream_t s) {
+__global__ __launch_bounds__(256) void dec_qkv0_sum_kernel(const float* __restrict__ pq, const float* __restrict__ ssq1, int rows, int id0,
+                                                           float* __restrict__ q0, float* __restrict__ q0ssq) {
+    const int r = blockIdx.x, tid = threadIdx.x;
+    if (tid < 240) {
+        const float* prow = pq + (int64_t)r * 960 + 4 * tid;
+        float4 x = *reinterpret_cast<const float4*>(prow);
+#pragma unroll
+        for (int s = 1; s < DEC_KC_QKV; ++s) x = f4add(x, *reinterpret_cast<const float4*>(prow + (int64_t)s * rows * 960));
+        reinterpret_cast<float4*>(q0 + (int64_t)(id0 + r) * 960)[tid] = x;
+    } else if (tid < 240 + DEC_KC_QKV) {
+        q0ssq[(int64_t)(id0 + r) * DEC_KC_QKV + tid - 240] = ssq1[(int64_t)r * DEC_KC_QKV + tid - 240];
+    }
+}
+void launch_dec_qkv0_table(const DecArgs& a, const float* Wp, int K8p, const float* embed, int vocab, int id0, int n, float* q0,
+                           float* q0ssq, hipStream_t s) {
+    if (n <= 0 || n > a.rows || id0 < 0 || id0 + n > vocab || a.RB * 32 != a.rows) { fprintf(stderr, "mellow: bad layer-0 table block\n"); abort(); }
+    hipLaunchKernelGGL(dec_load_rows_kernel, dim3(n), dim3(192), 0, s, a, embed + (int64_t)id0 * 576, (int64_t)576, (const int32_t*)nullptr, 1, vocab);
+    hipLaunchKernelGGL((dec_qkv_kernel<0, false, false, 0>), dim3(30, DEC_KC_QKV, a.RB), dim3(QKV_THREADS), 0, s, Wp, (const float*)a.xmidF,
+                       (const float*)a.dslabF, K8p, a, (const float*)nullptr);
+    hipLaunchKernelGGL(dec_qkv0_sum_kernel, dim3(n), dim3(256), 0, s, (const float*)a.pq, (const float*)a.ssq1, a.rows, id0, q0, q0ssq);
+}
+void launch_dec_attn(const DecArgs& a, float* k_cache, float* v_cache, bool fused, hipStream_t s, bool table) {
     const dim3 grid(3, a.rows, a.ts);
+    if (table && (fused || a.kv16 || !a.q0 || !a.q0ssq || !a.tok0 || !a.d_pos_done)) {
+        fprintf(stderr, "mellow: layer-0 table attention launched without its table / on a fused or bf16-page layer\n");
+        abort();
+    }
     const bool one = a.RB == 1 && !a.blk_live;
     if (a.ts != DEC_TS && (one || a.kv16 || a.ts != DEC_TS_MULTI)) {
         fprintf(stderr, "mellow: decode attention launched with %d key splits at RB = %d\n", a.ts, a.RB);
         abort();
     }
-    auto launch = [&](auto blk, auto one_c) { with_bool(fused, [&](auto fused_c) { with_bool(a.kv16 != 0, [&](auto kv16) {
-        constexpr bool ONE = one_c.value, KV16 = kv16.value;
+    auto launch = [&](auto blk, auto one_c) { with_int<2, 1, 0>(table ? 2 : fused ? 1 : 0, [&](auto src) { with_bool(a.kv16 != 0, [&](auto kv16) {
+        constexpr bool ONE = one_c.value, KV16 = kv16.value, TAB = src.value == 2, FUSED = src.value == 1;
+        if constexpr (!(TAB && KV16)) {
         constexpr int NW = !KV16 ? DA_WAVES : MELLOW_DA16_MFMA && DA_WAVES == 8 && !ONE ? MELLOW_DA16_NW : DA_WAVES;
         constexpr int TSM = ONE || KV16 ? DEC_TS : DEC_TS_MULTI;
         with_int<DEC_TS, TSM>(a.ts, [&](auto ts) {
-            hipLaunchKernelGGL((dec_attn_kernel<blk.value, fused_c.value, ONE, KV16, NW, ts.value>), grid, dim3(NW * 64), 0, s, k_cache, v_cache,
-                               (const int32_t*)a.d_pos, (const float*)a.pq, (const float*)a.xmidF, a.Tmax, a.gs, a.rows, a);
+            hipLaunchKernelGGL((dec_attn_kernel<blk.value, FUSED, ONE, KV16, NW, ts.value, TAB>), grid, dim3(NW * 64), 0, s, k_cache, v_cache,
+                               (const int32_t*)(TAB ? a.d_pos_done : a.d_pos), (const float*)a.pq, (const float*)a.xmidF, a.Tmax, a.gs, a.rows, a);
         });
+        }
     }); }); };
     if (one) launch(std::false_type{}, std::true_type{});
     else with_bool(a.blk_live != nullptr, [&](auto blk) { launch(blk, std::false_type{}); });
@@ -1918,6 +2006,7 @@
         f(&dec_head3r_kernel<G, D, b.value>, dec_head3r_lds());
     }); });
 }
+constexpr auto dec_head3r_norm_kernel = &dec_head3r_kernel<1, MELLOW_H3R_D1, false, true>;
 void launch_dec_qkv2x3(const DecArgs& a, const float* Wq2, const float* Wd, hipStream_t s) {
     const float* Wh = Wq2 + (size_t)72 * 64 * 4;
     const i32x4 *x3 = reinterpret_cast<const i32x4*>(a.xmid3_32), *h3 = reinterpret_cast<const i32x4*>(a.h3);
@@ -1990,12 +2079,22 @@
     }); });
 }
 bool dec_head3r_fits(int vocab) { return vocab % 32 == 0 && (vocab / 32) % H3_NW == 0; }
-void launch_dec_lm_head(const DecArgs& a, const float* Wp, int K8p, int vocab, hipStream_t s, const float* wscale) {
+bool dec_head_norm_fits(const DecArgs& a, int vocab) {
+    return a.head_norm && (a.x3 & DEC_X3_HEAD) && a.xn3 && a.RB == 1 && !a.blk_live && dec_head3r_fits(vocab);
+}
+void launch_dec_lm_head(const DecArgs& a, const float* Wp, int K8p, int vocab, hipStream_t s, const float* wscale, const float* norm_w) {
+    if (norm_w) {
+        if (wscale || !dec_head_norm_fits(a, vocab)) { fprintf(stderr, "mellow: lm_head asked to normalise in a form that cannot\n"); abort(); }
+        set_max_dynamic_lds(reinterpret_cast<const void*>(dec_head3r_norm_kernel), dec_head3r_lds());
+        hipLaunchKernelGGL(dec_head3r_norm_kernel, dim3(vocab / 32 / H3_NW), dim3(H3_NW * 64), dec_head3r_lds(), s, Wp, (const i32x4*)nullptr, K8p,
+                           vocab, a.RB, a, norm_w);
+        return;
+    }
     if ((a.x3 & DEC_X3_HEAD) && !wscale && a.xn3 && (vocab / 32) % H3_NW == 0) {
         const i32x4* X3 = reinterpret_cast<const i32x4*>(a.xn3);
         with_head3r(a.RB, a.blk_live != nullptr, [&](auto* kernel, size_t lds) {
             set_max_dynamic_lds(reinterpret_cast<const void*>(kernel), lds);
-            hipLaunchKernelGGL(kernel, dim3(vocab / 32 / H3_NW), dim3(H3_NW * 64), lds, s, Wp, X3, K8p, vocab, a.RB, a);
+            hipLaunchKernelGGL(kernel, dim3(vocab / 32 / H3_NW), dim3(H3_NW * 64), lds, s, Wp, X3, K8p, vocab, a.RB, a, (const float*)nullptr);
         });
         return;
     }
@@ -2006,6 +2105,7 @@
 }
 void dec_prepare_lds_attributes() {
     const auto raise = [](auto* kernel, size_t lds) { set_max_dynamic_lds(reinterpret_cast<const void*>(kernel), lds); };
+    raise(dec_head3r_norm_kernel, dec_head3r_lds());
     for (const int rb : {1, 2, 4})
         for (const bool blk : {false, true}) {
             with_head3r(rb, blk, raise);
diff --git a/mellow_amd/csrc/engine.cpp b/mellow_amd/csrc/engine.cpp
--- a/mellow_amd/csrc/engine.cpp
+++ b/mellow_amd/csrc/engine.cpp
@@ -289,6 +289,7 @@
     e->d_seen = e->d_tokens + 2048;
     e->d_row_of_slot = e->d_tokens + 3072;
     e->d_ncompact = e->d_tokens + 1029;
+    e->d_pos_done = e->d_tokens + 1030;
     HIPCHK(hipHostMalloc(reinterpret_cast<void**>(&e->h_progress), 64, hipHostMallocMapped | hipHostMallocCoherent));
     *e->h_progress = 0;
     HIPCHK(hipHostGetDevicePointer(reinterpret_cast<void**>(&e->d_progress), e->h_progress, 0));
@@ -367,6 +368,8 @@
     {"x3_apb", "1", true, "f32x3 LM prefill: producers hand over pre-split, GEMMs staged by LDS-DMA (0 = register-staged kernel on fp32 activations)"},
     {"x3_attn", "1", true, "f32x3: prefill attention on exact bf16 splits (0 = exact fp32 MFMA kernel)"},
     {"x3w", "1", false, "f32x3: K = 96 GEMMs on the weight-stationary persistent kernel; bit-identical"},
+    {"dec_qkv0_table", "1", false, "f32 / f32x3: layer 0 of a decode step reads W'0 . embed[token] from a table built at load time with the decode kernels (189 MB); 0 = the q/k/v launch; bit-identical"},
+    {"dec_head_norm", "1", false, "f32x3, batches of one 32-row block: the lm_head forms its normalised pre-split operand itself; 0 = the final-norm launch; bit-identical"},
     {"row_migration", "1", false, "reference-semantics loop, B > 32: rows still running are packed into the lowest 32-row blocks; tokens unchanged"},
     {"arena_mb", "3400", false, "size of the weight arena in MiB (before the first tensor is loaded)"},
 };
@@ -394,6 +397,8 @@
     e->opt.x3_attn = opt_val(e, "x3_attn") != 0;
     e->opt.x3w = opt_val(e, "x3w") != 0;
     e->opt.row_migration = opt_val(e, "row_migration") != 0;
+    e->opt.dec_qkv0_table = opt_val(e, "dec_qkv0_table") != 0;
+    e->opt.dec_head_norm = opt_val(e, "dec_head_norm") != 0;
     e->opt.arena_mb = (int)opt_val(e, "arena_mb");
     e->opt.fp8 = mode == MELLOW_PRECISION_FP8;
     e->opt.fp8_decode = e->opt.fp8 && opt_val(e, "fp8_decode") != 0;
diff --git a/mellow_amd/csrc/engine_dev.cpp b/mellow_amd/csrc/engine_dev.cpp
--- a/mellow_amd/csrc/engine_dev.cpp
+++ b/mellow_amd/csrc/engine_dev.cpp
@@ -27,6 +27,34 @@
     *ms_out = ms / iters;
     hipEventDestroy(a); hipEventDestroy(b);
     return 0;
+}
+
+__attribute__((visibility("default"))) int mellow_dev_qkv0_rows(mellow_engine_t* e, const int32_t* ids, int n, float* slabs, float* ssq,
+                                                                float* rows, float* rows_ssq) {
+    if (!e || !e->finalized || !ids || !slabs || !ssq || !rows || !rows_ssq || n <= 0 || n > 1024) return fail("bad argument");
+    if (!e->w.q0 || !e->w.q0ssq) return fail("this engine holds no layer-0 table (option dec_qkv0_table = 0, or the fp8 mode)");
+    HIPCHK(hipSetDevice(e->device));
+    hipStream_t s = e->stream;
+    CHK(ensure_lm(e, n, 1, 2));
+    e->cur_B = 0;
+    const int V = e->cfg.vocab_size, Bp = e->da.rows;
+    e->h_pos_word = 0;
+    HIPCHK(hipMemcpyAsync(e->d_pos, &e->h_pos_word, sizeof(int32_t), hipMemcpyHostToDevice, s));
+    DecArgs a = e->da;
+    a.blk_live = nullptr; a.row_of_slot = nullptr; a.first = 1; a.inc_pos = 0;
+    launch_dec_load_rows(a, n, e->w.embed, 576, ids, 0, V, s);
+    const LMLayerW& w0 = e->w.layers[0];
+    launch_dec_qkv(a, w0.qkv_f.p, w0.qkv_f.KP / 8, 0, s, nullptr);
+    HIPCHK(hipMemcpy2DAsync(slabs, (size_t)n * 960 * 4, a.pq, (size_t)Bp * 960 * 4, (size_t)n * 960 * 4, DEC_KC_QKV, hipMemcpyDeviceToDevice, s));
+    HIPCHK(hipMemcpyAsync(ssq, a.ssq1, (size_t)n * DEC_KC_QKV * 4, hipMemcpyDeviceToDevice, s));
+    launch_gather_rows(e->w.q0, 960, ids, n, V, rows, s);
+    launch_gather_rows(e->w.q0ssq, DEC_KC_QKV, ids, n, V, rows_ssq, s);
+    HIPCHK(hipGetLastError());
+    HIPCHK(hipStreamSynchronize(s));
+    return 0;
+}
+__attribute__((visibility("default"))) int64_t mellow_dev_qkv0_table_ptr(mellow_engine_t* e) {
+    return e ? (int64_t)reinterpret_cast<uintptr_t>(e->w.q0) : 0;
 }
 
 int mellow_debug_gemm_f32(mellow_engine_t* e, int mode, const float* A, int M, int K, const float* W, int N, float* C_out,
diff --git a/mellow_amd/csrc/engine_internal.h b/mellow_amd/csrc/engine_internal.h
--- a/mellow_amd/csrc/engine_internal.h
+++ b/mellow_amd/csrc/engine_internal.h
@@ -135,6 +135,8 @@
         int enc_apb_stages = 0x1CC;
         int sk_max = 8;
         int dec_fuse_max_rb = 1;
+        bool dec_qkv0_table = true;
+        bool dec_head_norm = true;
     };
     struct Fp8W { uint8_t* w8; float* scale; };
     struct LOCAL Weights {
@@ -154,6 +156,7 @@
         std::vector<LMLayerW> layers;
         float* final_norm = nullptr;
         float *rope_cos = nullptr, *rope_sin = nullptr;
+        float *q0 = nullptr, *q0ssq = nullptr;
         float *head8 = nullptr, *head_sc = nullptr;
         DecW head_w() const { return head8 ? DecW{head8, head_sc} : DecW{lm_head.p, nullptr}; }
         std::unordered_map<const float*, void*> bf_w;
@@ -209,6 +212,7 @@
     DecArgs da;
     int32_t *d_tokens = nullptr, *d_step = nullptr, *d_pos = nullptr, *d_seen = nullptr, *d_nseen = nullptr;
     int32_t *d_arrive = nullptr, *d_ticket = nullptr, *d_params = nullptr;
+    int32_t* d_pos_done = nullptr;
     int32_t *d_blk_left = nullptr, *d_blk_live = nullptr;
     int32_t *d_row_of_slot = nullptr, *d_ncompact = nullptr;
     int last_compactions = 0;
@@ -296,8 +300,9 @@
 LoopArgs loop_args(mellow_engine* e);
 int run_lm_head(mellow_engine* e, int B, int pending_kcd, const RecordArgs* rec);
 int run_prefill(mellow_engine* e, int B, int T, const RecordArgs* rec, bool all_positions = false);
-int enqueue_decode_layer_range(mellow_engine* e, int B, int l_begin, int l_end, bool inc_pos);
-int enqueue_decode_layers(mellow_engine* e, int B, const RecordArgs* rec);
+int enqueue_decode_layer_range(mellow_engine* e, int B, int l_begin, int l_end, bool inc_pos, const int32_t* tok0 = nullptr);
+int enqueue_decode_layers(mellow_engine* e, int B, const RecordArgs* rec, const int32_t* tok0);
+int build_qkv0_table(mellow_engine* e);
 int ensure_prefill_streams(mellow_engine* e);
 int encode_pair_to_prefix(mellow_engine* e, const float* a1, const float* a2, int64_t n_samples, const int32_t* ids, int B, float* prefix_out);
 int run_score_head(mellow_engine* e, int B, int T, int from_pos, int n, const int32_t* targets, float* out_logprob,
diff --git a/mellow_amd/csrc/engine_lm.cpp b/mellow_amd/csrc/engine_lm.cpp
--- a/mellow_amd/csrc/engine_lm.cpp
+++ b/mellow_amd/csrc/engine_lm.cpp
@@ -83,8 +83,32 @@
         }
         a.pq = p + o_pq; a.attF16 = p + o_att; a.att_ml = p + o_aml; a.ssq = p + o_ssq; a.guF = p + o_gu; a.xmidF16 = p + o_xmidF16;
         a.logits = e->dlogits.p; a.cand_val = e->cand.p; a.cand_idx = reinterpret_cast<int32_t*>(e->cand.p + (size_t)Bp * (V / 32));
+        a.q0 = e->w.q0; a.q0ssq = e->w.q0ssq; a.q0_vocab = (int)V; a.tok0 = nullptr; a.d_pos_done = e->d_pos_done;
+        a.head_norm = e->opt.dec_head_norm ? 1 : 0;
     }
     if (Bp > 1024) return fail("batch too large for the decode state block");
+    return 0;
+}
+
+int build_qkv0_table(mellow_engine* e) {
+    const int V = e->cfg.vocab_size;
+    e->w.q0 = e->w.q0ssq = nullptr;
+    if (!e->opt.dec_qkv0_table || e->opt.fp8_decode || e->cfg.hidden_size != 576 || e->w.layers.empty() || !e->w.layers[0].qkv_f.p) return 0;
+    CHK(dev_alloc(e, &e->w.q0, (size_t)V * 960));
+    CHK(dev_alloc(e, &e->w.q0ssq, (size_t)V * DEC_KC_QKV));
+    constexpr int RBT = 32, R = RBT * 32;
+    mellow_engine::Buf ws;
+    const size_t n_x = (size_t)R * 576, n_pq = (size_t)DEC_KC_QKV * R * 960, n_sq = (size_t)R * DEC_KC_QKV;
+    CHK(ensure(e, ws, 2 * n_x + n_pq + n_sq));
+    HIPCHK(hipMemsetAsync(ws.p, 0, (2 * n_x + n_pq + n_sq) * sizeof(float), e->stream));
+    DecArgs t;
+    t.rows = R; t.RB = RBT; t.eps = e->cfg.rms_norm_eps;
+    t.xmidF = ws.p; t.xnewR = ws.p + n_x; t.pq = ws.p + 2 * n_x; t.ssq1 = ws.p + 2 * n_x + n_pq;
+    const LMLayerW& w0 = e->w.layers[0];
+    for (int id0 = 0; id0 < V; id0 += R)
+        launch_dec_qkv0_table(t, w0.qkv_f.p, w0.qkv_f.KP / 8, e->w.embed, V, id0, V - id0 < R ? V - id0 : R, e->w.q0, e->w.q0ssq, e->stream);
+    HIPCHK(hipGetLastError());
+    HIPCHK(hipStreamSynchronize(e->stream));
     return 0;
 }
 
@@ -111,11 +135,13 @@
 int run_lm_head(mellow_engine* e, int B, int pending_kcd, const RecordArgs* rec) {
     const int NT = e->cfg.vocab_size / 32, Bp = e->da.rows;
     auto dh = [&](int k) { DecArgs x = e->da; x.dbg_seq = e->dbg_seq0 >= 0 ? e->dbg_seq0 + 5 * e->cfg.num_layers + k : -1000; return x; };
+    const DecW h = e->w.head_w();
+    const bool head_norm = pending_kcd == DEC_KC_DOWN && !h.scale && dec_head_norm_fits(e->da, e->cfg.vocab_size);
+    if (!head_norm)
     { ProfScope ps(e, PF_NORM, 0, (double)(pending_kcd + 2) * Bp * 576 * 4);
       launch_dec_final_norm(dh(0), e->w.final_norm, pending_kcd, e->stream); }
     { ProfScope ps(e, PF_SKINNY, 2.0 * Bp * 576.0 * e->cfg.vocab_size, 576.0 * e->cfg.vocab_size * 4);
-      const DecW h = e->w.head_w();
-      launch_dec_lm_head(dh(1), h.p, e->w.lm_head.KP / 8, e->cfg.vocab_size, e->stream, h.scale); }
+      launch_dec_lm_head(dh(1), h.p, e->w.lm_head.KP / 8, e->cfg.vocab_size, e->stream, h.scale, head_norm ? e->w.final_norm : nullptr); }
     { ProfScope ps(e, PF_MISC, 0, 0);
       if (e->sample_on) {
           SampleArgs sa;
@@ -126,7 +152,7 @@
           launch_dec_argmax(dh(2), B, NT, e->d_tokens, e->w.embed, (rec && rec->embed_next) ? 1 : 0, rec ? loop_args(e) : LoopArgs(),
                             e->stream);
       }
-      if (rec && e->da.row_of_slot) launch_dec_compact(e->da, B, loop_args(e), e->stream); }
+      if (rec && e->da.row_of_slot) launch_dec_compact(e->da, B, loop_args(e), e->stream, e->d_tokens); }
     return 0;
 }
 
@@ -260,9 +286,10 @@
     return 0;
 }
 
-int enqueue_decode_layer_range(mellow_engine* e, int B, int l_begin, int l_end, bool inc_pos) {
+int enqueue_decode_layer_range(mellow_engine* e, int B, int l_begin, int l_end, bool inc_pos, const int32_t* tok0) {
     hipStream_t s = e->stream;
     const int Bp = e->da.rows;
+    const bool table0 = tok0 && l_begin == 0 && e->opt.dec_qkv0_table && e->w.q0 && !e->opt.kv16 && !e->w.layers[0].qkv8;
 #ifdef MELLOW_DEVPROBE
     static const bool same_w = getenv("MELLOW_DEV_SAME_WEIGHTS") != nullptr, same_kv = getenv("MELLOW_DEV_SAME_KV") != nullptr;
     static const int skip = getenv("MELLOW_DEV_SKIP") ? atoi(getenv("MELLOW_DEV_SKIP")) : 0;
@@ -285,12 +312,15 @@
         a.dbg_seq = sq;
         a.first = l == l_begin ? 1 : 0;
         a.inc_pos = (inc_pos && l == l_begin) ? 1 : 0;
-        if (!(skip & 1) && !fused_in)
+        const bool tab = table0 && l == 0 && !same_w;
+        if (!(skip & 1) && !fused_in && !tab)
         { ProfScope ps(e, PF_SKINNY, 2.0 * Bp * 576.0 * 960.0, 576.0 * 960.0 * 4);
           launch_dec_qkv(a, qkv.p, w.qkv_f.KP / 8, kcd, s, qkv.scale); }
         if (!(skip & 2))
         { ProfScope ps(e, PF_DECODE_ATTN, 4.0 * 64 * 9 * (double)B * (e->cur_pos + 1), 2.0 * (double)B * 3 * 64 * 4 * (e->cur_pos + 1));
-          launch_dec_attn(da(1), kc, vc, fused_in, s); }
+          DecArgs at = da(1);
+          if (tab) { at.tok0 = tok0; at.inc_pos = a.inc_pos; }
+          launch_dec_attn(at, kc, vc, fused_in, s, tab); }
         if (!(skip & 4))
         { ProfScope ps(e, PF_SKINNY, 2.0 * Bp * 576.0 * 576.0, 576.0 * 576.0 * 4);
           launch_dec_oproj(da(2), o.p, s, o.scale); }
@@ -311,8 +341,8 @@
     }
     return 0;
 }
-int enqueue_decode_layers(mellow_engine* e, int B, const RecordArgs* rec) {
-    CHK(enqueue_decode_layer_range(e, B, 0, e->cfg.num_layers, true));
+int enqueue_decode_layers(mellow_engine* e, int B, const RecordArgs* rec, const int32_t* tok0) {
+    CHK(enqueue_decode_layer_range(e, B, 0, e->cfg.num_layers, true, tok0));
     CHK(run_lm_head(e, B, DEC_KC_DOWN, rec));
     return 0;
 }
@@ -321,7 +351,7 @@
     hipGraph_t gr = nullptr;
     HIPCHK(hipStreamBeginCapture(e->stream, hipStreamCaptureModeThreadLocal));
     int rc = 0;
-    for (int k = 0; k < n && !rc; ++k) rc = enqueue_decode_layers(e, B, rec);
+    for (int k = 0; k < n && !rc; ++k) rc = enqueue_decode_layers(e, B, rec, e->d_tokens);
     hipError_t err = hipStreamEndCapture(e->stream, &gr);
     if (!rc && err != hipSuccess) rc = fail("hipStreamEndCapture failed: %s", hipGetErrorString(err));
     if (!rc && (err = hipGraphInstantiate(exec, gr, nullptr, nullptr, 0)) != hipSuccess) { *exec = nullptr; rc = fail("instantiating the captured decode step failed: %s", hipGetErrorString(err)); }
@@ -447,7 +477,8 @@
     HIPCHK(hipSetDevice(e->device));
     const int B = e->cur_B;
     launch_dec_load_rows(e->da, B, e->w.embed, 576, token_ids, 0, e->cfg.vocab_size, e->stream);
-    CHK(enqueue_decode_layers(e, B, nullptr));
+    HIPCHK(hipMemcpyAsync(e->d_tokens, token_ids, (size_t)B * sizeof(int32_t), hipMemcpyDeviceToDevice, e->stream));
+    CHK(enqueue_decode_layers(e, B, nullptr, e->d_tokens));
     e->cur_pos += 1;
     if (logits)
         HIPCHK(hipMemcpyAsync(logits, e->dlogits.p, (size_t)B * e->cfg.vocab_size * 4, hipMemcpyDeviceToDevice, e->stream));
@@ -765,7 +796,7 @@
             const bool eight = graph && i + 8 <= max_len;
             if (eight) HIPCHK(hipGraphLaunch(e->graphs.eight, s));
             else if (graph) HIPCHK(hipGraphLaunch(e->graphs.one, s));
-            else CHK(enqueue_decode_layers(e, B, &rec));
+            else CHK(enqueue_decode_layers(e, B, &rec, e->d_tokens));
             i += eight ? 8 : 1;
             e->cur_pos += eight ? 8 : 1;
             steps_done = i;
@@ -775,7 +806,7 @@
     } else {
         for (int i = 1; i < max_len; ++i) {
             if (graph) HIPCHK(hipGraphLaunch(e->graphs.one, s));
-            else CHK(enqueue_decode_layers(e, B, &rec));
+            else CHK(enqueue_decode_layers(e, B, &rec, e->d_tokens));
             e->cur_pos += 1;
             steps_done = i + 1;
             unsigned nseen = 0;
diff --git a/mellow_amd/csrc/engine_weights.cpp b/mellow_amd/csrc/engine_weights.cpp
--- a/mellow_amd/csrc/engine_weights.cpp
+++ b/mellow_amd/csrc/engine_weights.cpp
@@ -375,6 +375,7 @@
         CHK(upload(e, &e->w.rope_sin, s.data(), s.size()));
     }
     CHK(alloc_state_words(e));
+    CHK(build_qkv0_table(e));
     e->host.clear();
     e->finalized = true;
     return 0;
diff --git a/mellow_amd/csrc/kernels.h b/mellow_amd/csrc/kernels.h
--- a/mellow_amd/csrc/kernels.h
+++ b/mellow_amd/csrc/kernels.h
@@ -142,10 +142,18 @@
     int dbg_seq = -1;
     float* logits = nullptr;
     float* cand_val = nullptr; int32_t* cand_idx = nullptr;
+    const float* q0 = nullptr;
+    const float* q0ssq = nullptr;
+    const int32_t* tok0 = nullptr;
+    int q0_vocab = 0;
+    int32_t* d_pos_done = nullptr;
+    int head_norm = 0;
 };
 void launch_dec_qkv(const DecArgs& a, const float* Wp_folded, int K8p, int kcd, hipStream_t s, const float* wscale = nullptr);
 void launch_pack_dec_fp8(const float* Wp, int tiles, int slots_per_tile, int rows_per_tile, void* out, float* scale, hipStream_t s);
-void launch_dec_attn(const DecArgs& a, float* k_cache, float* v_cache, bool fused, hipStream_t s);
+void launch_dec_attn(const DecArgs& a, float* k_cache, float* v_cache, bool fused, hipStream_t s, bool table = false);
+void launch_dec_qkv0_table(const DecArgs& a, const float* Wp_folded, int K8p, const float* embed, int vocab, int id0, int n, float* q0,
+                           float* q0ssq, hipStream_t s);
 void launch_kv_to_bf16(const float* src, void* dst, int64_t n, hipStream_t s);
 void launch_dec_qkv2(const DecArgs& a, const float* Wq2, const float* Wd, hipStream_t s);
 void launch_dec_qkv2x3(const DecArgs& a, const float* Wq2, const float* Wd, hipStream_t s);
@@ -159,8 +167,10 @@
 void launch_dec_gateup(const DecArgs& a, const float* Wp16_folded_pairs, hipStream_t s, const float* wscale = nullptr);
 void launch_dec_down(const DecArgs& a, const float* Wp, int K8p, hipStream_t s, const float* wscale = nullptr);
 void launch_dec_final_norm(const DecArgs& a, const float* norm_w, int kcd, hipStream_t s);
+bool dec_head_norm_fits(const DecArgs& a, int vocab);
 bool dec_head3r_fits(int vocab);
-void launch_dec_lm_head(const DecArgs& a, const float* Wp, int K8p, int vocab, hipStream_t s, const float* wscale = nullptr);
+void launch_dec_lm_head(const DecArgs& a, const float* Wp, int K8p, int vocab, hipStream_t s, const float* wscale = nullptr,
+                        const float* norm_w = nullptr);
 struct LoopArgs {
     int32_t* out_tokens = nullptr;
     const int32_t* params = nullptr;
@@ -189,7 +199,7 @@
 void launch_dec_sample(const SampleArgs& sa, const DecArgs& a, int B, int32_t* tokens, const float* embed, int write_x,
                        const LoopArgs& loop, hipStream_t s);
 void launch_sample_logits(const SampleArgs& sa, int B, int32_t* tokens, hipStream_t s);
-void launch_dec_compact(const DecArgs& a, int B, const LoopArgs& loop, hipStream_t s);
+void launch_dec_compact(const DecArgs& a, int B, const LoopArgs& loop, hipStream_t s, int32_t* tokens = nullptr);
 void launch_dec_load_rows(const DecArgs& a, int B, const float* in, int64_t ld, const int32_t* row_ids, int T_last,
                           int n_src , hipStream_t s);
 void launch_pack_weight16(const float* w, int N, int K, float* out, hipStream_t s);
diff --git a/mellow_amd/csrc/sample.hip b/mellow_amd/csrc/sample.hip
--- a/mellow_amd/csrc/sample.hip
+++ b/mellow_amd/csrc/sample.hip
@@ -226,6 +226,7 @@
                                                                  const float* __restrict__ embed, int write_x, const LoopArgs lp) {
     __shared__ int tok_s;
     const int b = blockIdx.x, tid = threadIdx.x;
+    if (b == 0 && tid == 0 && a.d_pos_done) *a.d_pos_done = *a.d_pos;
     const int row = lp.row_of_slot ? lp.row_of_slot[b] : b;
     const bool dead = (lp.blk_snap && lp.blk_snap[b >> 5] == 0) || row < 0;
     int idx = 0;
```

Measured after the change: 456.6. -1.3%, worse.
